# bmartacho/UniPose

Hardware: AMD Instinct MI355X
Metric: images/sec fwd+bwd, UniPose ResNet-101 368x368 (higher is better)
Workload: dtype f32; 1 GPU; UniPose ResNet-101 (K=16) train step: fwd + MSE + bwd + Adam, synthetic 368x368, batch 32/GPU (BASELINE.json configs[1]; configs[2] for N>1); global_batch=32, per_gpu_batch=32, parallelism=dp1, optimizer=torch.optim.Adam(lr=1e-4, fused=True), arithmetic=fp32 MFMA 32x32x2 everywhere

## Files before the change

include/unipose_hip.h:

```cpp
#ifndef UNIPOSE_HIP_H
#define UNIPOSE_HIP_H

#include <stddef.h>
#include <stdint.h>

#ifdef __cplusplus
extern "C" {
#endif

typedef enum {
    UP_OK = 0,
    UP_ERR_INVALID = -1,
    UP_ERR_UNSUPPORTED = -2,
    UP_ERR_LAUNCH = -3,
    UP_ERR_WORKSPACE = -4
} up_status;

const char* up_last_error(void);
int up_abi_version(void);

typedef struct {
    int32_t N, H, W;
    int32_t C, Cp;
    int32_t ldx;
    int32_t K;
    int32_t R, S;
    int32_t stride, pad, dil;
    int32_t P, Q;
    int32_t ldy;
    int32_t Kp;
} up_conv_desc;

typedef struct {
    float eps, momentum;
    float* running_mean;
    float* running_var;
    const float* gamma;
    const float* beta;
    float* mean;
    float* invstd;
    float* scale;
    float* shift;
    int32_t folded;
} up_bn_fold;
typedef struct {
    const float* scale;
    const float* shift;
    const float* bias;
    const float* residual;
    int32_t ldr;
    int32_t relu;
    float* stats;
    up_bn_fold* fold;
} up_conv_epilogue;

int up_pack_weights(const up_conv_desc* d, const float* w_oihw, float* w_fwd, float* w_dgrad, void* stream);
typedef struct {
    const float* w;
    float* w_fwd;
    float* w_dgrad;
    int32_t K, C, Cp, Kp, taps;
    int32_t geometry;
} up_pack_job;
int up_pack_weights_batched(const up_pack_job* jobs_device, int njobs, void* stream);

int up_conv2d_fwd(const up_conv_desc* d, const float* x, const float* w_fwd, float* y,
                  const up_conv_epilogue* ep, void* stream);
int up_conv_stats_tiles(const up_conv_desc* d);
int up_conv_stats_tiles_math(const up_conv_desc* d, int math);
int up_conv_split_parts(const up_conv_desc* d);
int up_stream_release(void* stream);
int up_stream_create_cu_mask(const uint32_t* mask, int words, void** stream);
int up_stream_destroy(void* stream);
int up_probe_placement(int blocks, int* out_device, void* stream);
int up_conv_tune(const char* key, int value);
long long up_conv_counter(const char* name);
int up_conv_tap_visits(const up_conv_desc* d, int data_gradient, double* image_order, double* tap_sorted, double* live);
int up_conv_wgrad_visits(const up_conv_desc* d, double* rect_fraction);

int up_conv2d_bwd_data(const up_conv_desc* d, const float* dy, const float* w_dgrad, float* dx,
                       const float* add, int ld_add, void* stream);
int up_bn_stats_groups_t(const void* y, int ldy, int64_t rows_per_group, int C, int groups, int dtype, float* stats, float eps,
                         float momentum, float* running_mean, float* running_var, const float* gamma, const float* beta, float* coef,
                         void* stream);
int up_bn_bwd_groups_finalized_t(const void* dz, int lddz, const uint32_t* relu_bits, const void* y, int ldy, const float* gamma,
                                 const float* coef, int relu, void* dy, int lddy, void* dres, int lddres, const float* gsum,
                                 int64_t rows_per_group, int C, int groups, int dtype, void* stream);
int up_bn_bwd_groups_prereduced_ok(int64_t rows_per_group, int C, int groups, int ld);
int up_bn_bwd_groups_prereduced_t(const void* dz, int lddz, const uint32_t* relu_bits, const void* y, int ldy, const float* gamma,
                                  const float* coef, int relu, void* dy, int lddy, void* dres, int lddres, float* dgamma, float* dbeta,
                                  float* workspace, size_t workspace_bytes, const float* partial, int tiles, int64_t rows_per_group,
                                  int C, int groups, int dtype, void* stream);
int up_conv_stats_tiles_grouped(const up_conv_desc* d, int groups);
int up_conv2d_fwd_grouped(const up_conv_desc* d, const float* x, const float* w_fwd, float* y, float* stats, int groups, void* stream);

typedef struct {
    const void* y;
    const uint32_t* relu_bits;
    const float* mean;
    const float* invstd;
    float* partial;
    int32_t ld, C;
    int32_t group_stride;
    float* dgamma;
    float* dbeta;
    float* gsum;
    int32_t folded;
} up_bn_reduce_slot;
typedef struct {
    const void* add;
    const uint32_t* add_relu_bits;
    up_bn_reduce_slot* bn;
    int32_t ld_add;
    int32_t groups;
} up_dgrad_epilogue;
int up_conv2d_bwd_data_tiles_grouped(const up_conv_desc* d, int groups);
int up_conv2d_bwd_data_tiles(const up_conv_desc* d);
int up_conv2d_bwd_data_tiles_math(const up_conv_desc* d, int math);
int up_conv2d_bwd_data_ex(const up_conv_desc* d, const void* dy, const void* w_dgrad, void* dx, const up_dgrad_epilogue* ep,
                          int math, void* stream);

typedef enum { UP_MATH_F32 = 0, UP_MATH_BF16X3 = 1, UP_MATH_BF16 = 2, UP_MATH_BF16S = 3, UP_MATH_BF16S_F32OUT = 4 } up_math;
int up_pack_weights_bf16(const up_conv_desc* d, const float* w_oihw, uint16_t* fwd_hi, uint16_t* fwd_lo,
                         uint16_t* dgrad_hi, uint16_t* dgrad_lo, void* stream);
typedef struct {
    const float* w;
    uint16_t* fwd_hi;
    uint16_t* fwd_lo;
    uint16_t* dgrad_hi;
    uint16_t* dgrad_lo;
    int32_t K, C, Cp, Kp, taps, reserved;
} up_pack_job_bf16;
int up_pack_weights_bf16_batched(const up_pack_job_bf16* jobs_device, int njobs, void* stream);
int up_conv2d_fwd_bf16(const up_conv_desc* d, const float* x, const uint16_t* w_hi, const uint16_t* w_lo, float* y,
                       const up_conv_epilogue* ep, int math, void* stream);
int up_conv2d_bwd_data_bf16(const up_conv_desc* d, const float* dy, const uint16_t* w_hi, const uint16_t* w_lo,
                            float* dx, const float* add, int ld_add, int math, void* stream);

size_t up_conv2d_bwd_weight_workspace(const up_conv_desc* d);
int up_conv2d_bwd_weight(const up_conv_desc* d, const float* x, const float* dy, float* dw_oihw,
                         float* dbias, void* workspace, size_t workspace_bytes, void* stream);
int up_conv2d_bwd_weight_bf16(const up_conv_desc* d, const float* x, const float* dy, float* dw_oihw,
                              float* dbias, void* workspace, size_t workspace_bytes, void* stream);

enum { UP_DT_F32 = 0, UP_DT_BF16 = 1 };
int up_conv2d_bwd_weight_bf16s(const up_conv_desc* d, const void* x_bf16, const void* dy_bf16, float* dw_oihw,
                               float* dbias, void* workspace, size_t workspace_bytes, void* stream);

int up_conv2d_bwd_weight_acc(const up_conv_desc* d, const void* x, const void* dy, float* dw_oihw, float* dbias,
                             void* workspace, size_t workspace_bytes, int math, int accumulate, void* stream);

int up_bn_eval_coeffs(const float* gamma, const float* beta, const float* running_mean,
                      const float* running_var, float eps, int C, float* scale, float* shift, void* stream);
int up_bn_finalize(const float* stats, int tiles, int C, float eps, float momentum,
                   float* running_mean, float* running_var,
                   const float* gamma, const float* beta,
                   float* mean, float* invstd, float* scale, float* shift, void* stream);
int up_bn_apply(const float* y, int ldy, const float* scale, const float* shift,
                const float* residual, int ldr, int relu, float* z, int ldz, uint32_t* relu_bits,
                int64_t rows, int C, void* stream);
int up_bn_bwd(const float* dz, int lddz, const float* z, int ldz, const uint32_t* relu_bits,
              const float* y, int ldy,
              const float* gamma, const float* mean, const float* invstd, int relu, int use_batch_stats,
              float* dy, int lddy, float* dres, int lddres, float* dgamma, float* dbeta,
              float* workspace, size_t workspace_bytes, int64_t rows, int C, void* stream);
size_t up_bn_bwd_workspace(int64_t rows, int C);
int up_bn_apply_t(const void* y, int ldy, const float* scale, const float* shift, const void* residual, int ldr,
                  int relu, void* z, int ldz, uint32_t* relu_bits, int64_t rows, int C, int dtype, void* stream);
int up_bn_apply_centered_t(const void* y, int ldy, const float* mean, const float* scale, const float* beta, const void* residual,
                           int ldr, int relu, void* z, int ldz, uint32_t* relu_bits, int64_t rows, int C, int dtype, void* stream);
int up_bn_bwd_t(const void* dz, int lddz, const void* z, int ldz, const uint32_t* relu_bits, const void* y, int ldy,
                const float* gamma, const float* mean, const float* invstd, int relu, int use_batch_stats,
                void* dy, int lddy, void* dres, int lddres, float* dgamma, float* dbeta,
                float* workspace, size_t workspace_bytes, int64_t rows, int C, int dtype, void* stream);
int up_bn_bwd_acc_t(const void* dz, int lddz, const void* z, int ldz, const uint32_t* relu_bits, const void* y, int ldy,
                const float* gamma, const float* mean, const float* invstd, int relu, int use_batch_stats,
                void* dy, int lddy, void* dres, int lddres, float* dgamma, float* dbeta, float* acc_dgamma, float* acc_dbeta,
                float* workspace, size_t workspace_bytes, int64_t rows, int C, int dtype, void* stream);
int up_bn_bwd_prereduced_t(const void* dz, int lddz, const uint32_t* relu_bits, const void* y, int ldy, const float* gamma,
                           const float* mean, const float* invstd, int relu, int use_batch_stats, void* dy, int lddy, void* dres,
                           int lddres, float* dgamma, float* dbeta, float* acc_dgamma, float* acc_dbeta, float* partial, int chunks,
                           int64_t rows, int C, int dtype, void* stream);
int up_bn_bwd_finalized_t(const void* dz, int lddz, const uint32_t* relu_bits, const void* y, int ldy, const float* gamma,
                          const float* mean, const float* invstd, int relu, int use_batch_stats, void* dy, int lddy, void* dres,
                          int lddres, const float* dgamma, const float* dbeta, int64_t rows, int C, int dtype, void* stream);

int up_bn_exact_stats_t(const void* y, int ldy, int64_t rows_per_group, int C, int groups, int dtype, float* stats, void* stream);
int up_bn_batch_stats_tiles(int64_t rows_per_group);
int up_bn_batch_stats_t(const void* y, int ldy, int64_t rows_per_group, int C, int groups, int dtype, float* stats, void* stream);
int up_bn_finalize_groups(const float* stats, int tiles, int C, int groups, int64_t rows_per_group, float eps, float momentum,
                          float* running_mean, float* running_var, const float* gamma, const float* beta, float* coef,
                          void* stream);
int up_bn_apply_groups_t(const void* y, int ldy, const float* coef, const float* beta, const void* res, int ldr, int relu, void* z,
                         int ldz, uint32_t* relu_bits, int64_t rows_per_group, int C, int groups, int dtype, void* stream);
size_t up_bn_bwd_groups_workspace(int64_t rows_per_group, int C, int groups);
int up_bn_bwd_groups_t(const void* dz, int lddz, const uint32_t* relu_bits, const void* y, int ldy, const float* gamma,
                       const float* coef, int relu, void* dy, int lddy, void* dres, int lddres, float* dgamma, float* dbeta,
                       float* workspace, size_t workspace_bytes, int64_t rows_per_group, int C, int groups, int dtype,
                       void* stream);

int up_relu_bwd(const float* dz, const float* z, float* dx, int64_t n, void* stream);
int up_copy2d(const float* src, int lds, float* dst, int ldd, int64_t rows, int C, void* stream);
int up_add2d(const float* a, int lda, const float* b, int ldb, float* dst, int ldd, int64_t rows, int C, void* stream);
int up_nchw_to_nhwc(const float* x, float* y, int N, int C, int H, int W, int ldy, void* stream);
int up_nhwc_to_nchw(const float* x, int ldx, float* y, int N, int C, int H, int W, void* stream);
int up_maxpool3s2_fwd(const float* x, int ldx, float* y, int ldy, uint8_t* idx,
                      int N, int H, int W, int C, int P, int Q, void* stream);
int up_maxpool3s2_bwd(const float* dy, int lddy, const uint8_t* idx, float* dx, int lddx,
                      int N, int H, int W, int C, int P, int Q, void* stream);
int up_bilinear_fwd(const float* x, int ldx, float* y, int ldy, int N, int H, int W, int C, int P, int Q, void* stream);
int up_bilinear_bwd(const float* dy, int lddy, float* dx, int lddx, int N, int H, int W, int C, int P, int Q, void* stream);
int up_gap_fwd(const float* x, int ldx, float* y, int N, int HW, int C, void* stream);
int up_gap_bwd(const float* dy, float* dx, int lddx, int N, int HW, int C, void* stream);
int up_avgpool9s8_fwd(const float* x, float* y, int ldy, int coff, int N, int H, int W, int P, int Q, void* stream);
int up_clip_nchw_to_nhwc(const float* x, float* y, int B, int T, int C, int H, int W, int ldy, void* stream);
int up_clip_avgpool9s8_fwd(const float* x, float* y, int ldy, int coff, int B, int T, int H, int W, int P, int Q, void* stream);
int up_clip_nhwc_to_nchw(const float* x, int ldx, float* y, int B, int T, int C, int H, int W, void* stream);
int up_dropout_fwd(const float* x, float* y, uint8_t* mask, const float* ext_mask, int64_t n,
                   float p, uint64_t seed, void* stream);
int up_dropout_bwd(const float* dy, const uint8_t* mask, float* dx, int64_t n, float p, void* stream);
int up_nchw_to_nhwc_t(const float* x, void* y, int N, int C, int H, int W, int ldy, int dt_out, void* stream);
int up_nhwc_to_nchw_t(const void* x, int ldx, float* y, int N, int C, int H, int W, int dt_in, void* stream);
int up_maxpool3s2_fwd_t(const void* x, int ldx, void* y, int ldy, uint8_t* idx, int N, int H, int W, int C, int P, int Q,
                        int dt_in, int dt_out, void* stream);
int up_maxpool3s2_bwd_t(const void* dy, int lddy, const uint8_t* idx, void* dx, int lddx, int N, int H, int W, int C, int P,
                        int Q, int dt_in, int dt_out, void* stream);
int up_bilinear_fwd_t(const void* x, int ldx, void* y, int ldy, int N, int H, int W, int C, int P, int Q, int dtype,
                      void* stream);
int up_bilinear_bwd_t(const void* dy, int lddy, void* dx, int lddx, int N, int H, int W, int C, int P, int Q, int dtype,
                      void* stream);
int up_gap_fwd_t(const void* x, int ldx, void* y, int N, int HW, int C, int dtype, void* stream);
int up_gap_bwd_t(const void* dy, void* dx, int lddx, int N, int HW, int C, int dtype, void* stream);
int up_dropout_fwd_t(const void* x, void* y, uint8_t* mask, const float* ext_mask, int64_t n, float p, uint64_t seed,
                     int dtype, void* stream);
int up_dropout_fwd_step_t(const void* x, void* y, uint8_t* mask, const float* ext_mask, int64_t n, float p, uint64_t seed,
                          const uint64_t* step_device, int dtype, void* stream);
int up_dropout_bwd_t(const void* dy, const uint8_t* mask, void* dx, int64_t n, float p, int dtype, void* stream);
int up_mse_fwd(const float* y, const float* t, float* loss, float* workspace, int64_t n, void* stream);
int up_mse_bwd(const float* y, const float* t, const float* dloss, float* dy, int64_t n, void* stream);
size_t up_mse_workspace(int64_t n);

int up_lstm0_fwd(const float* gates, int ldg, float* cell, float* hide, int ldo, int64_t rows, int Cg, void* stream);
int up_lstm0_bwd(const float* gates, int ldg, const float* dcell, const float* dhide, int ldo,
                 float* dgates, int64_t rows, int Cg, void* stream);
int up_lstm_fwd(const float* gates, int ldg, const float* cprev, int ldc, float* cell, float* hide, int ldo,
                int64_t rows, int Cg, void* stream);
int up_lstm_bwd(const float* gates, int ldg, const float* cprev, int ldc, const float* cell,
                const float* dcell, const float* dhide, int ldo,
                float* dgates, float* dcprev, int64_t rows, int Cg, void* stream);

int up_heatmap_argmax(const float* hm, int B, int J, int H, int W,
                      int32_t* idx, float* preds_xy, float* maxvals, void* stream);

int up_heatmap_decode(const float* hm, int64_t stride_b, int64_t stride_j, int64_t stride_p, int B, int J, int H, int W,
                      int P, int Q, int32_t* idx, float* preds_xy, float* maxvals, void* stream);

int up_make_heatmaps(const double* kpt_xy, int B, int K, int H, int W, double stride, double sigma, float* out,
                     void* stream);
int up_make_gaussian_maps(const double* center_xy, int N, int H, int W, double sigma, float* out, void* stream);
int up_normalize_image(const float* img_hwc, int B, int H, int W, int C, float mean, float stdv, float* out_chw,
                       void* stream);

enum { UP_BOX_OK = 0, UP_BOX_NO_VISIBLE_JOINT = 1 };
int up_make_box_maps(const double* kpt_xy, int B, int K, int height, int width, double stride, double sigma, float* out,
                     int32_t* status, void* stream);

enum { UP_PIX_U8 = 0, UP_PIX_F32 = 1 };
int up_augment_image(const void* src_hwc, int src_type, int B, int Hs, int Ws, int C, const int32_t* valid_hw, const double* inv,
                     int frames_per_map, float border, float mean, float stdv, float* out_chw, int Ho, int Wo, void* stream);

enum { UP_DS_LSP = 0, UP_DS_COCO = 1, UP_DS_PENN_ACTION = 2, UP_DS_NTID = 3, UP_DS_POSETRACK = 4, UP_DS_BBC = 5,
       UP_DS_MPII = 6 };
int up_pck_accuracy(const float* pred_xy, const float* target_xy, int B, int J, int H, int W, int dataset,
                    double thr_pck, double thr_pckh, double* acc, double* pck, double* pckh, double* visible,
                    int32_t* cnt, void* stream);

int up_peak_mask(const float* maps, int nmaps, int H, int W, uint8_t* mask, void* stream);
int up_box_argmax(const float* maps, int C, int H, int W, const int32_t* boxes, int P, int ch0, int nch,
                  int32_t* out_hw, void* stream);

enum { UP_PERSONS_OK = 0, UP_PERSONS_MISSING_CORNER = 1, UP_PERSONS_EMPTY_BOX = 2, UP_PERSONS_OVERFLOW = 3 };
enum { UP_PERSONS_CAP = 512 };
int up_persons_decode(const float* maps, int64_t stride_b, int64_t stride_j, int64_t stride_p, int B, int C, int H, int W,
                      int box_ch0, int joint_ch0, int njoints, int max_persons, int32_t* count, int32_t* status, int32_t* kpts,
                      void* stream);

typedef struct up_unipose_plan up_unipose_plan;
typedef struct {
    int32_t batch, height, width;
    int32_t output_stride;
    int32_t out_channels;
} up_unipose_config;
int up_unipose_plan_create(const up_unipose_config* cfg, up_unipose_plan** plan);
void up_unipose_plan_destroy(up_unipose_plan* plan);
int up_unipose_plan_num_convs(const up_unipose_plan* plan);
const char* up_unipose_plan_conv_name(const up_unipose_plan* plan, int i);
int up_unipose_plan_conv_shape(const up_unipose_plan* plan, int i, int32_t* oihw , int32_t* has_bias);
int up_unipose_plan_set_conv(up_unipose_plan* plan, int i, const float* w_oihw, const float* bias, void* stream);
size_t up_unipose_plan_workspace(const up_unipose_plan* plan);
int up_unipose_forward(up_unipose_plan* plan, const float* x_nchw, float* heat_nchw, void* workspace, size_t workspace_bytes,
                       void* stream);
int up_unipose_forward_upsampled(up_unipose_plan* plan, const float* x_nchw, float* heat_nchw, void* workspace,
                                 size_t workspace_bytes, void* stream);
int up_unipose_keypoints(up_unipose_plan* plan, const float* x_nchw, int out_h, int out_w, int32_t* idx, float* preds_xy,
                         float* maxvals, void* workspace, size_t workspace_bytes, void* stream);
int up_unipose_persons(up_unipose_plan* plan, const float* x_nchw, int box_ch0, int joint_ch0, int njoints, int max_persons,
                       int32_t* count, int32_t* status, int32_t* kpts, void* workspace, size_t workspace_bytes, void* stream);

typedef struct up_unipose_lstm_plan up_unipose_lstm_plan;
typedef struct {
    int32_t batch, frames, height, width;
    int32_t output_stride;
    int32_t num_classes;
} up_unipose_lstm_config;
int up_unipose_lstm_plan_create(const up_unipose_lstm_config* cfg, up_unipose_lstm_plan** plan);
void up_unipose_lstm_plan_destroy(up_unipose_lstm_plan* plan);
int up_unipose_lstm_plan_num_convs(const up_unipose_lstm_plan* plan);
const char* up_unipose_lstm_plan_conv_name(const up_unipose_lstm_plan* plan, int i);
int up_unipose_lstm_plan_conv_shape(const up_unipose_lstm_plan* plan, int i, int32_t* oihw , int32_t* has_bias);
int up_unipose_lstm_plan_set_conv(up_unipose_lstm_plan* plan, int i, const float* w_oihw, const float* bias, void* stream);
size_t up_unipose_lstm_plan_workspace(const up_unipose_lstm_plan* plan);
int up_unipose_lstm_step(up_unipose_lstm_plan* plan, const float* x_nchw, const float* center_nchw, const float* prev_hide,
                         const float* prev_cell, float* heat_nchw, float* cell_nchw, float* hide_nchw, void* workspace,
// ... 16 lines not shown
```

unipose_amd/_C.py:

```python
from __future__ import annotations

import ctypes as C
import os

_HERE = os.path.dirname(os.path.abspath(__file__))
LIB_PATH = os.path.join(_HERE, "libunipose_hip.so")



class ConvDesc(C.Structure):
    _fields_ = [(n, C.c_int32) for n in
                ("N", "H", "W", "C", "Cp", "ldx", "K", "R", "S", "stride", "pad", "dil", "P", "Q", "ldy", "Kp")]


class BnFold(C.Structure):
    _fields_ = [("eps", C.c_float), ("momentum", C.c_float), ("running_mean", C.c_void_p), ("running_var", C.c_void_p),
                ("gamma", C.c_void_p), ("beta", C.c_void_p), ("mean", C.c_void_p), ("invstd", C.c_void_p), ("scale", C.c_void_p),
                ("shift", C.c_void_p), ("folded", C.c_int32)]


class ConvEpilogue(C.Structure):
    _fields_ = [("scale", C.c_void_p), ("shift", C.c_void_p), ("bias", C.c_void_p), ("residual", C.c_void_p),
                ("ldr", C.c_int32), ("relu", C.c_int32), ("stats", C.c_void_p), ("fold", C.POINTER(BnFold))]


_i, _i64, _f, _u64, _sz, _p = C.c_int, C.c_int64, C.c_float, C.c_uint64, C.c_size_t, C.c_void_p


class BnReduceSlot(C.Structure):
    _fields_ = [("y", C.c_void_p), ("relu_bits", C.c_void_p), ("mean", C.c_void_p), ("invstd", C.c_void_p),
                ("partial", C.c_void_p), ("ld", C.c_int32), ("C", C.c_int32), ("group_stride", C.c_int32),
                ("dgamma", C.c_void_p), ("dbeta", C.c_void_p), ("gsum", C.c_void_p), ("folded", C.c_int32)]


class DgradEpilogue(C.Structure):
    _fields_ = [("add", C.c_void_p), ("add_relu_bits", C.c_void_p), ("bn", C.POINTER(BnReduceSlot)), ("ld_add", C.c_int32),
                ("groups", C.c_int32)]


_D, _E = C.POINTER(ConvDesc), C.POINTER(ConvEpilogue)

SIGNATURES = {
    "up_last_error": (C.c_char_p, []),
    "up_abi_version": (_i, []),
    "up_pack_weights": (_i, [_D, _p, _p, _p, _p]),
    "up_conv2d_fwd": (_i, [_D, _p, _p, _p, _E, _p]),
    "up_pack_weights_batched": (_i, [_p, _i, _p]),
    "up_conv_stats_tiles": (_i, [_D]),
    "up_conv_stats_tiles_math": (_i, [_D, _i]),
    "up_conv_split_parts": (_i, [_D]),
    "up_stream_release": (_i, [_p]),
    "up_stream_create_cu_mask": (_i, [C.POINTER(C.c_uint32), _i, C.POINTER(_p)]),
    "up_stream_destroy": (_i, [_p]),
    "up_probe_placement": (_i, [_i, _p, _p]),
    "up_conv_tune": (_i, [C.c_char_p, _i]),
    "up_conv_counter": (C.c_longlong, [C.c_char_p]),
    "up_conv_wgrad_visits": (_i, [_D, C.POINTER(C.c_double)]),
    "up_conv_tap_visits": (_i, [_D, _i, C.POINTER(C.c_double), C.POINTER(C.c_double), C.POINTER(C.c_double)]),
    "up_conv2d_bwd_data": (_i, [_D, _p, _p, _p, _p, _i, _p]),
    "up_conv2d_bwd_data_tiles": (_i, [_D]),
    "up_conv2d_bwd_data_tiles_math": (_i, [_D, _i]),
    "up_conv2d_bwd_data_ex": (_i, [_D, _p, _p, _p, C.POINTER(DgradEpilogue), _i, _p]),
    "up_conv_stats_tiles_grouped": (_i, [_D, _i]),
    "up_conv2d_bwd_data_tiles_grouped": (_i, [_D, _i]),
    "up_bn_bwd_groups_prereduced_ok": (_i, [_i64, _i, _i, _i]),
    "up_bn_stats_groups_t": (_i, [_p, _i, _i64, _i, _i, _i, _p, _f, _f, _p, _p, _p, _p, _p, _p]),
    "up_bn_bwd_groups_finalized_t": (_i, [_p, _i, _p, _p, _i, _p, _p, _i, _p, _i, _p, _i, _p, _i64, _i, _i, _i, _p]),
    "up_bn_bwd_groups_prereduced_t": (_i, [_p, _i, _p, _p, _i, _p, _p, _i, _p, _i, _p, _i, _p, _p, _p, _sz, _p, _i, _i64, _i, _i, _i, _p]),
    "up_conv2d_fwd_grouped": (_i, [_D, _p, _p, _p, _p, _i, _p]),
    "up_bn_bwd_prereduced_t": (_i, [_p, _i, _p, _p, _i, _p, _p, _p, _i, _i, _p, _i, _p, _i, _p, _p, _p, _p, _p, _i, _i64, _i,
                                    _i, _p]),
    "up_bn_bwd_finalized_t": (_i, [_p, _i, _p, _p, _i, _p, _p, _p, _i, _i, _p, _i, _p, _i, _p, _p, _i64, _i, _i, _p]),
    "up_pack_weights_bf16": (_i, [_D, _p, _p, _p, _p, _p, _p]),
    "up_pack_weights_bf16_batched": (_i, [_p, _i, _p]),
    "up_conv2d_fwd_bf16": (_i, [_D, _p, _p, _p, _p, _E, _i, _p]),
    "up_conv2d_bwd_data_bf16": (_i, [_D, _p, _p, _p, _p, _p, _i, _i, _p]),
    "up_conv2d_bwd_weight_workspace": (_sz, [_D]),
    "up_conv2d_bwd_weight": (_i, [_D, _p, _p, _p, _p, _p, _sz, _p]),
    "up_conv2d_bwd_weight_bf16": (_i, [_D, _p, _p, _p, _p, _p, _sz, _p]),
    "up_conv2d_bwd_weight_bf16s": (_i, [_D, _p, _p, _p, _p, _p, _sz, _p]),
    "up_conv2d_bwd_weight_acc": (_i, [_D, _p, _p, _p, _p, _p, _sz, _i, _i, _p]),
    "up_bn_eval_coeffs": (_i, [_p, _p, _p, _p, _f, _i, _p, _p, _p]),
    "up_bn_finalize": (_i, [_p, _i, _i, _f, _f, _p, _p, _p, _p, _p, _p, _p, _p, _p]),
    "up_bn_apply": (_i, [_p, _i, _p, _p, _p, _i, _i, _p, _i, _p, _i64, _i, _p]),
    "up_bn_bwd": (_i, [_p, _i, _p, _i, _p, _p, _i, _p, _p, _p, _i, _i, _p, _i, _p, _i, _p, _p, _p, _sz, _i64, _i, _p]),
    "up_bn_bwd_workspace": (_sz, [_i64, _i]),
    "up_bn_apply_t": (_i, [_p, _i, _p, _p, _p, _i, _i, _p, _i, _p, _i64, _i, _i, _p]),
    "up_bn_bwd_t": (_i, [_p, _i, _p, _i, _p, _p, _i, _p, _p, _p, _i, _i, _p, _i, _p, _i, _p, _p, _p, _sz, _i64, _i, _i, _p]),
    "up_bn_bwd_acc_t": (_i, [_p, _i, _p, _i, _p, _p, _i, _p, _p, _p, _i, _i, _p, _i, _p, _i, _p, _p, _p, _p, _p, _sz, _i64, _i, _i, _p]),
    "up_bn_exact_stats_t": (_i, [_p, _i, _i64, _i, _i, _i, _p, _p]),
    "up_bn_batch_stats_tiles": (_i, [_i64]),
    "up_bn_batch_stats_t": (_i, [_p, _i, _i64, _i, _i, _i, _p, _p]),
    "up_bn_finalize_groups": (_i, [_p, _i, _i, _i, _i64, _f, _f, _p, _p, _p, _p, _p, _p]),
    "up_bn_apply_groups_t": (_i, [_p, _i, _p, _p, _p, _i, _i, _p, _i, _p, _i64, _i, _i, _i, _p]),
    "up_bn_apply_centered_t": (_i, [_p, _i, _p, _p, _p, _p, _i, _i, _p, _i, _p, _i64, _i, _i, _p]),
    "up_bn_bwd_groups_workspace": (_sz, [_i64, _i, _i]),
    "up_bn_bwd_groups_t": (_i, [_p, _i, _p, _p, _i, _p, _p, _i, _p, _i, _p, _i, _p, _p, _p, _sz, _i64, _i, _i, _i, _p]),
    "up_relu_bwd": (_i, [_p, _p, _p, _i64, _p]),
    "up_copy2d": (_i, [_p, _i, _p, _i, _i64, _i, _p]),
    "up_add2d": (_i, [_p, _i, _p, _i, _p, _i, _i64, _i, _p]),
    "up_nchw_to_nhwc": (_i, [_p, _p, _i, _i, _i, _i, _i, _p]),
    "up_nhwc_to_nchw": (_i, [_p, _i, _p, _i, _i, _i, _i, _p]),
    "up_maxpool3s2_fwd": (_i, [_p, _i, _p, _i, _p, _i, _i, _i, _i, _i, _i, _p]),
    "up_maxpool3s2_bwd": (_i, [_p, _i, _p, _p, _i, _i, _i, _i, _i, _i, _i, _p]),
    "up_bilinear_fwd": (_i, [_p, _i, _p, _i, _i, _i, _i, _i, _i, _i, _p]),
    "up_bilinear_bwd": (_i, [_p, _i, _p, _i, _i, _i, _i, _i, _i, _i, _p]),
    "up_gap_fwd": (_i, [_p, _i, _p, _i, _i, _i, _p]),
    "up_gap_bwd": (_i, [_p, _p, _i, _i, _i, _i, _p]),
    "up_avgpool9s8_fwd": (_i, [_p, _p, _i, _i, _i, _i, _i, _i, _i, _p]),
    "up_dropout_fwd": (_i, [_p, _p, _p, _p, _i64, _f, _u64, _p]),
    "up_dropout_bwd": (_i, [_p, _p, _p, _i64, _f, _p]),
    "up_nchw_to_nhwc_t": (_i, [_p, _p, _i, _i, _i, _i, _i, _i, _p]),
    "up_nhwc_to_nchw_t": (_i, [_p, _i, _p, _i, _i, _i, _i, _i, _p]),
    "up_maxpool3s2_fwd_t": (_i, [_p, _i, _p, _i, _p, _i, _i, _i, _i, _i, _i, _i, _i, _p]),
    "up_maxpool3s2_bwd_t": (_i, [_p, _i, _p, _p, _i, _i, _i, _i, _i, _i, _i, _i, _i, _p]),
    "up_bilinear_fwd_t": (_i, [_p, _i, _p, _i, _i, _i, _i, _i, _i, _i, _i, _p]),
    "up_bilinear_bwd_t": (_i, [_p, _i, _p, _i, _i, _i, _i, _i, _i, _i, _i, _p]),
    "up_gap_fwd_t": (_i, [_p, _i, _p, _i, _i, _i, _i, _p]),
    "up_gap_bwd_t": (_i, [_p, _p, _i, _i, _i, _i, _i, _p]),
    "up_dropout_fwd_t": (_i, [_p, _p, _p, _p, _i64, _f, _u64, _i, _p]),
    "up_dropout_fwd_step_t": (_i, [_p, _p, _p, _p, _i64, _f, _u64, _p, _i, _p]),
    "up_dropout_bwd_t": (_i, [_p, _p, _p, _i64, _f, _i, _p]),
    "up_mse_fwd": (_i, [_p, _p, _p, _p, _i64, _p]),
    "up_mse_bwd": (_i, [_p, _p, _p, _p, _i64, _p]),
    "up_mse_workspace": (_sz, [_i64]),
    "up_lstm0_fwd": (_i, [_p, _i, _p, _p, _i, _i64, _i, _p]),
    "up_lstm0_bwd": (_i, [_p, _i, _p, _p, _i, _p, _i64, _i, _p]),
    "up_lstm_fwd": (_i, [_p, _i, _p, _i, _p, _p, _i, _i64, _i, _p]),
    "up_lstm_bwd": (_i, [_p, _i, _p, _i, _p, _p, _p, _i, _p, _p, _i64, _i, _p]),
    "up_heatmap_argmax": (_i, [_p, _i, _i, _i, _i, _p, _p, _p, _p]),
    "up_heatmap_decode": (_i, [_p, _i64, _i64, _i64, _i, _i, _i, _i, _i, _i, _p, _p, _p, _p]),
    "up_make_heatmaps": (_i, [_p, _i, _i, _i, _i, C.c_double, C.c_double, _p, _p]),
    "up_make_box_maps": (_i, [_p, _i, _i, _i, _i, C.c_double, C.c_double, _p, _p, _p]),
    "up_make_gaussian_maps": (_i, [_p, _i, _i, _i, C.c_double, _p, _p]),
    "up_normalize_image": (_i, [_p, _i, _i, _i, _i, _f, _f, _p, _p]),
    "up_augment_image": (_i, [_p, _i, _i, _i, _i, _i, _p, _p, _i, _f, _f, _f, _p, _i, _i, _p]),
    "up_pck_accuracy": (_i, [_p, _p, _i, _i, _i, _i, _i, C.c_double, C.c_double, _p, _p, _p, _p, _p, _p]),
    "up_peak_mask": (_i, [_p, _i, _i, _i, _p, _p]),
    "up_box_argmax": (_i, [_p, _i, _i, _i, _p, _i, _i, _i, _p, _p]),
    "up_persons_decode": (_i, [_p, _i64, _i64, _i64, _i, _i, _i, _i, _i, _i, _i, _i, _p, _p, _p, _p]),
    "up_unipose_plan_create": (_i, [_p, C.POINTER(_p)]),
    "up_unipose_plan_destroy": (None, [_p]),
    "up_unipose_plan_num_convs": (_i, [_p]),
    "up_unipose_plan_conv_name": (C.c_char_p, [_p, _i]),
    "up_unipose_plan_conv_shape": (_i, [_p, _i, C.POINTER(C.c_int32), C.POINTER(C.c_int32)]),
    "up_unipose_plan_set_conv": (_i, [_p, _i, _p, _p, _p]),
    "up_unipose_plan_workspace": (_sz, [_p]),
    "up_unipose_forward": (_i, [_p, _p, _p, _p, _sz, _p]),
    "up_unipose_forward_upsampled": (_i, [_p, _p, _p, _p, _sz, _p]),
    "up_unipose_keypoints": (_i, [_p, _p, _i, _i, _p, _p, _p, _p, _sz, _p]),
    "up_unipose_persons": (_i, [_p, _p, _i, _i, _i, _i, _p, _p, _p, _p, _sz, _p]),
    "up_clip_nchw_to_nhwc": (_i, [_p, _p, _i, _i, _i, _i, _i, _i, _p]),
    "up_clip_avgpool9s8_fwd": (_i, [_p, _p, _i, _i, _i, _i, _i, _i, _i, _i, _p]),
    "up_clip_nhwc_to_nchw": (_i, [_p, _i, _p, _i, _i, _i, _i, _i, _p]),
    "up_unipose_lstm_plan_create": (_i, [_p, C.POINTER(_p)]),
    "up_unipose_lstm_plan_destroy": (None, [_p]),
    "up_unipose_lstm_plan_num_convs": (_i, [_p]),
    "up_unipose_lstm_plan_conv_name": (C.c_char_p, [_p, _i]),
    "up_unipose_lstm_plan_conv_shape": (_i, [_p, _i, C.POINTER(C.c_int32), C.POINTER(C.c_int32)]),
    "up_unipose_lstm_plan_set_conv": (_i, [_p, _i, _p, _p, _p]),
    "up_unipose_lstm_plan_workspace": (_sz, [_p]),
    "up_unipose_lstm_step": (_i, [_p, _p, _p, _p, _p, _p, _p, _p, _p, _sz, _p]),
    "up_unipose_lstm_clip": (_i, [_p, _p, _p, _p, _p, _p, _p, _sz, _p]),
    "up_profile_variants": (_i, []),
    "up_profile_variant_name": (C.c_char_p, [_i]),
    "up_profile_begin": (_i, []),
    "up_profile_enable": (_i, [_i]),
    "up_profile_live_flops": (_i, [C.POINTER(C.c_double), _i]),
    "up_profile_end": (_i, [C.POINTER(C.c_double), _i]),
}

_lib = None
_ALLOW_HOST_POINTERS = False


class UniPoseHipError(RuntimeError):
    pass


def load(path: str | None = None):
    global _lib
    path = path or LIB_PATH
    if not os.path.exists(path):
        raise UniPoseHipError(
            f"{path} not found: build it with `python -c 'import __graft_entry__ as g; g.build()'` "
            "(hipcc --offload-arch=gfx950).  unipose_amd has no non-HIP fallback.")
    lib = C.CDLL(path)
    for name, (res, args) in SIGNATURES.items():
        fn = getattr(lib, name)
        fn.restype = res
        fn.argtypes = args
    _lib = lib
    return lib


def lib():
    return _lib if _lib is not None else load()


def check(status: int, what: str = ""):
    if status != 0:
        msg = lib().up_last_error().decode(errors="replace")
        if status == -2:
            raise NotImplementedError(f"{what}: {msg}")
        raise UniPoseHipError(f"{what}: status {status}: {msg}")
```

unipose_amd/csrc/norm_act.hip:

```cpp
#include "up_common.h"
#include "bn_fold.h"

#include <stdarg.h>
#include <stdlib.h>

namespace up {

static thread_local char g_err[512] = "";
void set_error(const char* fmt, ...) {
    va_list ap;
    va_start(ap, fmt);
    vsnprintf(g_err, sizeof(g_err), fmt, ap);
    va_end(ap);
}
int check_launch(const char* what) {
    hipError_t e = hipGetLastError();
    if (e != hipSuccess) {
        set_error("%s: %s", what, hipGetErrorString(e));
        return UP_ERR_LAUNCH;
    }
    return UP_OK;
}

static inline int grid_for(int64_t work_items, int per_block = 256, int cap = 16384) {
    int64_t g = (work_items + per_block - 1) / per_block;
    if (g < 1) g = 1;
    return (int)(g > cap ? cap : g);
}

__device__ __forceinline__ void wf_merge3(float& n1, float& m1, float& s1, float n2, float m2, float s2) {
    if (n2 == 0.f) return;
    if (n1 == 0.f) {
        n1 = n2;
        m1 = m2;
        s1 = s2;
        return;
    }
    float n = n1 + n2;
    float d = m2 - m1;
    m1 = m1 + d * (n2 / n);
    s1 = s1 + s2 + d * d * (n1 * n2 / n);
    n1 = n;
}

__global__ void __launch_bounds__(256) bn_eval_coeffs_kernel(const float* g, const float* b, const float* rm,
                                                             const float* rv, float eps, int C, float* scale,
                                                             float* shift) {
    int c = blockIdx.x * 256 + threadIdx.x;
    if (c >= C) return;
    float is = 1.0f / sqrtf(rv[c] + eps);
    float sc = g[c] * is;
    scale[c] = sc;
    shift[c] = b[c] - rm[c] * sc;
}

struct GroupArgs {
    int pstride, gstride;
};

template <int NV>
__global__ void __launch_bounds__(256) bn_fold_arrive_kernel(const float* partial, BnFold f) {
    __shared__ __attribute__((aligned(16))) unsigned char lds[FOLD_LDS_BYTES];
    const int c0 = blockIdx.y * FOLD_COLS;
    bn_fold_arrive<NV>(f, partial, blockIdx.x, c0, f.C - c0 < FOLD_COLS ? f.C - c0 : FOLD_COLS, lds, blockIdx.z);
}

__global__ void __launch_bounds__(256) bn_finalize_kernel(const float* stats, int tiles, int C, float eps, float mom,
                                                          float* rm, float* rv, const float* gamma,
                                                          const float* beta, float* mean_o, float* invstd_o,
                                                          float* scale, float* shift, GroupArgs grp) {
    __shared__ float red[256][3];
    const int c = blockIdx.x, t0 = threadIdx.x;
    {
        const int g = blockIdx.y;
        stats += (size_t)g * tiles * C * 3;
        mean_o += (size_t)g * grp.pstride;
        invstd_o += (size_t)g * grp.pstride;
        scale += (size_t)g * grp.pstride;
        shift += (size_t)g * grp.pstride;
    }
    float n = 0.f, m = 0.f, q = 0.f;
    for (int t = t0; t < tiles; t += 512) {
        const float* s = stats + ((size_t)t * C + c) * 3;
        const int t2 = t + 256;
        const float* s2 = stats + ((size_t)(t2 < tiles ? t2 : t) * C + c) * 3;
        const float a0 = s[0], a1 = s[1], a2 = s[2];
        const float b0 = t2 < tiles ? s2[0] : 0.f, b1 = s2[1], b2 = s2[2];
        wf_merge3(n, m, q, a0, a1, a2);
        wf_merge3(n, m, q, b0, b1, b2);
    }
    red[t0][0] = n;
    red[t0][1] = m;
    red[t0][2] = q;
    __syncthreads();
#pragma unroll
    for (int off = 128; off >= 1; off >>= 1) {
        if (t0 < off) {
            wf_merge3(n, m, q, red[t0 + off][0], red[t0 + off][1], red[t0 + off][2]);
            red[t0][0] = n;
            red[t0][1] = m;
            red[t0][2] = q;
        }
        __syncthreads();
    }
    if (t0 == 0) {
        float var = q / n;
        float is = 1.0f / sqrtf(var + eps);
        mean_o[c] = m;
        invstd_o[c] = is;
        float sc = gamma[c] * is;
        scale[c] = sc;
        shift[c] = beta[c] - m * sc;
        if (rm) {
            float unb = n > 1.f ? q / (n - 1.f) : var;
            rm[c] = (1.f - mom) * rm[c] + mom * m;
            rv[c] = (1.f - mom) * rv[c] + mom * unb;
        }
    }
}

template <typename T>
__global__ void __launch_bounds__(256) bn_apply_kernel(const T* y, int ldy, const float* scale,
                                                       const float* shift, const float* mean, const T* res, int ldr, int relu,
                                                       T* z, int ldz, uint32_t* relu_bits, int64_t total, int C4,
                                                       FastDiv fC4) {
    const int lane = threadIdx.x & 63;
    for (int64_t i0 = (int64_t)blockIdx.x * 256 + (threadIdx.x & ~63); i0 < total; i0 += (int64_t)gridDim.x * 256) {
        const int64_t i = i0 + lane;
        uint32_t nib = 0;
        if (i < total) {
            uint32_t row = fdiv((uint32_t)i, fC4);
            int c = ((int)i - (int)row * C4) * 4;
            float4 v = ld4<T>(y + (size_t)row * ldy + c);
            float4 s = *reinterpret_cast<const float4*>(scale + c);
            float4 h = *reinterpret_cast<const float4*>(shift + c);
            const float4 mu = mean ? *reinterpret_cast<const float4*>(mean + c) : make_float4(0.f, 0.f, 0.f, 0.f);
            v.x = (v.x - mu.x) * s.x + h.x;
            v.y = (v.y - mu.y) * s.y + h.y;
            v.z = (v.z - mu.z) * s.z + h.z;
            v.w = (v.w - mu.w) * s.w + h.w;
            if (res) {
                float4 r = ld4<T>(res + (size_t)row * ldr + c);
                v.x += r.x;
                v.y += r.y;
                v.z += r.z;
                v.w += r.w;
            }
            if (relu) {
                v.x = fmaxf(v.x, 0.f);
                v.y = fmaxf(v.y, 0.f);
                v.z = fmaxf(v.z, 0.f);
                v.w = fmaxf(v.w, 0.f);
            }
            st4(z + (size_t)row * ldz + c, v);
            nib = (v.x > 0.f ? 1u : 0u) | (v.y > 0.f ? 2u : 0u) | (v.z > 0.f ? 4u : 0u) | (v.w > 0.f ? 8u : 0u);
        }
        if (relu_bits) {
            uint32_t w = nib << (4 * (lane & 7));
            w |= __shfl_xor(w, 1);
            w |= __shfl_xor(w, 2);
            w |= __shfl_xor(w, 4);
            if ((lane & 7) == 0 && i < total) relu_bits[i >> 3] = w;
        }
    }
}

struct F8 {
    float v[8];
};
__device__ __forceinline__ F8 ld8(const bf16_t* p) {
    const uint4 u = *reinterpret_cast<const uint4*>(p);
    F8 r;
    r.v[0] = bf_lo(u.x); r.v[1] = bf_hi(u.x); r.v[2] = bf_lo(u.y); r.v[3] = bf_hi(u.y);
    r.v[4] = bf_lo(u.z); r.v[5] = bf_hi(u.z); r.v[6] = bf_lo(u.w); r.v[7] = bf_hi(u.w);
    return r;
}
__device__ __forceinline__ F8 ld8(const float* p) {
    const float4 a = *reinterpret_cast<const float4*>(p), b = *reinterpret_cast<const float4*>(p + 4);
    F8 r;
    r.v[0] = a.x; r.v[1] = a.y; r.v[2] = a.z; r.v[3] = a.w; r.v[4] = b.x; r.v[5] = b.y; r.v[6] = b.z; r.v[7] = b.w;
    return r;
}
__device__ __forceinline__ void st8(bf16_t* p, const F8& a) {
    uint4 u;
    u.x = pack_bf16x2(a.v[0], a.v[1]);
    u.y = pack_bf16x2(a.v[2], a.v[3]);
    u.z = pack_bf16x2(a.v[4], a.v[5]);
    u.w = pack_bf16x2(a.v[6], a.v[7]);
    *reinterpret_cast<uint4*>(p) = u;
}

__global__ void __launch_bounds__(256) bn_apply8_kernel(const bf16_t* y, int ldy, const float* scale, const float* shift,
                                                        const float* mean, const bf16_t* res, int ldr, int relu, bf16_t* z, int ldz,
                                                        uint32_t* relu_bits, int64_t total, int C8, FastDiv fC8) {
    const int lane = threadIdx.x & 63;
    for (int64_t i0 = (int64_t)blockIdx.x * 256 + (threadIdx.x & ~63); i0 < total; i0 += (int64_t)gridDim.x * 256) {
        const int64_t i = i0 + lane;
        uint32_t byte = 0;
        if (i < total) {
            const uint32_t row = fdiv((uint32_t)i, fC8);
            const int c = ((int)i - (int)row * C8) * 8;
            F8 v = ld8(y + (size_t)row * ldy + c);
            const F8 s = ld8(scale + c), h = ld8(shift + c);
            F8 mu;
#pragma unroll
            for (int e = 0; e < 8; ++e) mu.v[e] = 0.f;
            if (mean) mu = ld8(mean + c);
#pragma unroll
            for (int e = 0; e < 8; ++e) v.v[e] = (v.v[e] - mu.v[e]) * s.v[e] + h.v[e];
            if (res) {
                const F8 r = ld8(res + (size_t)row * ldr + c);
#pragma unroll
                for (int e = 0; e < 8; ++e) v.v[e] += r.v[e];
            }
            if (relu) {
#pragma unroll
                for (int e = 0; e < 8; ++e) v.v[e] = fmaxf(v.v[e], 0.f);
            }
            st8(z + (size_t)row * ldz + c, v);
#pragma unroll
            for (int e = 0; e < 8; ++e) byte |= v.v[e] > 0.f ? (1u << e) : 0u;
        }
        if (relu_bits) {
            uint32_t w = byte << (8 * (lane & 3));
            w |= __shfl_xor(w, 1);
            w |= __shfl_xor(w, 2);
            if ((lane & 3) == 0 && i < total) relu_bits[i >> 2] = w;
        }
    }
}

template <typename T>
struct Row16 {
    static constexpr int E = 16 / (int)sizeof(T);
    float v[E];
};
__device__ __forceinline__ Row16<float> ld16(const float* p) {
    const float4 a = *reinterpret_cast<const float4*>(p);
    return Row16<float>{{a.x, a.y, a.z, a.w}};
}
__device__ __forceinline__ Row16<bf16_t> ld16(const bf16_t* p) {
    const uint4 u = *reinterpret_cast<const uint4*>(p);
    return Row16<bf16_t>{{bf_lo(u.x), bf_hi(u.x), bf_lo(u.y), bf_hi(u.y), bf_lo(u.z), bf_hi(u.z), bf_lo(u.w), bf_hi(u.w)}};
}
__device__ __forceinline__ void st16(float* p, const Row16<float>& a) {
    *reinterpret_cast<float4*>(p) = make_float4(a.v[0], a.v[1], a.v[2], a.v[3]);
}
__device__ __forceinline__ void st16(bf16_t* p, const Row16<bf16_t>& a) {
    uint4 u;
    u.x = pack_bf16x2(a.v[0], a.v[1]);
    u.y = pack_bf16x2(a.v[2], a.v[3]);
    u.z = pack_bf16x2(a.v[4], a.v[5]);
    u.w = pack_bf16x2(a.v[6], a.v[7]);
    *reinterpret_cast<uint4*>(p) = u;
}
template <int E>
__device__ __forceinline__ void ldparam(const float* p, float (&o)[E]) {
#pragma unroll
    for (int e = 0; e < E; e += 4) {
        const float4 a = *reinterpret_cast<const float4*>(p + e);
        o[e] = a.x;
        o[e + 1] = a.y;
        o[e + 2] = a.z;
        o[e + 3] = a.w;
    }
}
constexpr int BN_ROWS_UNROLL = 4;

template <typename T>
__global__ void __launch_bounds__(256) bn_apply_rows_kernel(const T* __restrict__ y, int ldy, const float* __restrict__ scale,
                                                            const float* __restrict__ shift, const float* __restrict__ mean,
                                                            const T* __restrict__ res, int ldr,
                                                            int relu, T* __restrict__ z, int ldz, uint32_t* __restrict__ relu_bits,
                                                            int rows, int C, int lcs, GroupArgs grp) {
    constexpr int E = Row16<T>::E, LPW = 32 / E;
    const int lane = threadIdx.x & 63;
    const int64_t grow0 = (int64_t)blockIdx.z * rows;
    y += grow0 * ldy;
    z += grow0 * ldz;
    if (res) res += grow0 * ldr;
    scale += (size_t)blockIdx.z * grp.pstride;
    shift += mean ? 0 : (size_t)blockIdx.z * grp.pstride;
    const int cl = threadIdx.x & ((1 << lcs) - 1), rl = threadIdx.x >> lcs;
    const int rpb = 256 >> lcs;
    const int c = ((blockIdx.y << lcs) + cl) * E;
    float sc[E], sh[E], mu[E];
    ldparam<E>(scale + c, sc);
    ldparam<E>(shift + c, sh);
#pragma unroll
    for (int e = 0; e < E; ++e) mu[e] = 0.f;
    if (mean) ldparam<E>(mean + (size_t)blockIdx.z * grp.pstride + c, mu);
    const int stride = gridDim.x * rpb;
    for (int base = blockIdx.x * rpb; base < rows; base += BN_ROWS_UNROLL * stride) {
        Row16<T> v[BN_ROWS_UNROLL], r[BN_ROWS_UNROLL];
#pragma unroll
        for (int u = 0; u < BN_ROWS_UNROLL; ++u) {
            const int row = base + u * stride + rl;
            const int rr = row < rows ? row : rows - 1;
            v[u] = ld16(y + (size_t)rr * ldy + c);
            if (res) r[u] = ld16(res + (size_t)rr * ldr + c);
        }
#pragma unroll
        for (int u = 0; u < BN_ROWS_UNROLL; ++u) {
            const int row = base + u * stride + rl;
            const bool ok = row < rows;
            uint32_t bits = 0;
#pragma unroll
            for (int e = 0; e < E; ++e) {
                float t = (v[u].v[e] - mu[e]) * sc[e] + sh[e];
                if (res) t += r[u].v[e];
                if (relu) t = fmaxf(t, 0.f);
                v[u].v[e] = t;
                bits |= t > 0.f ? (1u << e) : 0u;
            }
            if (ok) st16(z + (size_t)row * ldz + c, v[u]);
            if (relu_bits) {
                uint32_t w = bits << (E * (lane & (LPW - 1)));
#pragma unroll
                for (int m = 1; m < LPW; m <<= 1) w |= __shfl_xor(w, m);
                if ((lane & (LPW - 1)) == 0 && ok) relu_bits[((grow0 + row) * C + c) >> 5] = w;
            }
        }
    }
}

template <typename T, int UNROLL, bool ZPATH>
__global__ void __launch_bounds__(256) bn_bwd_apply_rows_kernel(const T* __restrict__ dz, int lddz, const T* __restrict__ z, int ldz,
                                                                const uint32_t* __restrict__ bits, const T* __restrict__ y, int ldy,
                                                                const float* __restrict__ gamma, const float* __restrict__ mean,
                                                                const float* __restrict__ invstd, const float* __restrict__ dgamma,
                                                                const float* __restrict__ dbeta, int relu, int use_batch, float inv_m,
                                                                T* __restrict__ dy, int lddy, T* __restrict__ dres, int lddres,
                                                                int rows, int C, int lcs, GroupArgs grp) {
    constexpr int E = Row16<T>::E;
    const int64_t grow0 = (int64_t)blockIdx.z * rows;
    dz += grow0 * lddz;
    y += grow0 * ldy;
    dy += grow0 * lddy;
    if (ZPATH) z += grow0 * ldz;
    if (dres) dres += grow0 * lddres;
    mean += (size_t)blockIdx.z * grp.pstride;
    invstd += (size_t)blockIdx.z * grp.pstride;
    dgamma += (size_t)blockIdx.z * grp.gstride;
    dbeta += (size_t)blockIdx.z * grp.gstride;
    const int cl = threadIdx.x & ((1 << lcs) - 1), rl = threadIdx.x >> lcs;
    const int rpb = 256 >> lcs;
    const int c = ((blockIdx.y << lcs) + cl) * E;
    float kk[E], aa[E], bb[E], mu[E];
    {
        float is[E], t[E];
        ldparam<E>(invstd + c, is);
        ldparam<E>(gamma + c, kk);
        ldparam<E>(mean + c, mu);
#pragma unroll
        for (int e = 0; e < E; ++e) kk[e] *= is[e];
        ldparam<E>(dbeta + c, t);
#pragma unroll
        for (int e = 0; e < E; ++e) aa[e] = use_batch ? -kk[e] * t[e] * inv_m : 0.f;
        ldparam<E>(dgamma + c, t);
#pragma unroll
        for (int e = 0; e < E; ++e) bb[e] = use_batch ? -kk[e] * is[e] * t[e] * inv_m : 0.f;
    }
    const int stride = gridDim.x * rpb;
    for (int base = blockIdx.x * rpb + rl; base < rows; base += UNROLL * stride) {
        Row16<T> g[UNROLL], yv[UNROLL], zz[ZPATH ? UNROLL : 1];
        uint32_t mk[UNROLL];
#pragma unroll
        for (int u = 0; u < UNROLL; ++u) {
            const int row = base + u * stride;
            const int rr = row < rows ? row : rows - 1;
            g[u] = ld16(dz + (size_t)rr * lddz + c);
            yv[u] = ld16(y + (size_t)rr * ldy + c);
            mk[u] = 0xffffffffu;
            if (ZPATH) {
                zz[u] = ld16(z + (size_t)rr * ldz + c);
            } else if (relu) {
                const int64_t b = (grow0 + rr) * C + c;
                mk[u] = bits[b >> 5] >> (int)(b & 31);
            }
        }
#pragma unroll
        for (int u = 0; u < UNROLL; ++u) {
            const int row = base + u * stride;
            if (row >= rows) continue;
            Row16<T> o;
#pragma unroll
            for (int e = 0; e < E; ++e) {
                float ge = g[u].v[e];
                const bool pos = ZPATH ? zz[ZPATH ? u : 0].v[e] > 0.f : ((mk[u] >> e) & 1u) != 0u;
                if (!pos) ge = 0.f;
                g[u].v[e] = ge;
                o.v[e] = kk[e] * ge + (aa[e] + (yv[u].v[e] - mu[e]) * bb[e]);
            }
            if (dres) st16(dres + (size_t)row * lddres + c, g[u]);
            st16(dy + (size_t)row * lddy + c, o);
        }
    }
}
template <typename T>
static void launch_bn_bwd_apply_rows(dim3 grid, hipStream_t st, const T* dz, int lddz, const T* z, int ldz, const uint32_t* bits,
                                     const T* y, int ldy, const float* gamma, const float* mean, const float* invstd,
                                     const float* dgamma, const float* dbeta, int relu, int use_batch, float inv_m, T* dy, int lddy,
                                     T* dres, int lddres, int rows, int C, int lcs, GroupArgs grp) {
    constexpr int U = sizeof(T) == 4 ? 1 : 2;
    if (relu && !bits)
        hipLaunchKernelGGL((bn_bwd_apply_rows_kernel<T, U, true>), grid, dim3(256), 0, st, dz, lddz, z, ldz, bits, y, ldy, gamma, mean,
                           invstd, dgamma, dbeta, relu, use_batch, inv_m, dy, lddy, dres, lddres, rows, C, lcs, grp);
    else
        hipLaunchKernelGGL((bn_bwd_apply_rows_kernel<T, U, false>), grid, dim3(256), 0, st, dz, lddz, z, ldz, bits, y, ldy, gamma, mean,
                           invstd, dgamma, dbeta, relu, use_batch, inv_m, dy, lddy, dres, lddres, rows, C, lcs, grp);
}
template <typename T>
static bool rows_geometry(int64_t rows, int C, dim3& grid, int& lcs) {
    constexpr int E = 16 / (int)sizeof(T);
    if (C % E) return false;
    const int cgs = C / E;
    if (cgs < 8 || (cgs & (cgs - 1)) || rows >= (1ll << 31)) return false;
    const int lc = cgs < 256 ? cgs : 256;
    lcs = 0;
    while ((1 << lcs) < lc) ++lcs;
    const int rpb = 256 / lc, gy = cgs / lc;
    int64_t gx = (rows + (int64_t)rpb * BN_ROWS_UNROLL - 1) / ((int64_t)rpb * BN_ROWS_UNROLL);
    const int64_t cap = 2048 / gy;
    if (gx > cap) gx = cap;
    if (gx < 1) gx = 1;
    grid = dim3((unsigned)gx, (unsigned)gy);
    return true;
}
static int g_bn_rows = -1;
void set_bn_rows(int on) { g_bn_rows = on ? 1 : 0; }
static bool bn_rows_enabled() {
    if (g_bn_rows < 0) {
        const char* e = getenv("UP_BN_ROWS");
        g_bn_rows = (e && atoi(e) == 0) ? 0 : 1;
    }
    return g_bn_rows != 0;
}

constexpr int BNS_ROWS = 256;
template <typename T>
__global__ void __launch_bounds__(256) bn_batch_stats_kernel(const T* y, int ldy, int rows_per_group, int C, float* stats, int tiles,
                                                             BnFold fold) {
    __shared__ __attribute__((aligned(16))) float red[16][64][3];
    static_assert(sizeof(float) * 16 * 64 * 3 >= FOLD_LDS_BYTES, "the fold's ticket re-uses the reduction buffer");
    const int cq = threadIdx.x & 15, rl = threadIdx.x >> 4;
    const int c = blockIdx.y * 64 + cq * 4;
    const int g = blockIdx.z;
    const int r0 = blockIdx.x * BNS_ROWS, r1 = min(rows_per_group, r0 + BNS_ROWS);
    float n = 0.f, sh[4] = {0.f, 0.f, 0.f, 0.f}, s[4] = {0.f, 0.f, 0.f, 0.f}, q[4] = {0.f, 0.f, 0.f, 0.f};
    if (c < C) {
        const T* base = y + (size_t)g * rows_per_group * ldy + c;
        const float4 s0 = ld4<T>(base + (size_t)r0 * ldy);
        sh[0] = s0.x, sh[1] = s0.y, sh[2] = s0.z, sh[3] = s0.w;
        auto acc = [&](const float4& v) {
            const float x[4] = {v.x, v.y, v.z, v.w};
#pragma unroll
            for (int e = 0; e < 4; ++e) {
                const float d = x[e] - sh[e];
                s[e] += d;
                q[e] += d * d;
            }
            n += 1.f;
        };
// ... 287 lines not shown

__device__ __forceinline__ uint32_t mix_hash(uint64_t seed, uint64_t idx) {
    uint64_t v = seed ^ (idx * 0x9E3779B97F4A7C15ull);
    v ^= v >> 30;
    v *= 0xBF58476D1CE4E5B9ull;
    v ^= v >> 27;
    v *= 0x94D049BB133111EBull;
    v ^= v >> 31;
    return (uint32_t)(v >> 40);
}
template <typename T>
__global__ void __launch_bounds__(256) dropout_fwd_kernel(const T* x, T* y, uint8_t* mask,
                                                          const float* ext, int64_t n, float p, float inv_keep,
                                                          uint64_t seed, const uint64_t* step_dev) {
    if (step_dev) seed += *step_dev * 0x9E3779B97F4A7C15ull;
    for (int64_t i = (int64_t)blockIdx.x * 256 + threadIdx.x; i < n; i += (int64_t)gridDim.x * 256) {
        bool keep;
        if (ext)
            keep = ext[i] != 0.f;
        else
            keep = (float)mix_hash(seed, (uint64_t)i) * (1.0f / 16777216.0f) >= p;
        mask[i] = keep ? 1 : 0;
        st1(y + i, keep ? ld1(x + i) * inv_keep : 0.f);
    }
}
template <typename T>
__global__ void __launch_bounds__(256) dropout_bwd_kernel(const T* dy, const uint8_t* mask, T* dx, int64_t n,
                                                          float inv_keep) {
    for (int64_t i = (int64_t)blockIdx.x * 256 + threadIdx.x; i < n; i += (int64_t)gridDim.x * 256)
        st1(dx + i, mask[i] ? ld1(dy + i) * inv_keep : 0.f);
}

__device__ __forceinline__ float block_sum_256(float v, float* red) {
#pragma unroll
    for (int off = 32; off >= 1; off >>= 1) v += __shfl_down(v, off);
    if ((threadIdx.x & 63) == 0) red[threadIdx.x >> 6] = v;
    __syncthreads();
    return red[0] + red[1] + red[2] + red[3];
}
__global__ void __launch_bounds__(256) mse_partial_kernel(const float* y, const float* t, float* ws, int64_t n) {
    __shared__ float red[4];
    float s = 0.f;
    for (int64_t i = (int64_t)blockIdx.x * 256 + threadIdx.x; i < n; i += (int64_t)gridDim.x * 256) {
        float d = y[i] - t[i];
        s += d * d;
    }
    s = block_sum_256(s, red);
    if (threadIdx.x == 0) ws[blockIdx.x] = s;
}
__global__ void __launch_bounds__(256) mse_final_kernel(const float* ws, int parts, float inv_n, float* loss) {
    __shared__ float red[4];
    float s = 0.f;
    for (int i = threadIdx.x; i < parts; i += 256) s += ws[i];
    s = block_sum_256(s, red);
    if (threadIdx.x == 0) loss[0] = s * inv_n;
}
__global__ void __launch_bounds__(256) mse_bwd_kernel(const float* y, const float* t, const float* dloss, float* dy,
                                                      int64_t n, float two_inv_n) {
    float k = two_inv_n * dloss[0];
    for (int64_t i = (int64_t)blockIdx.x * 256 + threadIdx.x; i < n; i += (int64_t)gridDim.x * 256)
        dy[i] = (y[i] - t[i]) * k;
}

constexpr int MSE_PARTS = 512;
constexpr int BNB_ROWS = 128;

}

using namespace up;

extern "C" const char* up_last_error(void) { return g_err; }
extern "C" int up_stream_create_cu_mask(const uint32_t* mask, int words, void** stream) {
    UP_REQUIRE(mask && words > 0 && stream, UP_ERR_INVALID, "stream_create_cu_mask: bad argument");
#ifdef UP_EMU
    *stream = nullptr;
    return UP_OK;
#else
    hipStream_t st = nullptr;
    hipError_t e = hipExtStreamCreateWithCUMask(&st, (uint32_t)words, mask);
    if (e != hipSuccess) {
        set_error("stream_create_cu_mask: %s", hipGetErrorString(e));
        return UP_ERR_LAUNCH;
    }
    *stream = st;
    return UP_OK;
#endif
}
extern "C" int up_stream_destroy(void* stream) {
#ifndef UP_EMU
    if (stream && hipStreamDestroy(as_stream(stream)) != hipSuccess) {
        (void)hipGetLastError();
        return UP_ERR_LAUNCH;
    }
#endif
    return UP_OK;
}
namespace up {
__global__ void __launch_bounds__(64) placement_kernel(int* out) {
#ifndef UP_EMU
    if (threadIdx.x == 0) {
        const unsigned xcc = __builtin_amdgcn_s_getreg((20 << 0) | (0 << 6) | (3 << 11));
        const unsigned hw = __builtin_amdgcn_s_getreg((4 << 0) | (0 << 6) | (31 << 11));
        out[2 * blockIdx.x] = (int)(xcc & 15u);
        out[2 * blockIdx.x + 1] = (int)((hw >> 8) & 0xffu);
        for (int i = 0; i < 2000; ++i) __builtin_amdgcn_s_sleep(32);
    }
#else
    if (threadIdx.x == 0) out[2 * blockIdx.x] = out[2 * blockIdx.x + 1] = 0;
#endif
}
}
extern "C" int up_probe_placement(int blocks, int* out_device, void* stream) {
    UP_REQUIRE(blocks > 0 && out_device, UP_ERR_INVALID, "probe_placement: bad argument");
    hipLaunchKernelGGL(placement_kernel, dim3(blocks), dim3(64), 0, as_stream(stream), out_device);
    return check_launch("probe_placement");
}

extern "C" int up_abi_version(void) { return 10; }

extern "C" int up_bn_eval_coeffs(const float* gamma, const float* beta, const float* rm, const float* rv, float eps,
                                 int C, float* scale, float* shift, void* stream) {
    UP_REQUIRE(gamma && beta && rm && rv && scale && shift && C > 0, UP_ERR_INVALID, "bn_eval_coeffs: bad argument");
    hipLaunchKernelGGL(bn_eval_coeffs_kernel, dim3(cdiv(C, 256)), dim3(256), 0, as_stream(stream), gamma, beta, rm,
                       rv, eps, C, scale, shift);
    return check_launch("bn_eval_coeffs");
}

extern "C" int up_bn_finalize(const float* stats, int tiles, int C, float eps, float momentum, float* rm, float* rv,
                              const float* gamma, const float* beta, float* mean, float* invstd, float* scale,
                              float* shift, void* stream) {
    UP_REQUIRE(stats && gamma && beta && mean && invstd && scale && shift && tiles > 0 && C > 0, UP_ERR_INVALID,
               "bn_finalize: bad argument");
    UP_REQUIRE((rm == nullptr) == (rv == nullptr), UP_ERR_INVALID, "bn_finalize: running stats must come in pairs");
    BnFold f;
    memset(&f, 0, sizeof(f));
    UP_REQUIRE(bn_fold_scratch(as_stream(stream), tiles, C, 3, &f), UP_ERR_WORKSPACE,
               "bn_finalize: %d partial rows x %d channels exceed the per-stream merge scratch", tiles, C);
    f.eps = eps;
    f.mom = momentum;
    f.rm = rm;
    f.rv = rv;
    f.gamma = gamma;
    f.beta = beta;
    f.mean = mean;
    f.invstd = invstd;
    f.scale = scale;
    f.shift = shift;
    hipLaunchKernelGGL(bn_fold_arrive_kernel<3>, dim3(tiles, cdiv(C, FOLD_COLS)), dim3(256), 0, as_stream(stream), stats, f);
    return check_launch("bn_finalize");
}

static int bn_apply_impl(const void* y, int ldy, const float* mean, const float* scale, const float* shift, const void* res,
                         int ldr, int relu, void* z, int ldz, uint32_t* relu_bits, int64_t rows, int C, int dtype,
                         void* stream) {
    UP_REQUIRE(y && scale && shift && z && rows > 0 && C > 0, UP_ERR_INVALID, "bn_apply: bad argument");
    UP_REQUIRE(C % 4 == 0 && ldy % 4 == 0 && ldz % 4 == 0 && (!res || ldr % 4 == 0), UP_ERR_INVALID,
               "bn_apply: C and strides must be multiples of 4");
    UP_REQUIRE(rows * (C / 4) < (1ll << 31), UP_ERR_UNSUPPORTED, "bn_apply: tensor too large");
    UP_REQUIRE(dtype == UP_DT_F32 || dtype == UP_DT_BF16, UP_ERR_INVALID, "bn_apply: dtype %d", dtype);
    int64_t total = rows * (C / 4);
    {
        dim3 grid;
        int lcs = 0;
        if (bn_rows_enabled() && dtype == UP_DT_BF16 && ldy % 8 == 0 && ldz % 8 == 0 && (!res || ldr % 8 == 0) &&
            rows_geometry<bf16_t>(rows, C, grid, lcs)) {
            hipLaunchKernelGGL(bn_apply_rows_kernel<bf16_t>, grid, dim3(256), 0, as_stream(stream), (const bf16_t*)y, ldy, scale,
                               shift, mean, (const bf16_t*)res, ldr, relu, (bf16_t*)z, ldz, relu_bits, (int)rows, C, lcs, GroupArgs{0, 0});
            return check_launch("bn_apply");
        }
        if (bn_rows_enabled() && dtype == UP_DT_F32 && rows_geometry<float>(rows, C, grid, lcs)) {
            hipLaunchKernelGGL(bn_apply_rows_kernel<float>, grid, dim3(256), 0, as_stream(stream), (const float*)y, ldy, scale,
                               shift, mean, (const float*)res, ldr, relu, (float*)z, ldz, relu_bits, (int)rows, C, lcs, GroupArgs{0, 0});
            return check_launch("bn_apply");
        }
    }
    if (dtype == UP_DT_BF16 && C % 8 == 0 && ldy % 8 == 0 && ldz % 8 == 0 && (!res || ldr % 8 == 0))
        hipLaunchKernelGGL(bn_apply8_kernel, dim3(grid_for(total / 2)), dim3(256), 0, as_stream(stream), (const bf16_t*)y, ldy,
                           scale, shift, mean, (const bf16_t*)res, ldr, relu, (bf16_t*)z, ldz, relu_bits, total / 2, C / 8,
                           make_fastdiv(C / 8));
    else if (dtype == UP_DT_BF16)
        hipLaunchKernelGGL(bn_apply_kernel<bf16_t>, dim3(grid_for(total)), dim3(256), 0, as_stream(stream),
                           (const bf16_t*)y, ldy, scale, shift, mean, (const bf16_t*)res, ldr, relu, (bf16_t*)z, ldz, relu_bits,
                           total, C / 4, make_fastdiv(C / 4));
    else
        hipLaunchKernelGGL(bn_apply_kernel<float>, dim3(grid_for(total)), dim3(256), 0, as_stream(stream), (const float*)y,
                           ldy, scale, shift, mean, (const float*)res, ldr, relu, (float*)z, ldz, relu_bits, total, C / 4,
                           make_fastdiv(C / 4));
    return check_launch("bn_apply");
}
extern "C" int up_bn_apply_t(const void* y, int ldy, const float* scale, const float* shift, const void* res,
                             int ldr, int relu, void* z, int ldz, uint32_t* relu_bits, int64_t rows, int C, int dtype,
                             void* stream) {
    return bn_apply_impl(y, ldy, nullptr, scale, shift, res, ldr, relu, z, ldz, relu_bits, rows, C, dtype, stream);
}
extern "C" int up_bn_apply_centered_t(const void* y, int ldy, const float* mean, const float* scale, const float* beta,
                                      const void* res, int ldr, int relu, void* z, int ldz, uint32_t* relu_bits, int64_t rows,
                                      int C, int dtype, void* stream) {
    UP_REQUIRE(mean, UP_ERR_INVALID, "bn_apply_centered: null mean");
    return bn_apply_impl(y, ldy, mean, scale, beta, res, ldr, relu, z, ldz, relu_bits, rows, C, dtype, stream);
}
extern "C" int up_bn_apply(const float* y, int ldy, const float* scale, const float* shift, const float* res,
                           int ldr, int relu, float* z, int ldz, uint32_t* relu_bits, int64_t rows, int C,
                           void* stream) {
    return up_bn_apply_t(y, ldy, scale, shift, res, ldr, relu, z, ldz, relu_bits, rows, C, UP_DT_F32, stream);
}

extern "C" size_t up_bn_bwd_workspace(int64_t rows, int C) {
    return (size_t)cdiv(rows, BNB_ROWS) * C * 2 * sizeof(float);
}

namespace up {
template <typename T>
static void launch_bn_bwd(const T* dz, int lddz, const T* z, int ldz, const uint32_t* relu_bits, const T* y, int ldy,
                          const float* gamma, const float* mean, const float* invstd, int relu, int use_batch_stats, T* dy,
                          int lddy, T* dres, int lddres, float* dgamma, float* dbeta, float* acc_dgamma, float* acc_dbeta,
                          float* workspace, int64_t rows, int C, hipStream_t st, int prereduced_chunks = 0) {
    if (prereduced_chunks >= 0) {
        int chunks = prereduced_chunks > 0 ? prereduced_chunks : cdiv(rows, BNB_ROWS);
        BnFold f;
        memset(&f, 0, sizeof(f));
        const bool tree = !acc_dgamma && bn_fold_scratch(st, chunks, C, 2, &f);
        f.dgamma = dgamma;
        f.dbeta = dbeta;
        const bool carried = tree && prereduced_chunks == 0 && bn_fold_enabled();
        BnFold none;
        memset(&none, 0, sizeof(none));
        if (prereduced_chunks == 0)
            hipLaunchKernelGGL(bn_bwd_reduce_kernel<T>, dim3(chunks, cdiv(C, 64)), dim3(256), 0, st, dz, lddz, z, ldz, relu_bits,
                               y, ldy, mean, invstd, relu, workspace, rows, C, BNB_ROWS, GroupArgs{0, 0}, carried ? f : none);
        if (tree && !carried)
            hipLaunchKernelGGL(bn_fold_arrive_kernel<2>, dim3(chunks, cdiv(C, FOLD_COLS)), dim3(256), 0, st, (const float*)workspace, f);
        else if (!tree)
            hipLaunchKernelGGL(bn_bwd_finalize_kernel, dim3(C), dim3(256), 0, st, (const float*)workspace, chunks, C,
                               dgamma, dbeta, acc_dgamma, acc_dbeta, GroupArgs{0, 0});
    }
    int64_t total = rows * (C / 4);
    {
        dim3 grid;
        int lcs = 0;
        constexpr int E = 16 / (int)sizeof(T);
        if (bn_rows_enabled() && lddz % E == 0 && ldy % E == 0 && lddy % E == 0 && (!relu || relu_bits || ldz % E == 0) &&
            (!dres || lddres % E == 0) && rows_geometry<T>(rows, C, grid, lcs)) {
            launch_bn_bwd_apply_rows<T>(grid, st, dz, lddz, z, ldz, relu_bits, y, ldy, gamma, mean, invstd, (const float*)dgamma,
                                        (const float*)dbeta, relu, use_batch_stats, 1.0f / (float)rows, dy, lddy, dres, lddres,
                                        (int)rows, C, lcs, GroupArgs{0, 0});
            return;
        }
    }
    if constexpr (sizeof(T) == 2) {
        if (C % 8 == 0 && lddz % 8 == 0 && ldy % 8 == 0 && lddy % 8 == 0 && (!relu || relu_bits || ldz % 8 == 0) &&
            (!dres || lddres % 8 == 0)) {
            hipLaunchKernelGGL(bn_bwd_apply8_kernel, dim3(grid_for(total / 2)), dim3(256), 0, st, dz, lddz, z, ldz, relu_bits,
                               y, ldy, gamma, mean, invstd, (const float*)dgamma, (const float*)dbeta, relu, use_batch_stats,
                               1.0f / (float)rows, dy, lddy, dres, lddres, total / 2, C / 8, make_fastdiv(C / 8));
            return;
        }
    }
    hipLaunchKernelGGL(bn_bwd_apply_kernel<T>, dim3(grid_for(total)), dim3(256), 0, st, dz, lddz, z, ldz, relu_bits, y,
                       ldy, gamma, mean, invstd, (const float*)dgamma, (const float*)dbeta, relu, use_batch_stats,
                       1.0f / (float)rows, dy, lddy, dres, lddres, total, C / 4, make_fastdiv(C / 4));
}
}

extern "C" int up_bn_bwd_t(const void* dz, int lddz, const void* z, int ldz, const uint32_t* relu_bits, const void* y,
                           int ldy, const float* gamma, const float* mean, const float* invstd, int relu,
                           int use_batch_stats, void* dy, int lddy, void* dres, int lddres, float* dgamma, float* dbeta,
                           float* workspace, size_t workspace_bytes, int64_t rows, int C, int dtype, void* stream) {
    return up_bn_bwd_acc_t(dz, lddz, z, ldz, relu_bits, y, ldy, gamma, mean, invstd, relu, use_batch_stats, dy, lddy, dres,
                           lddres, dgamma, dbeta, nullptr, nullptr, workspace, workspace_bytes, rows, C, dtype, stream);
}
extern "C" int up_bn_bwd_acc_t(const void* dz, int lddz, const void* z, int ldz, const uint32_t* relu_bits, const void* y,
                               int ldy, const float* gamma, const float* mean, const float* invstd, int relu,
                               int use_batch_stats, void* dy, int lddy, void* dres, int lddres, float* dgamma,
                               float* dbeta, float* acc_dgamma, float* acc_dbeta, float* workspace, size_t workspace_bytes,
                               int64_t rows, int C, int dtype, void* stream) {
    UP_REQUIRE(!acc_dgamma == !acc_dbeta, UP_ERR_INVALID, "bn_bwd: acc_dgamma and acc_dbeta come together");
    UP_REQUIRE(dz && y && gamma && mean && invstd && dy && dgamma && dbeta && workspace, UP_ERR_INVALID,
               "bn_bwd: null pointer");
    UP_REQUIRE(!relu || z || relu_bits, UP_ERR_INVALID, "bn_bwd: relu needs the forward output z or its sign bits");
    UP_REQUIRE(C % 4 == 0 && lddz % 4 == 0 && ldy % 4 == 0 && lddy % 4 == 0 && (!relu || relu_bits || ldz % 4 == 0) &&
                   (!dres || lddres % 4 == 0),
               UP_ERR_INVALID, "bn_bwd: C and strides must be multiples of 4");
    UP_REQUIRE(rows * (C / 4) < (1ll << 31), UP_ERR_UNSUPPORTED, "bn_bwd: tensor too large");
    UP_REQUIRE(workspace_bytes >= up_bn_bwd_workspace(rows, C), UP_ERR_WORKSPACE, "bn_bwd: workspace too small");
    UP_REQUIRE(dtype == UP_DT_F32 || dtype == UP_DT_BF16, UP_ERR_INVALID, "bn_bwd: dtype %d", dtype);
    hipStream_t st = as_stream(stream);
    if (dtype == UP_DT_BF16)
        launch_bn_bwd<bf16_t>((const bf16_t*)dz, lddz, (const bf16_t*)z, ldz, relu_bits, (const bf16_t*)y, ldy, gamma, mean,
                              invstd, relu, use_batch_stats, (bf16_t*)dy, lddy, (bf16_t*)dres, lddres, dgamma, dbeta,
                              acc_dgamma, acc_dbeta, workspace, rows, C, st);
    else
        launch_bn_bwd<float>((const float*)dz, lddz, (const float*)z, ldz, relu_bits, (const float*)y, ldy, gamma, mean,
                             invstd, relu, use_batch_stats, (float*)dy, lddy, (float*)dres, lddres, dgamma, dbeta,
                             acc_dgamma, acc_dbeta, workspace, rows, C, st);
    return check_launch("bn_bwd");
}
extern "C" int up_bn_bwd_prereduced_t(const void* dz, int lddz, const uint32_t* relu_bits, const void* y, int ldy,
                                      const float* gamma, const float* mean, const float* invstd, int relu, int use_batch_stats,
                                      void* dy, int lddy, void* dres, int lddres, float* dgamma, float* dbeta, float* acc_dgamma,
                                      float* acc_dbeta, float* partial, int chunks, int64_t rows, int C, int dtype, void* stream) {
    UP_REQUIRE(!acc_dgamma == !acc_dbeta, UP_ERR_INVALID, "bn_bwd_prereduced: acc_dgamma and acc_dbeta come together");
    UP_REQUIRE(dz && y && gamma && mean && invstd && dy && dgamma && dbeta && partial && chunks > 0, UP_ERR_INVALID,
               "bn_bwd_prereduced: null pointer / no partial rows");
    UP_REQUIRE(!relu || relu_bits, UP_ERR_INVALID, "bn_bwd_prereduced: relu needs the sign bits of the forward output");
    UP_REQUIRE(C % 4 == 0 && lddz % 4 == 0 && ldy % 4 == 0 && lddy % 4 == 0 && (!dres || lddres % 4 == 0), UP_ERR_INVALID,
               "bn_bwd_prereduced: C and strides must be multiples of 4");
    UP_REQUIRE(rows * (C / 4) < (1ll << 31), UP_ERR_UNSUPPORTED, "bn_bwd_prereduced: tensor too large");
    UP_REQUIRE(dtype == UP_DT_F32 || dtype == UP_DT_BF16, UP_ERR_INVALID, "bn_bwd_prereduced: dtype %d", dtype);
    if (dtype == UP_DT_BF16)
        launch_bn_bwd<bf16_t>((const bf16_t*)dz, lddz, (const bf16_t*)nullptr, 0, relu_bits, (const bf16_t*)y, ldy, gamma, mean, invstd,
                              relu, use_batch_stats, (bf16_t*)dy, lddy, (bf16_t*)dres, lddres, dgamma, dbeta, acc_dgamma, acc_dbeta,
                              partial, rows, C, as_stream(stream), chunks);
    else
        launch_bn_bwd<float>((const float*)dz, lddz, (const float*)nullptr, 0, relu_bits, (const float*)y, ldy, gamma, mean, invstd, relu,
                             use_batch_stats, (float*)dy, lddy, (float*)dres, lddres, dgamma, dbeta, acc_dgamma, acc_dbeta, partial,
                             rows, C, as_stream(stream), chunks);
    return check_launch("bn_bwd_prereduced");
}
extern "C" int up_bn_bwd_finalized_t(const void* dz, int lddz, const uint32_t* relu_bits, const void* y, int ldy, const float* gamma,
                                     const float* mean, const float* invstd, int relu, int use_batch_stats, void* dy, int lddy,
                                     void* dres, int lddres, const float* dgamma, const float* dbeta, int64_t rows, int C, int dtype,
                                     void* stream) {
    UP_REQUIRE(dz && y && gamma && mean && invstd && dy && dgamma && dbeta, UP_ERR_INVALID, "bn_bwd_finalized: null pointer");
    UP_REQUIRE(!relu || relu_bits, UP_ERR_INVALID, "bn_bwd_finalized: relu needs the sign bits of the forward output");
    UP_REQUIRE(C % 4 == 0 && lddz % 4 == 0 && ldy % 4 == 0 && lddy % 4 == 0 && (!dres || lddres % 4 == 0), UP_ERR_INVALID,
               "bn_bwd_finalized: C and strides must be multiples of 4");
    UP_REQUIRE(rows * (C / 4) < (1ll << 31), UP_ERR_UNSUPPORTED, "bn_bwd_finalized: tensor too large");
    UP_REQUIRE(dtype == UP_DT_F32 || dtype == UP_DT_BF16, UP_ERR_INVALID, "bn_bwd_finalized: dtype %d", dtype);
    if (dtype == UP_DT_BF16)
        launch_bn_bwd<bf16_t>((const bf16_t*)dz, lddz, (const bf16_t*)nullptr, 0, relu_bits, (const bf16_t*)y, ldy, gamma, mean, invstd,
                              relu, use_batch_stats, (bf16_t*)dy, lddy, (bf16_t*)dres, lddres, const_cast<float*>(dgamma),
                              const_cast<float*>(dbeta), nullptr, nullptr, nullptr, rows, C, as_stream(stream), -1);
    else
        launch_bn_bwd<float>((const float*)dz, lddz, (const float*)nullptr, 0, relu_bits, (const float*)y, ldy, gamma, mean, invstd, relu,
                             use_batch_stats, (float*)dy, lddy, (float*)dres, lddres, const_cast<float*>(dgamma),
                             const_cast<float*>(dbeta), nullptr, nullptr, nullptr, rows, C, as_stream(stream), -1);
    return check_launch("bn_bwd_finalized");
}
extern "C" int up_bn_bwd(const float* dz, int lddz, const float* z, int ldz, const uint32_t* relu_bits,
                         const float* y, int ldy,
                         const float* gamma, const float* mean, const float* invstd, int relu, int use_batch_stats,
                         float* dy, int lddy, float* dres, int lddres, float* dgamma, float* dbeta,
                         float* workspace, size_t workspace_bytes, int64_t rows, int C, void* stream) {
    return up_bn_bwd_t(dz, lddz, z, ldz, relu_bits, y, ldy, gamma, mean, invstd, relu, use_batch_stats, dy, lddy, dres,
                       lddres, dgamma, dbeta, workspace, workspace_bytes, rows, C, UP_DT_F32, stream);
}

constexpr int BN_MAXG = 8;
__global__ void __launch_bounds__(256) bn_running_groups_kernel(const float* coef, int groups, int C, float n, float eps, float mom,
                                                                float* rm, float* rv) {
    const int c = blockIdx.x * 256 + threadIdx.x;
    if (c >= C) return;
    float m = rm[c], v = rv[c];
    for (int g = 0; g < groups; ++g) {
        const float mean = coef[(size_t)g * 4 * C + c], is = coef[(size_t)g * 4 * C + C + c];
        const float var = 1.0f / (is * is) - eps;
        const float unb = n > 1.f ? var * (n / (n - 1.f)) : var;
        m = (1.f - mom) * m + mom * mean;
        v = (1.f - mom) * v + mom * unb;
    }
    rm[c] = m;
    rv[c] = v;
}
__global__ void __launch_bounds__(256) bn_sum_groups_kernel(const float* gsum, int groups, int C, float* dgamma, float* dbeta) {
    const int c = blockIdx.x * 256 + threadIdx.x;
    if (c >= C) return;
    float a = 0.f, b = 0.f;
    for (int g = 0; g < groups; ++g) {
        a += gsum[(size_t)g * 2 * C + c];
        b += gsum[(size_t)g * 2 * C + C + c];
    }
    dgamma[c] = a;
    dbeta[c] = b;
}

extern "C" int up_bn_batch_stats_tiles(int64_t rows_per_group) { return cdiv(rows_per_group, BNS_ROWS); }
namespace up {
static void launch_bn_batch_stats(const void* y, int ldy, int64_t rows_per_group, int C, int groups, int dtype, float* stats,
                                  const BnFold& fold, hipStream_t st) {
    const int tiles = cdiv(rows_per_group, BNS_ROWS);
    dim3 grid(tiles, cdiv(C, 64), groups);
    if (dtype == UP_DT_BF16)
        hipLaunchKernelGGL(bn_batch_stats_kernel<bf16_t>, grid, dim3(256), 0, st, (const bf16_t*)y, ldy, (int)rows_per_group, C, stats,
                           tiles, fold);
    else
        hipLaunchKernelGGL(bn_batch_stats_kernel<float>, grid, dim3(256), 0, st, (const float*)y, ldy, (int)rows_per_group, C, stats,
                           tiles, fold);
}
}
extern "C" int up_bn_batch_stats_t(const void* y, int ldy, int64_t rows_per_group, int C, int groups, int dtype, float* stats,
                                   void* stream) {
    UP_REQUIRE(y && stats && rows_per_group > 0 && rows_per_group < (1ll << 31) && C > 0 && groups > 0 && groups <= 65535,
               UP_ERR_INVALID, "bn_batch_stats: bad argument");
    UP_REQUIRE(C % 4 == 0 && ldy % 4 == 0, UP_ERR_INVALID, "bn_batch_stats: C and ldy must be multiples of 4");
    UP_REQUIRE(dtype == UP_DT_F32 || dtype == UP_DT_BF16, UP_ERR_INVALID, "bn_batch_stats: dtype %d", dtype);
    BnFold none;
    memset(&none, 0, sizeof(none));
    launch_bn_batch_stats(y, ldy, rows_per_group, C, groups, dtype, stats, none, as_stream(stream));
    return check_launch("bn_batch_stats");
}
extern "C" int up_bn_stats_groups_t(const void* y, int ldy, int64_t rows_per_group, int C, int groups, int dtype, float* stats,
                                    float eps, float momentum, float* rm, float* rv, const float* gamma, const float* beta, float* coef,
                                    void* stream) {
    UP_REQUIRE(y && stats && gamma && beta && coef && rows_per_group > 0 && rows_per_group < (1ll << 31) && C > 0 && groups > 0 &&
                   groups <= 65535, UP_ERR_INVALID, "bn_stats_groups: bad argument");
    UP_REQUIRE(C % 4 == 0 && ldy % 4 == 0, UP_ERR_INVALID, "bn_stats_groups: C and ldy must be multiples of 4");
    UP_REQUIRE(dtype == UP_DT_F32 || dtype == UP_DT_BF16, UP_ERR_INVALID, "bn_stats_groups: dtype %d", dtype);
    UP_REQUIRE((rm == nullptr) == (rv == nullptr), UP_ERR_INVALID, "bn_stats_groups: running stats must come in pairs");
    const int tiles = cdiv(rows_per_group, BNS_ROWS);
    BnFold f;
    memset(&f, 0, sizeof(f));
    if (bn_fold_enabled() && groups <= BN_MAXG && bn_fold_scratch(as_stream(stream), tiles, C, 3, &f, groups)) {
        f.eps = eps;
        f.mom = momentum;
        f.rm = rm;
        f.rv = rv;
        f.gamma = gamma;
        f.beta = beta;
        f.mean = coef;
        f.invstd = coef + C;
        f.scale = coef + 2 * C;
        f.shift = coef + 3 * C;
        f.ostride = 4 * C;
        launch_bn_batch_stats(y, ldy, rows_per_group, C, groups, dtype, stats, f, as_stream(stream));
        return check_launch("bn_stats_groups");
    }
    if (int e = up_bn_batch_stats_t(y, ldy, rows_per_group, C, groups, dtype, stats, stream)) return e;
    return up_bn_finalize_groups(stats, tiles, C, groups, rows_per_group, eps, momentum, rm, rv, gamma, beta, coef, stream);
}
extern "C" int up_bn_exact_stats_t(const void* y, int ldy, int64_t rows_per_group, int C, int groups, int dtype, float* stats,
                                   void* stream) {
    UP_REQUIRE(y && stats && rows_per_group > 0 && rows_per_group <= 4096 && C > 0 && groups > 0 && groups <= 65535, UP_ERR_INVALID,
               "bn_exact_stats: bad argument (1..4096 rows per group)");
    UP_REQUIRE(dtype == UP_DT_F32 || dtype == UP_DT_BF16, UP_ERR_INVALID, "bn_exact_stats: dtype %d", dtype);
    dim3 grid(cdiv(C, 256), groups);
    if (dtype == UP_DT_BF16)
        hipLaunchKernelGGL(bn_exact_stats_kernel<bf16_t>, grid, dim3(256), 0, as_stream(stream), (const bf16_t*)y, ldy,
                           (int)rows_per_group, C, stats);
    else
        hipLaunchKernelGGL(bn_exact_stats_kernel<float>, grid, dim3(256), 0, as_stream(stream), (const float*)y, ldy,
                           (int)rows_per_group, C, stats);
    return check_launch("bn_exact_stats");
}
extern "C" int up_bn_finalize_groups(const float* stats, int tiles, int C, int groups, int64_t rows_per_group, float eps,
                                     float momentum, float* rm, float* rv, const float* gamma, const float* beta, float* coef,
                                     void* stream) {
    UP_REQUIRE(stats && gamma && beta && coef && tiles > 0 && C > 0 && groups > 0 && groups <= 65535 && rows_per_group > 0,
               UP_ERR_INVALID, "bn_finalize_groups: bad argument");
    UP_REQUIRE((rm == nullptr) == (rv == nullptr), UP_ERR_INVALID, "bn_finalize_groups: running stats must come in pairs");
    BnFold f;
    memset(&f, 0, sizeof(f));
    if (groups <= BN_MAXG && bn_fold_scratch(as_stream(stream), tiles, C, 3, &f, groups)) {
        f.eps = eps;
        f.mom = momentum;
        f.rm = rm;
        f.rv = rv;
        f.gamma = gamma;
        f.beta = beta;
        f.mean = coef;
        f.invstd = coef + C;
        f.scale = coef + 2 * C;
        f.shift = coef + 3 * C;
        f.ostride = 4 * C;
        hipLaunchKernelGGL(bn_fold_arrive_kernel<3>, dim3(tiles, cdiv(C, FOLD_COLS), groups), dim3(256), 0, as_stream(stream), stats, f);
        return check_launch("bn_finalize_groups");
    }
    hipLaunchKernelGGL(bn_finalize_kernel, dim3(C, groups), dim3(256), 0, as_stream(stream), stats, tiles, C, eps, momentum,
                       (float*)nullptr, (float*)nullptr, gamma, beta, coef, coef + C, coef + 2 * C, coef + 3 * C, GroupArgs{4 * C, 0});
    if (rm)
        hipLaunchKernelGGL(bn_running_groups_kernel, dim3(cdiv(C, 256)), dim3(256), 0, as_stream(stream), (const float*)coef, groups,
                           C, (float)rows_per_group, eps, momentum, rm, rv);
    return check_launch("bn_finalize_groups");
}
extern "C" int up_bn_apply_groups_t(const void* y, int ldy, const float* coef, const float* beta, const void* res, int ldr, int relu,
                                    void* z, int ldz, uint32_t* relu_bits, int64_t rows_per_group, int C, int groups, int dtype,
                                    void* stream) {
    const float* gmean = beta ? coef : nullptr;
    const float* gshift = beta ? beta : coef + 3 * C;
    UP_REQUIRE(y && z && coef && groups > 0 && groups <= 65535 && rows_per_group > 0, UP_ERR_INVALID, "bn_apply_groups: bad argument");
    UP_REQUIRE(dtype == UP_DT_F32 || dtype == UP_DT_BF16, UP_ERR_INVALID, "bn_apply_groups: dtype %d", dtype);
    UP_REQUIRE(!relu_bits || (rows_per_group * C) % 32 == 0, UP_ERR_UNSUPPORTED,
               "bn_apply_groups: rows_per_group * C must be a multiple of 32 (a group's ReLU bits start on a word)");
    const size_t es = dtype == UP_DT_BF16 ? 2 : 4;
    dim3 grid;
    int lcs = 0;
    const GroupArgs ga{4 * C, 0};
    if (dtype == UP_DT_F32 && ldy % 4 == 0 && ldz % 4 == 0 && (!res || ldr % 4 == 0) && rows_geometry<float>(rows_per_group, C, grid, lcs)) {
        grid.z = groups;
        hipLaunchKernelGGL(bn_apply_rows_kernel<float>, grid, dim3(256), 0, as_stream(stream), (const float*)y, ldy, coef + 2 * C,
                           gshift, gmean, (const float*)res, ldr, relu, (float*)z, ldz, relu_bits, (int)rows_per_group, C, lcs, ga);
        return check_launch("bn_apply_groups");
    }
    if (dtype == UP_DT_BF16 && ldy % 8 == 0 && ldz % 8 == 0 && (!res || ldr % 8 == 0) &&
        rows_geometry<bf16_t>(rows_per_group, C, grid, lcs)) {
        grid.z = groups;
        hipLaunchKernelGGL(bn_apply_rows_kernel<bf16_t>, grid, dim3(256), 0, as_stream(stream), (const bf16_t*)y, ldy, coef + 2 * C,
                           gshift, gmean, (const bf16_t*)res, ldr, relu, (bf16_t*)z, ldz, relu_bits, (int)rows_per_group, C, lcs, ga);
        return check_launch("bn_apply_groups");
    }
    for (int g = 0; g < groups; ++g) {
        const float* cg = coef + (size_t)g * 4 * C;
        const size_t r0 = (size_t)g * rows_per_group;
        if (int e = bn_apply_impl((const char*)y + r0 * ldy * es, ldy, beta ? cg : nullptr, cg + 2 * C, beta ? beta : cg + 3 * C,
                                  res ? (const char*)res + r0 * ldr * es : nullptr, ldr, relu, (char*)z + r0 * ldz * es, ldz,
                                  relu_bits ? relu_bits + r0 * C / 32 : nullptr, rows_per_group, C, dtype, stream))
            return e;
    }
    return UP_OK;
}
extern "C" size_t up_bn_bwd_groups_workspace(int64_t rows_per_group, int C, int groups) {
    return (size_t)groups * (up_bn_bwd_workspace(rows_per_group, C) + (size_t)2 * C * sizeof(float));
}
namespace up {
template <typename T>
static bool launch_bn_bwd_groups(const T* dz, int lddz, const uint32_t* relu_bits, const T* y, int ldy, const float* gamma,
                                 const float* coef, int relu, T* dy, int lddy, T* dres, int lddres, float* dgamma, float* dbeta,
                                 float* workspace, int64_t rows, int C, int groups, hipStream_t st,
                                 const float* prereduced = nullptr, int prereduced_tiles = 0, const float* finalized_gsum = nullptr) {
    constexpr int E = 16 / (int)sizeof(T);
    dim3 grid;
    int lcs = 0;
    if (!(lddz % E == 0 && ldy % E == 0 && lddy % E == 0 && (!dres || lddres % E == 0) && rows_geometry<T>(rows, C, grid, lcs)))
        return false;
    const int chunks = prereduced ? prereduced_tiles : cdiv(rows, BNB_ROWS);
    float* gsum = finalized_gsum ? const_cast<float*>(finalized_gsum) : workspace;
    const float* partial = prereduced ? prereduced : workspace + (size_t)groups * 2 * C;
    const GroupArgs ga{4 * C, 2 * C};
    if (!finalized_gsum) {
        BnFold f;
        memset(&f, 0, sizeof(f));
        const bool tree = groups <= BN_MAXG && bn_fold_scratch(st, chunks, C, 2, &f, groups);
        f.dgamma = dgamma;
        f.dbeta = dbeta;
        f.gsum = gsum;
        f.ostride = 2 * C;
        const bool carried = tree && !prereduced && bn_fold_enabled();
        BnFold none;
        memset(&none, 0, sizeof(none));
        if (!prereduced)
            hipLaunchKernelGGL(bn_bwd_reduce_kernel<T>, dim3(chunks, cdiv(C, 64), groups), dim3(256), 0, st, dz, lddz, (const T*)nullptr, 0,
                               relu_bits, y, ldy, coef, coef + C, relu, workspace + (size_t)groups * 2 * C, rows, C, BNB_ROWS, ga,
                               carried ? f : none);
        if (carried) {
        } else if (tree) {
            hipLaunchKernelGGL(bn_fold_arrive_kernel<2>, dim3(chunks, cdiv(C, FOLD_COLS), groups), dim3(256), 0, st, (const float*)partial, f);
        } else {
            hipLaunchKernelGGL(bn_bwd_finalize_kernel, dim3(C, groups), dim3(256), 0, st, (const float*)partial, chunks, C, gsum, gsum + C,
                               (float*)nullptr, (float*)nullptr, ga);
            hipLaunchKernelGGL(bn_sum_groups_kernel, dim3(cdiv(C, 256)), dim3(256), 0, st, (const float*)gsum, groups, C, dgamma, dbeta);
        }
    }
    grid.z = groups;
    launch_bn_bwd_apply_rows<T>(grid, st, dz, lddz, (const T*)nullptr, 0, relu_bits, y, ldy, gamma, coef, coef + C, (const float*)gsum,
                                (const float*)(gsum + C), relu, 1, 1.0f / (float)rows, dy, lddy, dres, lddres, (int)rows, C, lcs, ga);
    return true;
}
}
extern "C" int up_bn_bwd_groups_t(const void* dz, int lddz, const uint32_t* relu_bits, const void* y, int ldy, const float* gamma,
                                  const float* coef, int relu, void* dy, int lddy, void* dres, int lddres, float* dgamma,
                                  float* dbeta, float* workspace, size_t workspace_bytes, int64_t rows_per_group, int C, int groups,
                                  int dtype, void* stream) {
    UP_REQUIRE(dz && y && dy && gamma && coef && dgamma && dbeta && workspace && groups > 0 && groups <= 65535 && rows_per_group > 0,
               UP_ERR_INVALID, "bn_bwd_groups: bad argument");
    UP_REQUIRE(dtype == UP_DT_F32 || dtype == UP_DT_BF16, UP_ERR_INVALID, "bn_bwd_groups: dtype %d", dtype);
    UP_REQUIRE(!relu || relu_bits, UP_ERR_INVALID, "bn_bwd_groups: relu needs the sign bits of the forward output");
    UP_REQUIRE(C % 4 == 0 && rows_per_group * (C / 4) < (1ll << 31), UP_ERR_UNSUPPORTED, "bn_bwd_groups: C %% 4 or tensor too large");
    UP_REQUIRE(workspace_bytes >= up_bn_bwd_groups_workspace(rows_per_group, C, groups), UP_ERR_WORKSPACE,
               "bn_bwd_groups: workspace too small");
    UP_REQUIRE(!relu_bits || (rows_per_group * C) % 32 == 0, UP_ERR_UNSUPPORTED,
               "bn_bwd_groups: rows_per_group * C must be a multiple of 32 (a group's ReLU bits start on a word)");
    const size_t es = dtype == UP_DT_BF16 ? 2 : 4;
    hipStream_t st = as_stream(stream);
    const bool done = dtype == UP_DT_BF16
        ? launch_bn_bwd_groups<bf16_t>((const bf16_t*)dz, lddz, relu_bits, (const bf16_t*)y, ldy, gamma, coef, relu, (bf16_t*)dy, lddy,
                                       (bf16_t*)dres, lddres, dgamma, dbeta, workspace, rows_per_group, C, groups, st)
        : launch_bn_bwd_groups<float>((const float*)dz, lddz, relu_bits, (const float*)y, ldy, gamma, coef, relu, (float*)dy, lddy,
                                      (float*)dres, lddres, dgamma, dbeta, workspace, rows_per_group, C, groups, st);
    if (done) return check_launch("bn_bwd_groups");
    if (hipMemsetAsync(dgamma, 0, sizeof(float) * C, st) != hipSuccess || hipMemsetAsync(dbeta, 0, sizeof(float) * C, st) != hipSuccess)
        return check_launch("bn_bwd_groups memset");
    float* gsum = workspace;
    float* ws = workspace + 2 * (size_t)C;
    for (int g = 0; g < groups; ++g) {
        const float* cg = coef + (size_t)g * 4 * C;
        const size_t r0 = (size_t)g * rows_per_group;
        if (int e = up_bn_bwd_acc_t((const char*)dz + r0 * lddz * es, lddz, nullptr, 0, relu_bits ? relu_bits + r0 * C / 32 : nullptr,
                                    (const char*)y + r0 * ldy * es, ldy, gamma, cg, cg + C, relu, 1, (char*)dy + r0 * lddy * es, lddy,
                                    dres ? (char*)dres + r0 * lddres * es : nullptr, lddres, gsum, gsum + C, dgamma, dbeta, ws,
                                    workspace_bytes - 2 * (size_t)C * sizeof(float), rows_per_group, C, dtype, stream))
            return e;
    }
    return UP_OK;
}

extern "C" int up_bn_bwd_groups_prereduced_t(const void* dz, int lddz, const uint32_t* relu_bits, const void* y, int ldy,
                                             const float* gamma, const float* coef, int relu, void* dy, int lddy, void* dres,
                                             int lddres, float* dgamma, float* dbeta, float* workspace, size_t workspace_bytes,
                                             const float* partial, int tiles, int64_t rows_per_group, int C, int groups, int dtype,
                                             void* stream) {
    UP_REQUIRE(dz && y && dy && gamma && coef && dgamma && dbeta && workspace && partial && tiles > 0 && groups > 0 && groups <= BN_MAXG &&
               rows_per_group > 0, UP_ERR_INVALID, "bn_bwd_groups_prereduced: bad argument (1..%d groups)", BN_MAXG);
    UP_REQUIRE(dtype == UP_DT_F32, UP_ERR_UNSUPPORTED, "bn_bwd_groups_prereduced: fp32 only");
    UP_REQUIRE(!relu || relu_bits, UP_ERR_INVALID, "bn_bwd_groups_prereduced: relu needs the sign bits of the forward output");
    UP_REQUIRE(C % 4 == 0 && rows_per_group * (C / 4) < (1ll << 31), UP_ERR_UNSUPPORTED, "bn_bwd_groups_prereduced: C %% 4 or tensor too large");
    UP_REQUIRE(workspace_bytes >= (size_t)groups * 2 * C * sizeof(float), UP_ERR_WORKSPACE, "bn_bwd_groups_prereduced: workspace too small");
    UP_REQUIRE(!relu_bits || (rows_per_group * C) % 32 == 0, UP_ERR_UNSUPPORTED,
               "bn_bwd_groups_prereduced: rows_per_group * C must be a multiple of 32");
    const bool done = launch_bn_bwd_groups<float>((const float*)dz, lddz, relu_bits, (const float*)y, ldy, gamma, coef, relu, (float*)dy,
                                                  lddy, (float*)dres, lddres, dgamma, dbeta, workspace, rows_per_group, C, groups,
                                                  as_stream(stream), partial, tiles);
    UP_REQUIRE(done, UP_ERR_UNSUPPORTED, "bn_bwd_groups_prereduced: no row-strided geometry for C = %d (use up_bn_bwd_groups_t)", C);
    return check_launch("bn_bwd_groups_prereduced");
}
extern "C" int up_bn_bwd_groups_finalized_t(const void* dz, int lddz, const uint32_t* relu_bits, const void* y, int ldy,
                                            const float* gamma, const float* coef, int relu, void* dy, int lddy, void* dres, int lddres,
                                            const float* gsum, int64_t rows_per_group, int C, int groups, int dtype, void* stream) {
    UP_REQUIRE(dz && y && dy && gamma && coef && gsum && groups > 0 && groups <= BN_MAXG && rows_per_group > 0, UP_ERR_INVALID,
               "bn_bwd_groups_finalized: bad argument (1..%d groups)", BN_MAXG);
    UP_REQUIRE(dtype == UP_DT_F32, UP_ERR_UNSUPPORTED, "bn_bwd_groups_finalized: fp32 only");
    UP_REQUIRE(!relu || relu_bits, UP_ERR_INVALID, "bn_bwd_groups_finalized: relu needs the sign bits of the forward output");
    UP_REQUIRE(C % 4 == 0 && rows_per_group * (C / 4) < (1ll << 31), UP_ERR_UNSUPPORTED, "bn_bwd_groups_finalized: C %% 4 or tensor too large");
    UP_REQUIRE(!relu_bits || (rows_per_group * C) % 32 == 0, UP_ERR_UNSUPPORTED,
               "bn_bwd_groups_finalized: rows_per_group * C must be a multiple of 32");
    const bool done = launch_bn_bwd_groups<float>((const float*)dz, lddz, relu_bits, (const float*)y, ldy, gamma, coef, relu, (float*)dy,
                                                  lddy, (float*)dres, lddres, nullptr, nullptr, nullptr, rows_per_group, C, groups,
                                                  as_stream(stream), nullptr, 0, gsum);
    UP_REQUIRE(done, UP_ERR_UNSUPPORTED, "bn_bwd_groups_finalized: no row-strided geometry for C = %d", C);
    return check_launch("bn_bwd_groups_finalized");
}
extern "C" int up_bn_bwd_groups_prereduced_ok(int64_t rows_per_group, int C, int groups, int ld) {
    dim3 grid;
    int lcs = 0;
    return groups >= 1 && groups <= BN_MAXG && ld % 4 == 0 && rows_geometry<float>(rows_per_group, C, grid, lcs) ? 1 : 0;
}

extern "C" int up_relu_bwd(const float* dz, const float* z, float* dx, int64_t n, void* stream) {
    UP_REQUIRE(dz && z && dx && n > 0, UP_ERR_INVALID, "relu_bwd: bad argument");
    hipLaunchKernelGGL(relu_bwd_kernel, dim3(grid_for(n)), dim3(256), 0, as_stream(stream), dz, z, dx, n);
    return check_launch("relu_bwd");
}

extern "C" int up_dropout_fwd_step_t(const void* x, void* y, uint8_t* mask, const float* ext_mask, int64_t n, float p,
                                     uint64_t seed, const uint64_t* step_device, int dtype, void* stream) {
    UP_REQUIRE(x && y && mask && n > 0 && p >= 0.f && p < 1.f, UP_ERR_INVALID, "dropout_fwd: bad argument");
    UP_REQUIRE(dtype == UP_DT_F32 || dtype == UP_DT_BF16, UP_ERR_INVALID, "dropout_fwd: dtype %d", dtype);
    if (dtype == UP_DT_BF16)
        hipLaunchKernelGGL(dropout_fwd_kernel<bf16_t>, dim3(grid_for(n)), dim3(256), 0, as_stream(stream), (const bf16_t*)x,
                           (bf16_t*)y, mask, ext_mask, n, p, 1.0f / (1.0f - p), seed, step_device);
    else
        hipLaunchKernelGGL(dropout_fwd_kernel<float>, dim3(grid_for(n)), dim3(256), 0, as_stream(stream), (const float*)x,
// ... 43 lines not shown
```

unipose_amd/modules.py:

```python
from __future__ import annotations

import math

import torch
import torch.nn as nn

from . import ops


def _kaiming_all(module: nn.Module):
    for m in module.modules():
        if isinstance(m, nn.Conv2d):
            nn.init.kaiming_normal_(m.weight)
        elif isinstance(m, nn.BatchNorm2d):
            nn.init.ones_(m.weight)
            nn.init.zeros_(m.bias)


_GLOBAL_FWD_HOOKS = getattr(torch.nn.modules.module, "_global_forward_hooks", {})
_GLOBAL_PRE_HOOKS = getattr(torch.nn.modules.module, "_global_forward_pre_hooks", {})


class Bottleneck(nn.Module):
    expansion = 4

    def __init__(self, inplanes, planes, stride=1, dilation=1, downsample=None, BatchNorm=nn.BatchNorm2d):
        super().__init__()
        self.conv1 = nn.Conv2d(inplanes, planes, 1, bias=False)
        self.bn1 = BatchNorm(planes)
        self.conv2 = nn.Conv2d(planes, planes, 3, stride=stride, dilation=dilation, padding=dilation, bias=False)
        self.bn2 = BatchNorm(planes)
        self.conv3 = nn.Conv2d(planes, planes * 4, 1, bias=False)
        self.bn3 = BatchNorm(planes * 4)
        self.relu = nn.ReLU(inplace=True)
        self.downsample = downsample
        self.stride = stride
        self.dilation = dilation

    def forward(self, x):
        grad = torch.is_grad_enabled()
        link = ops.GradLink() if self.downsample is None and x.requires_grad and grad else None
        s_in = getattr(x, "_up_bnslot", None) if link is not None else None
        s1, s2, s3 = (ops.BnSlot(), ops.BnSlot(), ops.BnSlot()) if grad else (None, None, None)
        if self._forward_hooks or self._forward_pre_hooks or _GLOBAL_FWD_HOOKS or _GLOBAL_PRE_HOOKS:
            s_in = s3 = None
        link_ds = ops.GradLink() if self.downsample is not None and x.requires_grad and grad else None
        y = ops.conv_bn_act(x, self.conv1, self.bn1, relu=True, link_in=link if link is not None else link_ds, slot_in=s_in,
                            slot_out=s1)
        y = ops.conv_bn_act(y, self.conv2, self.bn2, relu=True, slot_in=s1, slot_out=s2)
        if self.downsample is not None:
            x = ops.conv_bn_act(x, self.downsample[0], self.downsample[1], relu=False, link_dx=link_ds)
        out = ops.conv_bn_act(y, self.conv3, self.bn3, relu=True, residual=x, link_out=link, slot_in=s2, slot_out=s3)
        if s3 is not None and s3.y is not None:
            out._up_bnslot = s3
        return out


class ResNet(nn.Module):

    def __init__(self, layers=(3, 4, 23, 3), output_stride=16, BatchNorm=nn.BatchNorm2d, pretrained_path=None):
        super().__init__()
        if output_stride == 16:
            strides, dilations = (1, 2, 2, 1), (1, 1, 1, 2)
        elif output_stride == 8:
            strides, dilations = (1, 2, 1, 1), (1, 1, 2, 4)
        else:
            raise NotImplementedError
        self.inplanes = 64
        self.conv1 = nn.Conv2d(3, 64, 7, stride=2, padding=3, bias=False)
        self.bn1 = BatchNorm(64)
        self.relu = nn.ReLU(inplace=True)
        self.maxpool = nn.MaxPool2d(3, 2, 1)
        self.layer1 = self._stage(64, [1] * layers[0], strides[0], dilations[0], BatchNorm)
        self.layer2 = self._stage(128, [1] * layers[1], strides[1], dilations[1], BatchNorm)
        self.layer3 = self._stage(256, [1] * layers[2], strides[2], dilations[2], BatchNorm)
        self.layer4 = self._stage(512, [1, 2, 4], strides[3], dilations[3], BatchNorm)
        self._init_weight()
        if pretrained_path:
            self.load_pretrained(pretrained_path)

    def _stage(self, planes, grid, stride, dilation, BatchNorm):
        down = None
        if stride != 1 or self.inplanes != planes * 4:
            down = nn.Sequential(nn.Conv2d(self.inplanes, planes * 4, 1, stride=stride, bias=False),
                                 BatchNorm(planes * 4))
        blocks = [Bottleneck(self.inplanes, planes, stride, grid[0] * dilation, down, BatchNorm)]
        self.inplanes = planes * 4
        for g in grid[1:]:
            blocks.append(Bottleneck(self.inplanes, planes, 1, g * dilation, None, BatchNorm))
        return nn.Sequential(*blocks)

    def _init_weight(self):
        for m in self.modules():
            if isinstance(m, nn.Conv2d):
                fan = m.kernel_size[0] * m.kernel_size[1] * m.out_channels
                m.weight.data.normal_(0, math.sqrt(2.0 / fan))
            elif isinstance(m, nn.BatchNorm2d):
                m.weight.data.fill_(1)
                m.bias.data.zero_()

    def load_pretrained(self, path):
        src = torch.load(path, map_location="cpu")
        own = self.state_dict()
        own.update({k: v for k, v in src.items() if k in own})
        self.load_state_dict(own)

    def forward(self, x_nhwc):
        x = ops.conv_bn_act(x_nhwc, self.conv1, self.bn1, relu=True)
        x = ops.MaxPool3s2.apply(x, ops.storage_dtype())
        x = self.layer1(x)
        low = x
        x = self.layer4(self.layer3(self.layer2(x)))
        return x, low


def build_backbone(backbone, output_stride, BatchNorm):
    if backbone == "resnet":
        return ResNet((3, 4, 23, 3), output_stride, BatchNorm)
    raise NotImplementedError


class _AtrousModule(nn.Module):

    def __init__(self, inplanes, planes, kernel_size, padding, dilation, BatchNorm):
        super().__init__()
        self.atrous_conv = nn.Conv2d(inplanes, planes, kernel_size, stride=1, padding=padding, dilation=dilation,
                                     bias=False)
        self.bn = BatchNorm(planes)
        self.relu = nn.ReLU()
        _kaiming_all(self)

    def forward(self, x):
        return ops.conv_bn_act(x, self.atrous_conv, self.bn, relu=True)


class WASP(nn.Module):

    def __init__(self, backbone, output_stride, BatchNorm, video=False):
        super().__init__()
        inplanes = 2048
        if output_stride == 16:
            dil = (24, 18, 12, 6)
        elif output_stride == 8:
            dil = (48, 36, 24, 12)
        else:
            raise NotImplementedError
        self.aspp1 = _AtrousModule(inplanes, 256, 1, 0, dil[0], BatchNorm)
        self.aspp2 = _AtrousModule(256, 256, 3, dil[1], dil[1], BatchNorm)
        self.aspp3 = _AtrousModule(256, 256, 3, dil[2], dil[2], BatchNorm)
        self.aspp4 = _AtrousModule(256, 256, 3, dil[3], dil[3], BatchNorm)
        gap = [nn.AdaptiveAvgPool2d((1, 1)), nn.Conv2d(inplanes, 256, 1, stride=1, bias=False)]
        if not video:
            gap.append(nn.BatchNorm2d(256))
        gap.append(nn.ReLU())
        self.global_avg_pool = nn.Sequential(*gap)
        self.conv1 = nn.Conv2d(1280, 256, 1, bias=False)
        self.conv2 = nn.Conv2d(256, 256, 1, bias=False)
        self.bn1 = BatchNorm(256)
        self.relu = nn.ReLU()
        self.dropout = nn.Dropout(0.5)
        self.video = video
        _kaiming_all(self)

    def forward(self, x):
        x1 = self.aspp1(x)
        x2 = self.aspp2(x1)
        x3 = self.aspp3(x2)
        x4 = self.aspp4(x3)
        n = x1.shape[0]
        ys = ops.conv_bias_act(ops.conv_bias_act(torch.cat((x1, x2, x3, x4), 0), self.conv2), self.conv2)
        br = ops.SplitBatch.apply(ys, 4)
        g = ops.GlobalAvgPool.apply(x)
        if self.video:
            g = ops.conv_bias_act(g, self.global_avg_pool[1], relu=True)
        else:
            g = ops.conv_bn_act(g, self.global_avg_pool[1], self.global_avg_pool[2], relu=True)
        g = ops.Bilinear.apply(g, x4.shape[1], x4.shape[2])
        y = ops.ConcatC.apply(0, *br, g)
        y = ops.conv_bn_act(y, self.conv1, self.bn1, relu=True)
        return ops.dropout(y, self.dropout)


def build_wasp(backbone, output_stride, BatchNorm, video=False):
    return WASP(backbone, output_stride, BatchNorm, video)


class Decoder(nn.Module):

    def __init__(self, dataset, num_classes, backbone, BatchNorm, bbox=False):
        super().__init__()
        if backbone != "resnet":
            raise NotImplementedError
        self.conv1 = nn.Conv2d(256, 48, 1, bias=False)
        self.bn1 = BatchNorm(48)
        self.relu = nn.ReLU()
        self.conv2 = nn.Conv2d(2048, 256, 1, bias=False)
        self.bn2 = BatchNorm(256)
        self.last_conv = nn.Sequential(nn.Conv2d(304, 256, 3, stride=1, padding=1, bias=False), BatchNorm(256),
                                       nn.ReLU(), nn.Dropout(0.5),
                                       nn.Conv2d(256, 256, 3, stride=1, padding=1, bias=False), BatchNorm(256),
                                       nn.ReLU(), nn.Dropout(0.1),
                                       nn.Conv2d(256, num_classes + (6 if bbox else 1), 1, stride=1))
        self.maxpool = nn.MaxPool2d(3, 2, 1)
        _kaiming_all(self)

# ... 59 lines not shown
```

unipose_amd/ops.py:

```python
from __future__ import annotations

import collections
import ctypes as C
import os
import weakref
from typing import Optional

import torch
from torch.autograd import Function
from torch.autograd.function import once_differentiable

from . import _C

BN_EPS_DEFAULT = 1e-5


def rup4(c: int) -> int:
    return (c + 3) // 4 * 4


def rup32(c: int) -> int:
    return (c + 31) // 32 * 32


# ... 281 lines not shown
        _launch_repack(self, weight, "up_pack_weights_bf16_batched", "pack_weights_bf16_batched", 64)
        for e in live:
            e[1] = e[0]()._version


_PACK16_CACHE = {}


def _packed_bf16(weight: torch.Tensor, d: _C.ConvDesc):
    ps = _PACK16_CACHE.get(weight.device.index)
    if ps is None:
        ps = _PACK16_CACHE[weight.device.index] = _Pack16Set()
    return ps.get(weight, d)


def invalidate_packed_weights():
    for ps in list(_PACK_CACHE.values()) + list(_PACK16_CACHE.values()):
        for e in ps.entries.values():
            e[1] = -1


OPTIMIZER_STEPS = 0


def _optimizer_stepped(optimizer, _args, _kwargs):
    global OPTIMIZER_STEPS
    OPTIMIZER_STEPS += 1
    try:
        ids = {id(p) for g in optimizer.param_groups for p in g["params"]}
    except Exception:
        return invalidate_packed_weights()
    for ps in list(_PACK_CACHE.values()) + list(_PACK16_CACHE.values()):
        for k, e in ps.entries.items():
            if k in ids:
                e[1] = -1


try:
    from torch.optim.optimizer import register_optimizer_step_post_hook as _reg_step_hook
    _STEP_HOOK = _reg_step_hook(_optimizer_stepped)
except ImportError:
    _STEP_HOOK = None


DEBUG_PACK = os.environ.get("UNIPOSE_DEBUG_PACK", "0") != "0"


def _check_packed(weight, d, wf):
    ref = torch.empty_like(wf)
    _C.check(_C.lib().up_pack_weights(C.byref(d), _dense(weight).data_ptr(), ref.data_ptr(), None, _stream(weight)), "pack_weights")
    if not torch.equal(ref, wf):
        raise _C.UniPoseHipError(
            f"stale packed weight image for a {tuple(weight.shape)} convolution weight: the parameter changed without the cache "
            "noticing (edited through .data / a raw pointer?) — call ops.invalidate_packed_weights() after such edits")


def packed_fwd(weight: torch.Tensor, d: _C.ConvDesc) -> torch.Tensor:
    wf = _packed(weight, d)[0]
    if DEBUG_PACK:
        _check_packed(weight, d, wf)
    return wf


def packed_dgrad(weight: torch.Tensor, d: _C.ConvDesc) -> torch.Tensor:
    return _packed(weight, d)[1]


def conv_fwd_raw(x, weight, cfg, *, scale=None, shift=None, bias=None, residual=None, relu=False, stats=False,
                 out=None, out_f32=False, fold=None):
    _dev_ok(x, weight, scale, shift, bias, residual)
    d = make_desc(x, weight, cfg, None if out is None else _nhwc_ok(out))
    out_f32 = out_f32 and x.dtype == torch.bfloat16
    if out is None:
        alloc = torch.zeros if d.ldy != d.K else torch.empty
        out = alloc((d.N, d.P, d.Q, d.ldy), dtype=torch.float32 if out_f32 else x.dtype, device=x.device)
    ep = _C.ConvEpilogue()
    ep.scale, ep.shift, ep.bias = _ptr(scale), _ptr(shift), _ptr(bias)
    ep.residual = _ptr(residual)
    ep.ldr = _nhwc_ok(residual) if residual is not None else 0
    ep.relu = int(relu)
    st = None
    if x.dtype == torch.bfloat16:
        math = MATH_BF16S
    elif CONV_MATH in (MATH_BF16X3, MATH_BF16, MATH_BF16S) and d.Cp % 32 == 0:
        math = min(CONV_MATH, MATH_BF16)
    else:
        math = MATH_F32
    if stats:
        tiles = _C.lib().up_conv_stats_tiles_math(C.byref(d), math)
        st = torch.empty((tiles, d.K, 3), dtype=torch.float32, device=x.device)
        ep.stats = st.data_ptr()
        if fold is not None:
            ep.fold = C.pointer(fold)
    if x.dtype == torch.bfloat16:
        if d.Cp % 32 or (residual is not None and residual.dtype != x.dtype) or \
                out.dtype != (torch.float32 if out_f32 else x.dtype) or (out_f32 and (residual is not None or stats)):
            raise NotImplementedError(f"bf16-storage convolution needs 32-aligned input channels (got {d.Cp}) and bf16 "
                                      "residual / output tensors (fp32 output: no residual, no statistics)")
        wf, _ = _packed_bf16(weight, d)
        _C.check(_C.lib().up_conv2d_fwd_bf16(C.byref(d), x.data_ptr(), wf[0].data_ptr(), wf[1].data_ptr(),
                                             out.data_ptr(), C.byref(ep), MATH_BF16S_F32OUT if out_f32 else MATH_BF16S,
                                             _stream(x)), "conv2d_fwd_bf16s")
    elif CONV_MATH in (MATH_BF16X3, MATH_BF16, MATH_BF16S) and d.Cp % 32 == 0:
        wf, _ = _packed_bf16(weight, d)
        _C.check(_C.lib().up_conv2d_fwd_bf16(C.byref(d), x.data_ptr(), wf[0].data_ptr(), wf[1].data_ptr(),
                                             out.data_ptr(), C.byref(ep), min(CONV_MATH, MATH_BF16), _stream(x)),
                 "conv2d_fwd_bf16")
    else:
        wp = packed_fwd(weight, d)
        _C.check(_C.lib().up_conv2d_fwd(C.byref(d), x.data_ptr(), wp.data_ptr(), out.data_ptr(), C.byref(ep),
                                        _stream(x)), "conv2d_fwd")
    return out, d, st


GROUPED_TILES = os.environ.get("UNIPOSE_GROUPED_TILES", "0") != "0"


def conv_fwd_grouped_raw(x, weight, cfg, groups):
    if not GROUPED_TILES or x.dtype != torch.float32 or CONV_MATH != MATH_F32:
        return None
    _dev_ok(x, weight)
    d = make_desc(x, weight, cfg)
    tiles = _C.lib().up_conv_stats_tiles_grouped(C.byref(d), groups)
    if tiles <= 0:
        return None
    alloc = torch.zeros if d.ldy != d.K else torch.empty
    out = alloc((d.N, d.P, d.Q, d.ldy), dtype=x.dtype, device=x.device)
    st = torch.empty((groups, tiles, d.K, 3), dtype=torch.float32, device=x.device)
    wp = packed_fwd(weight, d)
    _C.check(_C.lib().up_conv2d_fwd_grouped(C.byref(d), x.data_ptr(), wp.data_ptr(), out.data_ptr(), st.data_ptr(), groups,
                                            _stream(x)), "conv2d_fwd_grouped")
    return out, d, st


class BnSlot:
    __slots__ = ("y", "bits", "mean", "invstd", "C", "partial", "dz_ptr", "dz_version", "groups", "gstride", "dgb", "gsum")

    def __init__(self, y=None, bits=None, mean=None, invstd=None, C=0):
        self.y, self.bits, self.mean, self.invstd, self.C = y, bits, mean, invstd, C
        self.partial, self.dz_ptr, self.dz_version = None, 0, -1
        self.dgb = None
        self.gsum = None
        self.groups, self.gstride = 1, 0

    def clear(self):
        self.y = self.bits = self.mean = self.invstd = self.partial = self.dgb = self.gsum = None
        self.dz_ptr, self.dz_version = 0, -1
        self.groups, self.gstride = 1, 0

    def matches(self, dz, y):
        return self.partial is not None and self.dz_ptr == dz.data_ptr() and self.dz_version == dz._version and self.y is y


HOST_COUNTERS = {"bn_prereduced": 0, "dx_handed_over": 0, "bn_fwd_folded": 0, "bn_bwd_folded": 0}
BN_FUSE_REDUCE = os.environ.get("UNIPOSE_BN_FUSE_REDUCE", "1") != "0"
MASKED_ADDEND = os.environ.get("UNIPOSE_MASKED_ADDEND", "1") != "0"
GROUPED_REDUCE = os.environ.get("UNIPOSE_GROUPED_REDUCE", "1") != "0"
DX_HANDOVER = os.environ.get("UNIPOSE_DX_HANDOVER", "1") != "0"
BNRED_MIN_K = int(os.environ.get("UNIPOSE_BNRED_MIN_K", "0"))
BNRED_MIN_K_BF16 = int(os.environ.get("UNIPOSE_BNRED_MIN_K_BF16", "0"))


def dgrad_extras_tiles(d: _C.ConvDesc, x_shape, dtype) -> int:
    if dtype == torch.bfloat16:
        math = MATH_BF16S
    elif dtype == torch.float32 and CONV_MATH == MATH_F32:
        math = MATH_F32
    else:
        return 0
    dd = _C.ConvDesc.from_buffer_copy(d)
    dd.ldx = x_shape[3]
    return _C.lib().up_conv2d_bwd_data_tiles_math(C.byref(dd), math)


def conv_bwd_data_raw(dy, weight, d: _C.ConvDesc, x_shape, dev, add=None, bn_slot=None, add_bits=None):
    n, h, w, cp = x_shape
    alloc = torch.zeros if cp != d.C else torch.empty
    dx = alloc((n, h, w, cp), dtype=dy.dtype, device=dev)
    dd = _C.ConvDesc.from_buffer_copy(d)
    dd.ldx = cp
    dd.ldy = _nhwc_ok(dy)
    ld_add = _nhwc_ok(add) if add is not None else 0
    ex_math = MATH_BF16S if dy.dtype == torch.bfloat16 else (MATH_F32 if CONV_MATH == MATH_F32 else -1)
    tiles = 0
    want_slot = bn_slot is not None and bn_slot.y is not None and bn_slot.C == d.C == cp and bn_slot.y.dtype == dy.dtype and \
        bn_slot.y.shape[:3] == (n, h, w) and d.R * d.S * d.Kp >= (BNRED_MIN_K_BF16 if dy.dtype == torch.bfloat16 else BNRED_MIN_K)
    groups = bn_slot.groups if want_slot else 1
    if (want_slot or add_bits is not None) and ex_math >= 0:
        tiles = _C.lib().up_conv2d_bwd_data_tiles_math(C.byref(dd), ex_math)
        if groups > 1 and tiles > 0:
            gt = _C.lib().up_conv2d_bwd_data_tiles_grouped(C.byref(dd), groups) if ex_math == MATH_F32 else 0
            if gt > 0:
                tiles = groups * gt
            else:
                want_slot, groups = False, 1
                if add_bits is None:
                    tiles = 0
    if add_bits is not None and tiles <= 0:
        raise _C.UniPoseHipError("conv_bwd_data_raw: this launch cannot mask its addend (check dgrad_extras_tiles first)")
    if tiles > 0:
        ep = _C.DgradEpilogue()
        ep.add, ep.add_relu_bits, ep.ld_add = _ptr(add), _ptr(add_bits), ld_add
        if want_slot:
            partial = torch.empty((tiles, d.C, 2), dtype=torch.float32, device=dev)
            sl = _C.BnReduceSlot()
            sl.y, sl.relu_bits, sl.mean, sl.invstd = bn_slot.y.data_ptr(), _ptr(bn_slot.bits), bn_slot.mean.data_ptr(), \
                bn_slot.invstd.data_ptr()
            sl.partial, sl.ld, sl.C = partial.data_ptr(), _nhwc_ok(bn_slot.y), d.C
            sl.group_stride = bn_slot.gstride if groups > 1 else 0
            dgb = gsum = None
            if groups > 1 or not _DEFER["on"]:
                dgb = torch.empty((2, d.C), dtype=torch.float32, device=dev)
                sl.dgamma, sl.dbeta = dgb[0].data_ptr(), dgb[1].data_ptr()
                if groups > 1:
                    gsum = torch.empty((groups, 2, d.C), dtype=torch.float32, device=dev)
                    sl.gsum = gsum.data_ptr()
            ep.bn = C.pointer(sl)
            ep.groups = groups
        if ex_math == MATH_BF16S:
            if d.Kp % 32 or (add is not None and add.dtype != dy.dtype):
                raise NotImplementedError("bf16-storage data gradient needs 32-aligned output channels and a bf16 addend")
            wimg = _packed_bf16(weight, d)[1][0]
        else:
            wimg = packed_dgrad(weight, d)
        _C.check(_C.lib().up_conv2d_bwd_data_ex(C.byref(dd), dy.data_ptr(), wimg.data_ptr(), dx.data_ptr(), C.byref(ep), ex_math,
                                                _stream(dy)), "conv2d_bwd_data_ex")
        if want_slot:
            bn_slot.partial, bn_slot.dz_ptr, bn_slot.dz_version = partial, dx.data_ptr(), dx._version
            bn_slot.dgb = dgb if (dgb is not None and sl.folded) else None
            bn_slot.gsum = gsum if bn_slot.dgb is not None else None
        return dx
    if dy.dtype == torch.bfloat16:
        if d.Kp % 32 or (add is not None and add.dtype != dy.dtype):
            raise NotImplementedError("bf16-storage data gradient needs 32-aligned output channels and a bf16 addend")
        _, wd16 = _packed_bf16(weight, d)
        _C.check(_C.lib().up_conv2d_bwd_data_bf16(C.byref(dd), dy.data_ptr(), wd16[0].data_ptr(), wd16[1].data_ptr(),
                                                  dx.data_ptr(), _ptr(add), ld_add, MATH_BF16S, _stream(dy)),
                 "conv2d_bwd_data_bf16s")
    elif CONV_MATH in (MATH_BF16X3, MATH_BF16, MATH_BF16S) and d.Kp % 32 == 0:
        _, wd16 = _packed_bf16(weight, d)
        _C.check(_C.lib().up_conv2d_bwd_data_bf16(C.byref(dd), dy.data_ptr(), wd16[0].data_ptr(), wd16[1].data_ptr(),
                                                  dx.data_ptr(), _ptr(add), ld_add, min(CONV_MATH, MATH_BF16),
                                                  _stream(dy)), "conv2d_bwd_data_bf16")
    else:
        wd = packed_dgrad(weight, d)
        _C.check(_C.lib().up_conv2d_bwd_data(C.byref(dd), dy.data_ptr(), wd.data_ptr(), dx.data_ptr(), _ptr(add),
                                             ld_add, _stream(dy)), "conv2d_bwd_data")
    return dx


class GradLink:
    __slots__ = ("grad", "armed", "bits", "masked_ok")

    def __init__(self):
        self.grad = None
        self.armed = False
        self.bits = None
        self.masked_ok = False


def conv_bwd_weight_raw(x, dy, weight_shape, d: _C.ConvDesc, want_bias: bool, ws_tag: str = "main", out=None, accumulate=None,
                        db_out=None):
    if accumulate is None:
        accumulate = out is not None
    dd = _C.ConvDesc.from_buffer_copy(d)
    dd.ldx = _nhwc_ok(x)
    dd.ldy = _nhwc_ok(dy)
    need = _C.lib().up_conv2d_bwd_weight_workspace(C.byref(dd))
    ws = workspace(x.device, need, ws_tag)
    dw = out if out is not None else torch.empty(weight_shape, dtype=torch.float32, device=x.device)
    db = (db_out if db_out is not None else torch.empty(weight_shape[0], dtype=torch.float32, device=x.device)) if want_bias else None
    if x.dtype == torch.bfloat16 and dy.dtype == torch.bfloat16:
        math = MATH_BF16S
    elif x.dtype != torch.float32 or dy.dtype != torch.float32:
        raise TypeError(f"weight gradient of mixed element types {x.dtype} / {dy.dtype}")
    else:
        bf = CONV_MATH in (MATH_BF16, MATH_BF16S) and (WGRAD_BF16_ANY_WIDTH or (dd.Cp % 32 == 0 and dd.Kp % 32 == 0))
        math = MATH_BF16 if bf else MATH_F32
    _C.check(_C.lib().up_conv2d_bwd_weight_acc(C.byref(dd), x.data_ptr(), dy.data_ptr(), dw.data_ptr(), _ptr(db), ws.data_ptr(),
                                               ws.numel(), math, int(bool(accumulate)), _stream(x)), "conv2d_bwd_weight")
    return dw, db


ASYNC_WGRAD = os.environ.get("UNIPOSE_SYNC_WGRAD", "") == ""
_SIDE = {}
_PASS = {"seen": set(), "task": None, "keep": []}
KEEP_WGRAD_INPUTS = os.environ.get("UNIPOSE_KEEP_WGRAD_INPUTS", "0") != "0"
_DEFER = {"on": False, "acc": {}, "bn": {}, "shared": {}}
_SHARED_USES = {}


def _count_shared_use(weight):
    key = id(weight)
    if key not in _SHARED_USES:
        import weakref
        _SHARED_USES[key] = 0
        weakref.finalize(weight, _SHARED_USES.pop, key, None)
    _SHARED_USES[key] += 1


class deferred_wgrad:

    def __enter__(self):
        if _DEFER["on"]:
            raise RuntimeError("ops.deferred_wgrad() does not nest")
        _DEFER["on"], _DEFER["acc"], _DEFER["bn"], _DEFER["shared"] = True, {}, {}, {}
        return self

    def __exit__(self, exc_type, exc, tb):
        acc, bn, shared = _DEFER["acc"], _DEFER["bn"], _DEFER["shared"]
        _DEFER["acc"], _DEFER["bn"], _DEFER["shared"], _DEFER["on"] = {}, {}, {}, False
        if exc_type is None:
            wgrad_fence()
            pending = [e for e in shared.values() if e[2] > 0]
            if pending:
                raise RuntimeError(f"ops.deferred_wgrad: {len(pending)} shared non-leaf weight(s) still wait for "
                                   f"{sum(e[2] for e in pending)} use(s) whose gradient never arrived; their sums were not handed to autograd")
            pairs = []
            for ent in acc.values():
                pairs.append((ent[0], ent[1]))
                if ent[2] is not None:
                    pairs.append((ent[2], ent[3]))
            for gamma, beta, dgb in bn.values():
                pairs += [(gamma, dgb[0]), (beta, dgb[1])]
            for p, buf in pairs:
                if p.grad is None:
                    p.grad = buf
                else:
                    p.grad.add_(buf)
        return False


_GRAD_DEST = {"fn": None}


def set_grad_destinations(fn):
    _GRAD_DEST["fn"] = fn


def cu_mask_stream(dev, mask_bits):
    words = (C.c_uint32 * 8)()
    for b in mask_bits:
        words[b // 32] |= 1 << (b % 32)
    h = C.c_void_p()
    _C.check(_C.lib().up_stream_create_cu_mask(words, 8, C.byref(h)), "stream_create_cu_mask")
    return torch.cuda.ExternalStream(h.value, device=dev)


def _side_stream(dev):
    st = _SIDE.get(dev.index)
    if st is None:
        ncu = int(os.environ.get("UNIPOSE_SIDE_CUS", "0"))
        if ncu > 0 and dev.type == "cuda":
            stride = max(1, int(os.environ.get("UNIPOSE_SIDE_CU_STRIDE", "1")))
            bits, b = [], 0
            while len(bits) < ncu:
                if b not in bits:
                    bits.append(b)
                b = (b + stride) % 256
                if b in bits:
                    b = (b + 1) % 256
            st = cu_mask_stream(dev, bits)
        else:
            st = torch.cuda.Stream(device=dev, priority=int(os.environ.get("UNIPOSE_SIDE_PRIO", "0")))
        _SIDE[dev.index] = st
    return st


def wgrad_fence(dev=None):
    want = None
    if dev is not None:
        dev = torch.device(dev)
        if dev.type != "cuda":
            return
        want = dev.index if dev.index is not None else torch.cuda.current_device()
    for idx, st in _SIDE.items():
        if want is None or want == idx:
            torch.cuda.current_stream(st.device).wait_stream(st)


def _end_of_backward():
    wgrad_fence()
    _PASS["seen"].clear()
    _PASS["keep"].clear()
    _PASS["task"] = None


def _hold_for_side(side, *tensors):
    if KEEP_WGRAD_INPUTS:
        _PASS["keep"].extend(tensors)
    else:
        for t in tensors:
            t.record_stream(side)


def _graph_task_id():
    try:
        return torch._C._current_graph_task_id()
    except AttributeError:
        return 0


def _shared_wgrad(x, dy, weight, d, want_bias):
# ... 22 lines not shown
            return None, None
        main.wait_stream(side)
    else:
        conv_bwd_weight_raw(x, dy, weight.shape, d, want_bias, out=ent[0], accumulate=not first, db_out=ent[1])
        if ent[2] > 0:
            return None, None
    return ent[0], ent[1]


def _ensure_end_of_backward(dev):
    task = _graph_task_id()
    if task == -1:
        return False
    if _PASS["task"] != task:
        if _PASS["task"] is not None:
            wgrad_fence(dev)
            _PASS["seen"].clear()
            _PASS["keep"].clear()
        try:
            torch.autograd.Variable._execution_engine.queue_callback(_end_of_backward)
            _PASS["task"] = task
        except RuntimeError:
            return False
    return True


DEFER_BIAS = os.environ.get("UNIPOSE_DEFER_BIAS", "1") != "0"
DEFER_SHARED = os.environ.get("UNIPOSE_DEFER_SHARED", "1") != "0"
DEFER_WAIT = int(os.environ.get("UNIPOSE_DEFER_WAIT", "1"))


def conv_bwd_weight(x, dy, weight, d, want_bias, bias=None):
    if _DEFER["on"] and DEFER_SHARED and not weight.is_leaf and weight.requires_grad:
        return _shared_wgrad(x, dy, weight, d, want_bias)
    if not (ASYNC_WGRAD and dy.is_cuda and weight.is_leaf):
        return conv_bwd_weight_raw(x, dy, weight.shape, d, want_bias)
    dev = dy.device
    main, side = torch.cuda.current_stream(dev), _side_stream(dev)
    task = _graph_task_id()
    if task == -1:
        return conv_bwd_weight_raw(x, dy, weight.shape, d, want_bias)
    if _PASS["task"] != task:
        if _PASS["task"] is not None:
            wgrad_fence(dev)
            _PASS["seen"].clear()
            _PASS["keep"].clear()
        try:
            torch.autograd.Variable._execution_engine.queue_callback(_end_of_backward)
            _PASS["task"] = task
        except RuntimeError:
            return conv_bwd_weight_raw(x, dy, weight.shape, d, want_bias)
    bias_ok = not want_bias or (DEFER_BIAS and bias is not None and bias.is_leaf and not getattr(bias, "_post_accumulate_grad_hooks", None))
    defer = _DEFER["on"] and bias_ok and not getattr(weight, "_post_accumulate_grad_hooks", None)
    entry = _DEFER["acc"].get(id(weight)) if defer else None
    dst = None
    if entry is None:
        if _GRAD_DEST["fn"] is not None and not defer and weight.grad is None and id(weight) not in _PASS["seen"]:
            dst = _GRAD_DEST["fn"](weight)
        if dst is None:
            dst = torch.empty(weight.shape, dtype=torch.float32, device=dev)
    db_buf = torch.empty(weight.shape[0], dtype=torch.float32, device=dev) if want_bias else None
    side.wait_stream(main)
    with torch.cuda.stream(side):
        if entry is not None:
            conv_bwd_weight_raw(x, dy, weight.shape, d, want_bias, ws_tag="side", out=entry[1], db_out=entry[3])
            _hold_for_side(side, x, dy)
            if want_bias and DEFER_WAIT:
                main.wait_stream(side)
            return None, None
        dw, db = conv_bwd_weight_raw(x, dy, weight.shape, d, want_bias, ws_tag="side", out=dst, accumulate=False, db_out=db_buf)
        if defer:
            _DEFER["acc"][id(weight)] = (weight, dw, bias if want_bias else None, db)
            _hold_for_side(side, x, dy)
            if want_bias and DEFER_WAIT > 1:
                main.wait_stream(side)
            return None, None
    _hold_for_side(side, x, dy)
    key = id(weight)
    if key in _PASS["seen"] or weight.grad is not None:
        main.wait_stream(side)
    _PASS["seen"].add(key)
    return dw, db


_RELU_TRACE = None


def set_relu_trace(lst):
    global _RELU_TRACE
    _RELU_TRACE = lst


class ConvBias(Function):

    @staticmethod
    def forward(ctx, x, weight, bias, cfg: ConvCfg, relu: bool, out_f32: bool = False):
        y, d, _ = conv_fwd_raw(x, weight, cfg, bias=bias, relu=relu, out_f32=out_f32)
        if relu and _RELU_TRACE is not None:
            _RELU_TRACE.append(y.detach())
        ctx.d, ctx.relu, ctx.has_bias = d, relu, bias is not None
        ctx.bias = bias
        if ctx.needs_input_grad[1] and not weight.is_leaf:
            _count_shared_use(weight)
            ctx.shared_w = weight
        ctx.save_for_backward(x, weight, y if relu else None)
        return y

    @staticmethod
    @once_differentiable
    def backward(ctx, dy):
        x, weight, y = ctx.saved_tensors
        dy = _dense(dy)
        if dy.dtype != x.dtype and not ctx.relu:
            dy = dy.to(x.dtype)
        if ctx.relu:
            if dy.dtype != torch.float32:
                dy = torch.where(y > 0, dy, torch.zeros_like(dy))
            else:
                g = torch.empty_like(dy)
                _C.check(_C.lib().up_relu_bwd(dy.data_ptr(), y.data_ptr(), g.data_ptr(), dy.numel(), _stream(dy)),
                         "relu_bwd")
                dy = g
        dx = conv_bwd_data_raw(dy, weight, ctx.d, x.shape, x.device) if ctx.needs_input_grad[0] else None
        dw = db = None
        if ctx.needs_input_grad[1]:
            dw, db = conv_bwd_weight(x, dy, getattr(ctx, "shared_w", weight), ctx.d, ctx.has_bias and ctx.needs_input_grad[2], bias=ctx.bias)
        elif ctx.has_bias and ctx.needs_input_grad[2]:
            db = dy.reshape(-1, dy.shape[3]).float().sum(0)[:weight.shape[0]]
        return dx, dw, db, None, None, None


_BN_GROUPS = {"n": 1}
EXACT_STATS_ROWS = 256


class bn_groups:

    def __init__(self, n: int):
        self.n, self.prev = int(n), 1

    def __enter__(self):
        self.prev, _BN_GROUPS["n"] = _BN_GROUPS["n"], self.n
        return self

    def __exit__(self, exc_type, exc, tb):
        _BN_GROUPS["n"] = self.prev
        return False


class ConvBnAct(Function):

    @staticmethod
    def forward(ctx, x, weight, gamma, beta, residual, rm, rv, cfg: ConvCfg, relu: bool, train: bool, eps: float,
                momentum: float, link_in=None, link_out=None, slot_in=None, slot_out=None, link_dx=None):
        L = _C.lib()
        dev = x.device
        k = weight.shape[0]
        groups = _BN_GROUPS["n"] if train else 1
        if groups > 1:
            if x.shape[0] % groups:
                raise ValueError(f"batch {x.shape[0]} is not a multiple of {groups} BatchNorm groups")
            d0 = make_desc(x, weight, cfg)
            fused = conv_fwd_grouped_raw(x, weight, cfg, groups) if (d0.N * d0.P * d0.Q) // groups > EXACT_STATS_ROWS else None
            if fused is not None:
                y, d, st = fused
                tiles = st.shape[1]
            else:
                y, d, _ = conv_fwd_raw(x, weight, cfg)
            rows = d.N * d.P * d.Q
            rpg = rows // groups
            if rpg <= 1:
                raise ValueError(f"Expected more than 1 value per channel when training, got input size "
                                 f"{(d.N // groups, k, d.P, d.Q)}")
            coef = torch.empty((groups, 4, k), dtype=torch.float32, device=dev)
            done = False
            if fused is None:
                tiles = 1 if rpg <= EXACT_STATS_ROWS else L.up_bn_batch_stats_tiles(rpg)
                st = torch.empty((groups, tiles, k, 3), dtype=torch.float32, device=dev)
                if rpg <= EXACT_STATS_ROWS:
                    _C.check(L.up_bn_exact_stats_t(y.data_ptr(), d.ldy, rpg, k, groups, _dt(y), st.data_ptr(), _stream(x)), "bn_exact_stats")
                else:
                    _C.check(L.up_bn_stats_groups_t(y.data_ptr(), d.ldy, rpg, k, groups, _dt(y), st.data_ptr(), eps, momentum,
                                                    _ptr(rm), _ptr(rv), gamma.data_ptr(), beta.data_ptr(), coef.data_ptr(),
                                                    _stream(x)), "bn_stats_groups")
                    done = True
            if not done:
                _C.check(L.up_bn_finalize_groups(st.data_ptr(), tiles, k, groups, rpg, eps, momentum, _ptr(rm), _ptr(rv),
                                                 gamma.data_ptr(), beta.data_ptr(), coef.data_ptr(), _stream(x)), "bn_finalize_groups")
        elif train:
            small = x.shape[0] * ((x.shape[1] + 2 * cfg.pad - cfg.dil * (weight.shape[2] - 1) - 1) // cfg.stride + 1) * \
                ((x.shape[2] + 2 * cfg.pad - cfg.dil * (weight.shape[3] - 1) - 1) // cfg.stride + 1) <= EXACT_STATS_ROWS
            coef = torch.empty((4, k), dtype=torch.float32, device=dev)
            fold = None
            if not small:
                fold = _C.BnFold()
                fold.eps, fold.momentum, fold.running_mean, fold.running_var = eps, momentum, _ptr(rm), _ptr(rv)
                fold.gamma, fold.beta = gamma.data_ptr(), beta.data_ptr()
                base, step = coef.data_ptr(), 4 * k
                fold.mean, fold.invstd, fold.scale, fold.shift = base, base + step, base + 2 * step, base + 3 * step
            y, d, st = conv_fwd_raw(x, weight, cfg, stats=not small, fold=fold)
            rows = d.N * d.P * d.Q
            if rows <= 1:
                raise ValueError(f"Expected more than 1 value per channel when training, got input size "
                                 f"{(d.N, k, d.P, d.Q)}")
            if small:
                assert rows <= EXACT_STATS_ROWS
                st = torch.empty((1, k, 3), dtype=torch.float32, device=dev)
                _C.check(L.up_bn_exact_stats_t(y.data_ptr(), d.ldy, rows, k, 1, _dt(y), st.data_ptr(), _stream(x)), "bn_exact_stats")
            if fold is not None and fold.folded:
                HOST_COUNTERS["bn_fwd_folded"] += 1
            else:
                _C.check(L.up_bn_finalize(st.data_ptr(), st.shape[0], k, eps, momentum, _ptr(rm), _ptr(rv),
                                          gamma.data_ptr(), beta.data_ptr(), coef[0].data_ptr(), coef[1].data_ptr(),
                                          coef[2].data_ptr(), coef[3].data_ptr(), _stream(x)), "bn_finalize")
        else:
            y, d, _ = conv_fwd_raw(x, weight, cfg)
            rows = d.N * d.P * d.Q
            coef = torch.empty((4, k), dtype=torch.float32, device=dev)
            coef[0].copy_(rm)
            torch.rsqrt(rv + eps, out=coef[1])
            _C.check(L.up_bn_eval_coeffs(gamma.data_ptr(), beta.data_ptr(), rm.data_ptr(), rv.data_ptr(), eps, k,
                                         coef[2].data_ptr(), coef[3].data_ptr(), _stream(x)), "bn_eval_coeffs")
        z = torch.empty_like(y) if d.ldy == k else torch.zeros_like(y)
        bits = torch.empty(((rows * k + 31) // 32,), dtype=torch.int32, device=dev) \
            if relu and any(ctx.needs_input_grad[:5]) else None
        if residual is not None and residual.dtype != y.dtype:
            raise TypeError(f"residual {residual.dtype} vs convolution output {y.dtype}")
        if groups > 1:
            _C.check(L.up_bn_apply_groups_t(y.data_ptr(), d.ldy, coef.data_ptr(), beta.data_ptr(), _ptr(residual),
                                            _nhwc_ok(residual) if residual is not None else 0, int(relu), z.data_ptr(), d.ldy,
                                            _ptr(bits), rows // groups, k, groups, _dt(y), _stream(x)), "bn_apply_groups")
        else:
            _C.check(L.up_bn_apply_centered_t(y.data_ptr(), d.ldy, coef[0].data_ptr(), coef[2].data_ptr(), beta.data_ptr(),
                                              _ptr(residual), _nhwc_ok(residual) if residual is not None else 0, int(relu),
                                              z.data_ptr(), d.ldy, _ptr(bits), rows, k, _dt(y), _stream(x)), "bn_apply")
        if relu and _RELU_TRACE is not None:
            _RELU_TRACE.append(z.detach())
        ctx.d, ctx.relu, ctx.train, ctx.has_res, ctx.groups = d, relu, train, residual is not None, groups
        ctx.beta = beta
        ctx.link_in, ctx.link_out = link_in, link_out
        if link_in is not None:
            link_in.armed = True
            link_in.masked_ok = MASKED_ADDEND and dgrad_extras_tiles(d, x.shape, x.dtype) > 0
        ctx.link_dx = link_dx if (DX_HANDOVER and link_dx is not None and ctx.needs_input_grad[0]) else None
        ctx.slot_out = None
        if slot_out is not None:
            slot_out.clear()
            if BN_FUSE_REDUCE and groups == 1 and d.ldy == k and (bits is not None or not relu) and \
                    ((y.dtype == torch.float32 and CONV_MATH == MATH_F32) or y.dtype == torch.bfloat16):
                slot_out.y, slot_out.bits, slot_out.mean, slot_out.invstd, slot_out.C = y, bits, coef[0], coef[1], k
                ctx.slot_out = slot_out
            elif BN_FUSE_REDUCE and GROUPED_REDUCE and 1 < groups <= 8 and d.ldy == k and (bits is not None or not relu) and \
                    y.dtype == torch.float32 and CONV_MATH == MATH_F32 and \
                    L.up_bn_bwd_groups_prereduced_ok((d.N * d.P * d.Q) // groups, k, groups, d.ldy):
                slot_out.y, slot_out.bits, slot_out.mean, slot_out.invstd, slot_out.C = y, bits, coef[0, 0], coef[0, 1], k
                slot_out.groups, slot_out.gstride = groups, 4 * k
                ctx.slot_out = slot_out
        ctx.slot_in = slot_in if (slot_in is not None and slot_in.y is not None and ctx.needs_input_grad[0]) else None
        ctx.save_for_backward(x, weight, gamma, y, bits, coef)
        return z

    @staticmethod
    def _slot_usable(ctx, dz, y):
        so = ctx.slot_out
        if so is None or not so.matches(dz, y):
            return False
        hooks = getattr(ctx, "z_hooks", None)
        return hooks is not None and len(hooks) == 0

    @staticmethod
    @once_differentiable
    def backward(ctx, dz):
        x, weight, gamma, y, bits, coef = ctx.saved_tensors
        L, d = _C.lib(), ctx.d
        dz = _dense(dz)
        k = weight.shape[0]
        rows = d.N * d.P * d.Q
        fresh = torch.empty_like if d.ldy == k else torch.zeros_like
        dy = fresh(y)
        lo = ctx.link_out
        masked = ctx.has_res and lo is not None and lo.armed and lo.masked_ok and ctx.relu and bits is not None and d.ldy == k \
            and (ctx.groups == 1 or GROUPED_REDUCE)
        dres = fresh(y) if ctx.has_res and not masked else None
        dgb = torch.empty((2, k), dtype=torch.float32, device=x.device)
        if dz.dtype != y.dtype:
            raise TypeError(f"gradient {dz.dtype} vs saved convolution output {y.dtype}")
        if ctx.groups > 1:
            rpg = rows // ctx.groups
            ws = workspace(x.device, L.up_bn_bwd_groups_workspace(rpg, k, ctx.groups))
            so = ctx.slot_out
            if so is not None and so.groups == ctx.groups and ConvBnAct._slot_usable(ctx, dz, y):
                partial, so.partial, so.dz_ptr, so.dz_version = so.partial, None, 0, -1
                HOST_COUNTERS["bn_prereduced"] += 1
                done, gsum, so.dgb, so.gsum = so.dgb, so.gsum, None, None
                if done is not None and gsum is not None:
                    HOST_COUNTERS["bn_bwd_folded"] += 1
                    dgb = done
                    _C.check(L.up_bn_bwd_groups_finalized_t(dz.data_ptr(), d.ldy, _ptr(bits), y.data_ptr(), d.ldy, gamma.data_ptr(),
                                                            coef.data_ptr(), int(ctx.relu), dy.data_ptr(), d.ldy, _ptr(dres), d.ldy,
                                                            gsum.data_ptr(), rpg, k, ctx.groups, _dt(y), _stream(x)),
                             "bn_bwd_groups_finalized")
                    return ConvBnAct._finish_backward(ctx, x, weight, d, dy, dres, dgb, True, (dz, bits) if masked else None)
                _C.check(L.up_bn_bwd_groups_prereduced_t(dz.data_ptr(), d.ldy, _ptr(bits), y.data_ptr(), d.ldy, gamma.data_ptr(),
                                                         coef.data_ptr(), int(ctx.relu), dy.data_ptr(), d.ldy, _ptr(dres), d.ldy,
                                                         dgb[0].data_ptr(), dgb[1].data_ptr(), ws.data_ptr(), ws.numel(),
                                                         partial.data_ptr(), partial.shape[0] // ctx.groups, rpg, k, ctx.groups,
                                                         _dt(y), _stream(x)), "bn_bwd_groups_prereduced")
                return ConvBnAct._finish_backward(ctx, x, weight, d, dy, dres, dgb, True, (dz, bits) if masked else None)
            _C.check(L.up_bn_bwd_groups_t(dz.data_ptr(), d.ldy, _ptr(bits), y.data_ptr(), d.ldy, gamma.data_ptr(), coef.data_ptr(),
                                          int(ctx.relu), dy.data_ptr(), d.ldy, _ptr(dres), d.ldy, dgb[0].data_ptr(),
                                          dgb[1].data_ptr(), ws.data_ptr(), ws.numel(), rpg, k, ctx.groups, _dt(y), _stream(x)),
                     "bn_bwd_groups")
            return ConvBnAct._finish_backward(ctx, x, weight, d, dy, dres, dgb, True, (dz, bits) if masked else None)
        need = L.up_bn_bwd_workspace(rows, k)
        ws = workspace(x.device, need)
        beta = ctx.beta
        hand_over = True
        acc = None
        if _DEFER["on"] and gamma.is_leaf and beta.is_leaf and ctx.needs_input_grad[2] and ctx.needs_input_grad[3] and \
                not getattr(gamma, "_post_accumulate_grad_hooks", None) and not getattr(beta, "_post_accumulate_grad_hooks", None):
            hand_over = False
            entry = _DEFER["bn"].get(id(gamma))
            if entry is None:
                _DEFER["bn"][id(gamma)] = (gamma, beta, dgb)
            else:
                acc = entry[2]
        so = ctx.slot_out
        if ConvBnAct._slot_usable(ctx, dz, y):
            partial, so.partial, so.dz_ptr, so.dz_version = so.partial, None, 0, -1
            HOST_COUNTERS["bn_prereduced"] += 1
            done, so.dgb = so.dgb, None
            if done is not None and acc is None:
                HOST_COUNTERS["bn_bwd_folded"] += 1
                dgb = done
                _C.check(L.up_bn_bwd_finalized_t(dz.data_ptr(), d.ldy, _ptr(bits), y.data_ptr(), d.ldy, gamma.data_ptr(),
                                                 coef[0].data_ptr(), coef[1].data_ptr(), int(ctx.relu), int(ctx.train), dy.data_ptr(),
                                                 d.ldy, _ptr(dres), d.ldy, dgb[0].data_ptr(), dgb[1].data_ptr(), rows, k, _dt(y),
                                                 _stream(x)), "bn_bwd_finalized")
                return ConvBnAct._finish_backward(ctx, x, weight, d, dy, dres, dgb, hand_over, (dz, bits) if masked else None)
            _C.check(L.up_bn_bwd_prereduced_t(dz.data_ptr(), d.ldy, _ptr(bits), y.data_ptr(), d.ldy, gamma.data_ptr(),
                                              coef[0].data_ptr(), coef[1].data_ptr(), int(ctx.relu), int(ctx.train), dy.data_ptr(),
                                              d.ldy, _ptr(dres), d.ldy, dgb[0].data_ptr(), dgb[1].data_ptr(),
                                              acc[0].data_ptr() if acc is not None else None,
                                              acc[1].data_ptr() if acc is not None else None, partial.data_ptr(),
                                              partial.shape[0], rows, k, _dt(y), _stream(x)), "bn_bwd_prereduced")
            return ConvBnAct._finish_backward(ctx, x, weight, d, dy, dres, dgb, hand_over, (dz, bits) if masked else None)
        _C.check(L.up_bn_bwd_acc_t(dz.data_ptr(), d.ldy, None, 0, _ptr(bits), y.data_ptr(), d.ldy, gamma.data_ptr(),
                                   coef[0].data_ptr(), coef[1].data_ptr(), int(ctx.relu), int(ctx.train), dy.data_ptr(),
                                   d.ldy, _ptr(dres), d.ldy, dgb[0].data_ptr(), dgb[1].data_ptr(),
                                   acc[0].data_ptr() if acc is not None else None,
                                   acc[1].data_ptr() if acc is not None else None, ws.data_ptr(),
                                   ws.numel(), rows, k, _dt(y), _stream(x)), "bn_bwd")
        return ConvBnAct._finish_backward(ctx, x, weight, d, dy, dres, dgb, hand_over, (dz, bits) if masked else None)

    @staticmethod
    def _finish_backward(ctx, x, weight, d, dy, dres, dgb, hand_over, masked_skip=None):
        add = add_bits = None
        if ctx.link_in is not None:
            li = ctx.link_in
            add, add_bits, li.grad, li.bits, li.armed = li.grad, li.bits, None, None, False
        si = ctx.slot_in
        if si is not None and ctx.link_in is not None and add is None:
            si = None
        if ctx.needs_input_grad[0]:
            dx = conv_bwd_data_raw(dy, weight, d, x.shape, x.device, add, bn_slot=si, add_bits=add_bits)
        else:
            dx = add if add_bits is None else None
        ld = ctx.link_dx
        if ld is not None and ld.armed and dx is not None and ld.grad is None:
            ld.grad, dx = dx, None
            HOST_COUNTERS["dx_handed_over"] += 1
        if masked_skip is not None:
            ctx.link_out.grad, ctx.link_out.bits = masked_skip
        elif ctx.link_out is not None and ctx.link_out.armed and dres is not None:
            ctx.link_out.grad, dres = dres, None
        dw = conv_bwd_weight(x, dy, weight, d, False)[0] if ctx.needs_input_grad[1] else None
        return dx, dw, (dgb[0] if hand_over else None), (dgb[1] if hand_over else None), dres, None, None, None, None, None, \
            None, None, None, None, None, None, None


def conv_bn_act_eval_fused(x, weight, gamma, beta, rm, rv, cfg, relu, residual=None, eps=BN_EPS_DEFAULT):
    k = weight.shape[0]
    coef = torch.empty((2, k), dtype=torch.float32, device=x.device)
    _C.check(_C.lib().up_bn_eval_coeffs(gamma.data_ptr(), beta.data_ptr(), rm.data_ptr(), rv.data_ptr(), eps, k,
                                        coef[0].data_ptr(), coef[1].data_ptr(), _stream(x)), "bn_eval_coeffs")
    y, _, _ = conv_fwd_raw(x, weight, cfg, scale=coef[0], shift=coef[1], residual=residual, relu=relu)
    return y


_BN_COUNT = {"mode": None, "seen": None}


class bn_counters:

    def __init__(self, module):
        self.module = module

    def __enter__(self):
        if _BN_COUNT["mode"] is not None:
            self.own = False
            return self
        self.own = True
        bns = self.module.__dict__.get("_up_bn_list")
        if bns is None:
            bns = self.module.__dict__["_up_bn_list"] = [m for m in self.module.modules()
                                                         if isinstance(m, torch.nn.BatchNorm2d)]
        self.sig = tuple(m.training for m in bns)
        plan = self.module.__dict__.get("_up_bn_plan")
        if plan is not None and plan[0] == self.sig:
            if plan[1]:
                torch._foreach_add_(plan[1], _BN_GROUPS["n"] if any(self.sig) else 1)
            _BN_COUNT["mode"] = "skip"
        else:
            _BN_COUNT["mode"], _BN_COUNT["seen"] = "record", []
        return self

    def __exit__(self, exc_type, exc, tb):
        if self.own:
            if _BN_COUNT["mode"] == "record" and exc_type is None:
                self.module.__dict__["_up_bn_plan"] = (self.sig, list(_BN_COUNT["seen"]))
            _BN_COUNT["mode"], _BN_COUNT["seen"] = None, None
        return False


class FoldedBatchNorm(torch.nn.Identity):
    """Stands where a BatchNorm2d stood after ``checkpoint.load_folded``: its affine map lives in the preceding
    convolution's weight and bias (inference export, SURVEY 8f N1).  No parameters, no buffers, inference only."""


def conv_bn_act(x, conv, bn, relu=True, residual=None, link_in=None, link_out=None, slot_in=None, slot_out=None, link_dx=None):
    weight, cfg = conv.weight, ConvCfg(conv.stride[0], conv.padding[0], conv.dilation[0])
    if isinstance(bn, FoldedBatchNorm):
        if torch.is_grad_enabled() and (x.requires_grad or weight.requires_grad):
            raise NotImplementedError("a BatchNorm-folded network is an inference export: run it under torch.no_grad()")
        return conv_fwd_raw(x, weight, cfg, bias=conv.bias, residual=residual, relu=relu)[0]
    need_grad = torch.is_grad_enabled() and (x.requires_grad or conv.weight.requires_grad or bn.weight.requires_grad)
    train = bn.training
    if not train and not need_grad:
        return conv_bn_act_eval_fused(x, weight, bn.weight, bn.bias, bn.running_mean, bn.running_var, cfg, relu,
                                      residual, bn.eps)
    if train and _BN_GROUPS["n"] > 1 and bn.momentum is None:
        raise NotImplementedError("grouped BatchNorm (ops.bn_groups) with momentum=None (cumulative average)")
    if train and bn.track_running_stats and _BN_COUNT["mode"] != "skip":
        bn.num_batches_tracked.add_(_BN_GROUPS["n"])
        if _BN_COUNT["mode"] == "record":
            _BN_COUNT["seen"].append(bn.num_batches_tracked)
    if bn.momentum is not None:
        mom = bn.momentum
    elif train and bn.track_running_stats:
        mom = 1.0 / float(max(int(bn.num_batches_tracked.item()), 1))
    else:
        mom = 0.0
    rm, rv = (bn.running_mean, bn.running_var) if bn.track_running_stats else (None, None)
    z = ConvBnAct.apply(x, weight, bn.weight, bn.bias, residual, rm, rv, cfg, relu, train, bn.eps, mom,
                        link_in, link_out, slot_in, slot_out, link_dx)
    node = z.grad_fn
    if node is not None and getattr(node, "slot_out", None) is not None:
        hooks = z._backward_hooks
        if hooks is None:
            hooks = z._backward_hooks = collections.OrderedDict()
            node._register_hook_dict(z)
        node.z_hooks = hooks
    return z


def conv_bias_act(x, conv, relu=False, out_f32=False):
    cfg = ConvCfg(conv.stride[0], conv.padding[0], conv.dilation[0])
    return ConvBias.apply(x, conv.weight, conv.bias, cfg, relu, out_f32)


class SplitBatch(Function):

    @staticmethod
    def forward(ctx, x, n):
        b = x.shape[0] // n
        ctx.b, ctx.tail = b, x.shape[1:]
        return tuple(x.narrow(0, i * b, b) for i in range(n))

    @staticmethod
    def backward(ctx, *grads):
        like = next((g for g in grads if g is not None), None)
        if like is None:
            return None, None
        parts = [g if g is not None else torch.zeros((ctx.b,) + tuple(ctx.tail), dtype=like.dtype, device=like.device) for g in grads]
        return torch.cat(parts, 0), None


class ToNHWC(Function):
    @staticmethod
    def forward(ctx, x):
        _dev_ok(x)
        x = _dense(x)
        n, c, h, w = x.shape
        y = torch.empty((n, h, w, rup4(c)), dtype=torch.float32, device=x.device)
        _C.check(_C.lib().up_nchw_to_nhwc(x.data_ptr(), y.data_ptr(), n, c, h, w, rup4(c), _stream(x)), "nchw_to_nhwc")
        ctx.c = c
        return y

    @staticmethod
    @once_differentiable
    def backward(ctx, dy):
        dy = _dense(dy)
        n, h, w, ld = dy.shape
        dx = torch.empty((n, ctx.c, h, w), dtype=torch.float32, device=dy.device)
        _C.check(_C.lib().up_nhwc_to_nchw(dy.data_ptr(), ld, dx.data_ptr(), n, ctx.c, h, w, _stream(dy)), "nhwc_to_nchw")
        return dx


class ToNCHW(Function):
    @staticmethod
    def forward(ctx, x, c: int):
        _dev_ok(x)
        n, h, w, _ = x.shape
        ld = _nhwc_ok(x)
        y = torch.empty((n, c, h, w), dtype=torch.float32, device=x.device)
        _C.check(_C.lib().up_nhwc_to_nchw_t(x.data_ptr(), ld, y.data_ptr(), n, c, h, w, _dt(x), _stream(x)),
                 "nhwc_to_nchw")
        ctx.ld, ctx.dtype = x.shape[3], x.dtype
        return y

    @staticmethod
    @once_differentiable
    def backward(ctx, dy):
        dy = _dense(dy)
        n, c, h, w = dy.shape
        dx = torch.empty((n, h, w, ctx.ld), dtype=ctx.dtype, device=dy.device)
        _C.check(_C.lib().up_nchw_to_nhwc_t(dy.data_ptr(), dx.data_ptr(), n, c, h, w, ctx.ld, _dt(dx), _stream(dy)),
                 "nchw_to_nhwc")
        return dx, None


class MaxPool3s2(Function):

    @staticmethod
    def forward(ctx, x, out_dtype=None):
        _dev_ok(x)
        n, h, w, c = x.shape
        p, q = (h - 1) // 2 + 1, (w - 1) // 2 + 1
        y = torch.empty((n, p, q, c), dtype=out_dtype or x.dtype, device=x.device)
        if y.dtype == torch.bfloat16 and c % 8:
            raise ValueError(f"bf16 tensors need channel counts that are multiples of 8, got {c}")
        idx = torch.empty((n, p, q, c), dtype=torch.uint8, device=x.device)
        _C.check(_C.lib().up_maxpool3s2_fwd_t(x.data_ptr(), _nhwc_ok(x), y.data_ptr(), c, idx.data_ptr(), n, h, w, c,
                                              p, q, _dt(x), _dt(y), _stream(x)), "maxpool_fwd")
        ctx.save_for_backward(idx)
        ctx.hw, ctx.in_dtype = (h, w), x.dtype
        return y

    @staticmethod
    @once_differentiable
    def backward(ctx, dy):
        (idx,) = ctx.saved_tensors
        dy = _dense(dy)
        n, p, q, c = dy.shape
        h, w = ctx.hw
        dx = torch.empty((n, h, w, c), dtype=ctx.in_dtype, device=dy.device)
        _C.check(_C.lib().up_maxpool3s2_bwd_t(dy.data_ptr(), c, idx.data_ptr(), dx.data_ptr(), c, n, h, w, c, p, q,
                                              _dt(dy), _dt(dx), _stream(dy)), "maxpool_bwd")
        return dx, None


class Bilinear(Function):

    @staticmethod
    def forward(ctx, x, p: int, q: int):
        _dev_ok(x)
        n, h, w, c = x.shape
        y = torch.empty((n, p, q, c), dtype=x.dtype, device=x.device)
        _C.check(_C.lib().up_bilinear_fwd_t(x.data_ptr(), _nhwc_ok(x), y.data_ptr(), c, n, h, w, c, p, q, _dt(x),
                                            _stream(x)), "bilinear_fwd")
        ctx.hw = (h, w)
        return y

    @staticmethod
    @once_differentiable
    def backward(ctx, dy):
        dy = _dense(dy)
        n, p, q, c = dy.shape
        h, w = ctx.hw
        dx = torch.empty((n, h, w, c), dtype=dy.dtype, device=dy.device)
        _C.check(_C.lib().up_bilinear_bwd_t(dy.data_ptr(), c, dx.data_ptr(), c, n, h, w, c, p, q, _dt(dy), _stream(dy)),
                 "bilinear_bwd")
        return dx, None, None


class GlobalAvgPool(Function):

    @staticmethod
    def forward(ctx, x):
        _dev_ok(x)
        n, h, w, c = x.shape
        y = torch.empty((n, 1, 1, c), dtype=x.dtype, device=x.device)
        _C.check(_C.lib().up_gap_fwd_t(x.data_ptr(), _nhwc_ok(x), y.data_ptr(), n, h * w, c, _dt(x), _stream(x)),
                 "gap_fwd")
        ctx.hw = (h, w)
        return y

    @staticmethod
    @once_differentiable
    def backward(ctx, dy):
        dy = _dense(dy)
        n, _, _, c = dy.shape
        h, w = ctx.hw
        dx = torch.empty((n, h, w, c), dtype=dy.dtype, device=dy.device)
        _C.check(_C.lib().up_gap_bwd_t(dy.data_ptr(), dx.data_ptr(), c, n, h * w, c, _dt(dy), _stream(dy)), "gap_bwd")
        return dx


# ... 484 lines not shown
```

Before: 523.6 images/sec.

## Fuse downsample BN apply into residual BN apply pass and reuse relu mask in backward

In bottleneck blocks with a downsample branch, the downsample BatchNorm apply is deferred. It is computed on the fly inside the conv3 BN+residual+ReLU apply kernel, which reads the raw downsample conv output and normalizes it as the residual. This removes one full elementwise read/write pass over the downsample activation. In backward, the residual gradient is passed through as dz instead of materializing a separate dres buffer, and the downsample BN backward reuses the conv3 relu bits. The cost is more cross-op state carried through a host-side pair object, with more fragile coupling between the two autograd nodes.

```diff
diff --git a/include/unipose_hip.h b/include/unipose_hip.h
--- a/include/unipose_hip.h
+++ b/include/unipose_hip.h
@@ -169,6 +169,9 @@
                   int relu, void* z, int ldz, uint32_t* relu_bits, int64_t rows, int C, int dtype, void* stream);
 int up_bn_apply_centered_t(const void* y, int ldy, const float* mean, const float* scale, const float* beta, const void* residual,
                            int ldr, int relu, void* z, int ldz, uint32_t* relu_bits, int64_t rows, int C, int dtype, void* stream);
+int up_bn_apply_pair_t(const void* y, int ldy, const float* mean, const float* scale, const float* beta, const void* y2, int ld2,
+                       const float* mean2, const float* scale2, const float* beta2, int relu, void* z, int ldz, uint32_t* relu_bits,
+                       int64_t rows, int C, int dtype, void* stream);
 int up_bn_bwd_t(const void* dz, int lddz, const void* z, int ldz, const uint32_t* relu_bits, const void* y, int ldy,
                 const float* gamma, const float* mean, const float* invstd, int relu, int use_batch_stats,
                 void* dy, int lddy, void* dres, int lddres, float* dgamma, float* dbeta,
diff --git a/unipose_amd/_C.py b/unipose_amd/_C.py
--- a/unipose_amd/_C.py
+++ b/unipose_amd/_C.py
@@ -94,6 +94,7 @@
     "up_bn_finalize_groups": (_i, [_p, _i, _i, _i, _i64, _f, _f, _p, _p, _p, _p, _p, _p]),
     "up_bn_apply_groups_t": (_i, [_p, _i, _p, _p, _p, _i, _i, _p, _i, _p, _i64, _i, _i, _i, _p]),
     "up_bn_apply_centered_t": (_i, [_p, _i, _p, _p, _p, _p, _i, _i, _p, _i, _p, _i64, _i, _i, _p]),
+    "up_bn_apply_pair_t": (_i, [_p, _i, _p, _p, _p, _p, _i, _p, _p, _p, _i, _p, _i, _p, _i64, _i, _i, _p]),
     "up_bn_bwd_groups_workspace": (_sz, [_i64, _i, _i]),
     "up_bn_bwd_groups_t": (_i, [_p, _i, _p, _p, _i, _p, _p, _i, _p, _i, _p, _i, _p, _p, _p, _sz, _i64, _i, _i, _i, _p]),
     "up_relu_bwd": (_i, [_p, _p, _p, _i64, _p]),
diff --git a/unipose_amd/csrc/norm_act.hip b/unipose_amd/csrc/norm_act.hip
--- a/unipose_amd/csrc/norm_act.hip
+++ b/unipose_amd/csrc/norm_act.hip
@@ -120,10 +120,16 @@
 }
 
 template <typename T>
+__device__ __forceinline__ float pair_residual(float r, float mu2, float sc2, float sh2) {
+    const float t = (r - mu2) * sc2 + sh2;
+    if (sizeof(T) == 2) return bf_lo(pack_bf16x2(t, 0.f));
+    return t;
+}
+template <typename T, bool PAIR>
 __global__ void __launch_bounds__(256) bn_apply_kernel(const T* y, int ldy, const float* scale,
                                                        const float* shift, const float* mean, const T* res, int ldr, int relu,
                                                        T* z, int ldz, uint32_t* relu_bits, int64_t total, int C4,
-                                                       FastDiv fC4) {
+                                                       FastDiv fC4, const float* mean2, const float* scale2, const float* shift2) {
     const int lane = threadIdx.x & 63;
     for (int64_t i0 = (int64_t)blockIdx.x * 256 + (threadIdx.x & ~63); i0 < total; i0 += (int64_t)gridDim.x * 256) {
         const int64_t i = i0 + lane;
@@ -141,6 +147,14 @@
             v.w = (v.w - mu.w) * s.w + h.w;
             if (res) {
                 float4 r = ld4<T>(res + (size_t)row * ldr + c);
+                if (PAIR) {
+                    const float4 m2 = *reinterpret_cast<const float4*>(mean2 + c), s2 = *reinterpret_cast<const float4*>(scale2 + c);
+                    const float4 h2 = *reinterpret_cast<const float4*>(shift2 + c);
+                    r.x = pair_residual<T>(r.x, m2.x, s2.x, h2.x);
+                    r.y = pair_residual<T>(r.y, m2.y, s2.y, h2.y);
+                    r.z = pair_residual<T>(r.z, m2.z, s2.z, h2.z);
+                    r.w = pair_residual<T>(r.w, m2.w, s2.w, h2.w);
+                }
                 v.x += r.x;
                 v.y += r.y;
                 v.z += r.z;
@@ -190,9 +204,11 @@
     *reinterpret_cast<uint4*>(p) = u;
 }
 
+template <bool PAIR>
 __global__ void __launch_bounds__(256) bn_apply8_kernel(const bf16_t* y, int ldy, const float* scale, const float* shift,
                                                         const float* mean, const bf16_t* res, int ldr, int relu, bf16_t* z, int ldz,
-                                                        uint32_t* relu_bits, int64_t total, int C8, FastDiv fC8) {
+                                                        uint32_t* relu_bits, int64_t total, int C8, FastDiv fC8, const float* mean2,
+                                                        const float* scale2, const float* shift2) {
     const int lane = threadIdx.x & 63;
     for (int64_t i0 = (int64_t)blockIdx.x * 256 + (threadIdx.x & ~63); i0 < total; i0 += (int64_t)gridDim.x * 256) {
         const int64_t i = i0 + lane;
@@ -209,7 +225,12 @@
 #pragma unroll
             for (int e = 0; e < 8; ++e) v.v[e] = (v.v[e] - mu.v[e]) * s.v[e] + h.v[e];
             if (res) {
-                const F8 r = ld8(res + (size_t)row * ldr + c);
+                F8 r = ld8(res + (size_t)row * ldr + c);
+                if (PAIR) {
+                    const F8 m2 = ld8(mean2 + c), s2 = ld8(scale2 + c), h2 = ld8(shift2 + c);
+#pragma unroll
+                    for (int e = 0; e < 8; ++e) r.v[e] = pair_residual<bf16_t>(r.v[e], m2.v[e], s2.v[e], h2.v[e]);
+                }
 #pragma unroll
                 for (int e = 0; e < 8; ++e) v.v[e] += r.v[e];
             }
@@ -267,12 +288,13 @@
 }
 constexpr int BN_ROWS_UNROLL = 4;
 
-template <typename T>
+template <typename T, bool PAIR>
 __global__ void __launch_bounds__(256) bn_apply_rows_kernel(const T* __restrict__ y, int ldy, const float* __restrict__ scale,
                                                             const float* __restrict__ shift, const float* __restrict__ mean,
                                                             const T* __restrict__ res, int ldr,
                                                             int relu, T* __restrict__ z, int ldz, uint32_t* __restrict__ relu_bits,
-                                                            int rows, int C, int lcs, GroupArgs grp) {
+                                                            int rows, int C, int lcs, GroupArgs grp, const float* __restrict__ mean2,
+                                                            const float* __restrict__ scale2, const float* __restrict__ shift2) {
     constexpr int E = Row16<T>::E, LPW = 32 / E;
     const int lane = threadIdx.x & 63;
     const int64_t grow0 = (int64_t)blockIdx.z * rows;
@@ -290,6 +312,12 @@
 #pragma unroll
     for (int e = 0; e < E; ++e) mu[e] = 0.f;
     if (mean) ldparam<E>(mean + (size_t)blockIdx.z * grp.pstride + c, mu);
+    float sc2[E], sh2[E], mu2[E];
+    if (PAIR) {
+        ldparam<E>(scale2 + c, sc2);
+        ldparam<E>(shift2 + c, sh2);
+        ldparam<E>(mean2 + c, mu2);
+    }
     const int stride = gridDim.x * rpb;
     for (int base = blockIdx.x * rpb; base < rows; base += BN_ROWS_UNROLL * stride) {
         Row16<T> v[BN_ROWS_UNROLL], r[BN_ROWS_UNROLL];
@@ -308,7 +336,10 @@
 #pragma unroll
             for (int e = 0; e < E; ++e) {
                 float t = (v[u].v[e] - mu[e]) * sc[e] + sh[e];
-                if (res) t += r[u].v[e];
+                if (PAIR)
+                    t += pair_residual<T>(r[u].v[e], mu2[e], sc2[e], sh2[e]);
+                else if (res)
+                    t += r[u].v[e];
                 if (relu) t = fmaxf(t, 0.f);
                 v[u].v[e] = t;
                 bits |= t > 0.f ? (1u << e) : 0u;
@@ -902,40 +933,47 @@
 
 static int bn_apply_impl(const void* y, int ldy, const float* mean, const float* scale, const float* shift, const void* res,
                          int ldr, int relu, void* z, int ldz, uint32_t* relu_bits, int64_t rows, int C, int dtype,
-                         void* stream) {
+                         void* stream, const float* mean2 = nullptr, const float* scale2 = nullptr, const float* shift2 = nullptr) {
     UP_REQUIRE(y && scale && shift && z && rows > 0 && C > 0, UP_ERR_INVALID, "bn_apply: bad argument");
     UP_REQUIRE(C % 4 == 0 && ldy % 4 == 0 && ldz % 4 == 0 && (!res || ldr % 4 == 0), UP_ERR_INVALID,
                "bn_apply: C and strides must be multiples of 4");
     UP_REQUIRE(rows * (C / 4) < (1ll << 31), UP_ERR_UNSUPPORTED, "bn_apply: tensor too large");
     UP_REQUIRE(dtype == UP_DT_F32 || dtype == UP_DT_BF16, UP_ERR_INVALID, "bn_apply: dtype %d", dtype);
     int64_t total = rows * (C / 4);
+    const bool pair = scale2 != nullptr;
+    hipStream_t st = as_stream(stream);
+#define UP_BN_APPLY_LAUNCH(PAIRED, PLAIN, GRID, ...)                                                           \
+    do {                                                                                                       \
+        if (pair)                                                                                              \
+            hipLaunchKernelGGL(PAIRED, GRID, dim3(256), 0, st, __VA_ARGS__, mean2, scale2, shift2);            \
+        else                                                                                                   \
+            hipLaunchKernelGGL(PLAIN, GRID, dim3(256), 0, st, __VA_ARGS__, mean2, scale2, shift2);             \
+    } while (0)
     {
         dim3 grid;
         int lcs = 0;
         if (bn_rows_enabled() && dtype == UP_DT_BF16 && ldy % 8 == 0 && ldz % 8 == 0 && (!res || ldr % 8 == 0) &&
             rows_geometry<bf16_t>(rows, C, grid, lcs)) {
-            hipLaunchKernelGGL(bn_apply_rows_kernel<bf16_t>, grid, dim3(256), 0, as_stream(stream), (const bf16_t*)y, ldy, scale,
-                               shift, mean, (const bf16_t*)res, ldr, relu, (bf16_t*)z, ldz, relu_bits, (int)rows, C, lcs, GroupArgs{0, 0});
+            UP_BN_APPLY_LAUNCH((bn_apply_rows_kernel<bf16_t, true>), (bn_apply_rows_kernel<bf16_t, false>), grid, (const bf16_t*)y, ldy, scale, shift, mean,
+                               (const bf16_t*)res, ldr, relu, (bf16_t*)z, ldz, relu_bits, (int)rows, C, lcs, GroupArgs{0, 0});
             return check_launch("bn_apply");
         }
         if (bn_rows_enabled() && dtype == UP_DT_F32 && rows_geometry<float>(rows, C, grid, lcs)) {
-            hipLaunchKernelGGL(bn_apply_rows_kernel<float>, grid, dim3(256), 0, as_stream(stream), (const float*)y, ldy, scale,
-                               shift, mean, (const float*)res, ldr, relu, (float*)z, ldz, relu_bits, (int)rows, C, lcs, GroupArgs{0, 0});
+            UP_BN_APPLY_LAUNCH((bn_apply_rows_kernel<float, true>), (bn_apply_rows_kernel<float, false>), grid, (const float*)y, ldy, scale, shift, mean,
+                               (const float*)res, ldr, relu, (float*)z, ldz, relu_bits, (int)rows, C, lcs, GroupArgs{0, 0});
             return check_launch("bn_apply");
         }
     }
     if (dtype == UP_DT_BF16 && C % 8 == 0 && ldy % 8 == 0 && ldz % 8 == 0 && (!res || ldr % 8 == 0))
-        hipLaunchKernelGGL(bn_apply8_kernel, dim3(grid_for(total / 2)), dim3(256), 0, as_stream(stream), (const bf16_t*)y, ldy,
-                           scale, shift, mean, (const bf16_t*)res, ldr, relu, (bf16_t*)z, ldz, relu_bits, total / 2, C / 8,
-                           make_fastdiv(C / 8));
+        UP_BN_APPLY_LAUNCH((bn_apply8_kernel<true>), (bn_apply8_kernel<false>), dim3(grid_for(total / 2)), (const bf16_t*)y, ldy, scale, shift, mean,
+                           (const bf16_t*)res, ldr, relu, (bf16_t*)z, ldz, relu_bits, total / 2, C / 8, make_fastdiv(C / 8));
     else if (dtype == UP_DT_BF16)
-        hipLaunchKernelGGL(bn_apply_kernel<bf16_t>, dim3(grid_for(total)), dim3(256), 0, as_stream(stream),
-                           (const bf16_t*)y, ldy, scale, shift, mean, (const bf16_t*)res, ldr, relu, (bf16_t*)z, ldz, relu_bits,
-                           total, C / 4, make_fastdiv(C / 4));
+        UP_BN_APPLY_LAUNCH((bn_apply_kernel<bf16_t, true>), (bn_apply_kernel<bf16_t, false>), dim3(grid_for(total)), (const bf16_t*)y, ldy, scale, shift, mean,
+                           (const bf16_t*)res, ldr, relu, (bf16_t*)z, ldz, relu_bits, total, C / 4, make_fastdiv(C / 4));
     else
-        hipLaunchKernelGGL(bn_apply_kernel<float>, dim3(grid_for(total)), dim3(256), 0, as_stream(stream), (const float*)y,
-                           ldy, scale, shift, mean, (const float*)res, ldr, relu, (float*)z, ldz, relu_bits, total, C / 4,
-                           make_fastdiv(C / 4));
+        UP_BN_APPLY_LAUNCH((bn_apply_kernel<float, true>), (bn_apply_kernel<float, false>), dim3(grid_for(total)), (const float*)y, ldy, scale, shift, mean,
+                           (const float*)res, ldr, relu, (float*)z, ldz, relu_bits, total, C / 4, make_fastdiv(C / 4));
+#undef UP_BN_APPLY_LAUNCH
     return check_launch("bn_apply");
 }
 extern "C" int up_bn_apply_t(const void* y, int ldy, const float* scale, const float* shift, const void* res,
@@ -948,6 +986,12 @@
                                       int C, int dtype, void* stream) {
     UP_REQUIRE(mean, UP_ERR_INVALID, "bn_apply_centered: null mean");
     return bn_apply_impl(y, ldy, mean, scale, beta, res, ldr, relu, z, ldz, relu_bits, rows, C, dtype, stream);
+}
+extern "C" int up_bn_apply_pair_t(const void* y, int ldy, const float* mean, const float* scale, const float* beta, const void* y2,
+                                  int ld2, const float* mean2, const float* scale2, const float* beta2, int relu, void* z, int ldz,
+                                  uint32_t* relu_bits, int64_t rows, int C, int dtype, void* stream) {
+    UP_REQUIRE(mean && y2 && mean2 && scale2 && beta2, UP_ERR_INVALID, "bn_apply_pair: null pointer");
+    return bn_apply_impl(y, ldy, mean, scale, beta, y2, ld2, relu, z, ldz, relu_bits, rows, C, dtype, stream, mean2, scale2, beta2);
 }
 extern "C" int up_bn_apply(const float* y, int ldy, const float* scale, const float* shift, const float* res,
                            int ldr, int relu, float* z, int ldz, uint32_t* relu_bits, int64_t rows, int C,
@@ -1237,15 +1281,17 @@
     const GroupArgs ga{4 * C, 0};
     if (dtype == UP_DT_F32 && ldy % 4 == 0 && ldz % 4 == 0 && (!res || ldr % 4 == 0) && rows_geometry<float>(rows_per_group, C, grid, lcs)) {
         grid.z = groups;
-        hipLaunchKernelGGL(bn_apply_rows_kernel<float>, grid, dim3(256), 0, as_stream(stream), (const float*)y, ldy, coef + 2 * C,
-                           gshift, gmean, (const float*)res, ldr, relu, (float*)z, ldz, relu_bits, (int)rows_per_group, C, lcs, ga);
+        hipLaunchKernelGGL((bn_apply_rows_kernel<float, false>), grid, dim3(256), 0, as_stream(stream), (const float*)y, ldy,
+                           coef + 2 * C, gshift, gmean, (const float*)res, ldr, relu, (float*)z, ldz, relu_bits, (int)rows_per_group, C,
+                           lcs, ga, (const float*)nullptr, (const float*)nullptr, (const float*)nullptr);
         return check_launch("bn_apply_groups");
     }
     if (dtype == UP_DT_BF16 && ldy % 8 == 0 && ldz % 8 == 0 && (!res || ldr % 8 == 0) &&
         rows_geometry<bf16_t>(rows_per_group, C, grid, lcs)) {
         grid.z = groups;
-        hipLaunchKernelGGL(bn_apply_rows_kernel<bf16_t>, grid, dim3(256), 0, as_stream(stream), (const bf16_t*)y, ldy, coef + 2 * C,
-                           gshift, gmean, (const bf16_t*)res, ldr, relu, (bf16_t*)z, ldz, relu_bits, (int)rows_per_group, C, lcs, ga);
+        hipLaunchKernelGGL((bn_apply_rows_kernel<bf16_t, false>), grid, dim3(256), 0, as_stream(stream), (const bf16_t*)y, ldy,
+                           coef + 2 * C, gshift, gmean, (const bf16_t*)res, ldr, relu, (bf16_t*)z, ldz, relu_bits, (int)rows_per_group,
+                           C, lcs, ga, (const float*)nullptr, (const float*)nullptr, (const float*)nullptr);
         return check_launch("bn_apply_groups");
     }
     for (int g = 0; g < groups; ++g) {
diff --git a/unipose_amd/modules.py b/unipose_amd/modules.py
--- a/unipose_amd/modules.py
+++ b/unipose_amd/modules.py
@@ -48,9 +48,15 @@
         y = ops.conv_bn_act(x, self.conv1, self.bn1, relu=True, link_in=link if link is not None else link_ds, slot_in=s_in,
                             slot_out=s1)
         y = ops.conv_bn_act(y, self.conv2, self.bn2, relu=True, slot_in=s1, slot_out=s2)
+        pair = None
         if self.downsample is not None:
-            x = ops.conv_bn_act(x, self.downsample[0], self.downsample[1], relu=False, link_dx=link_ds)
-        out = ops.conv_bn_act(y, self.conv3, self.bn3, relu=True, residual=x, link_out=link, slot_in=s2, slot_out=s3)
+            watched = self._forward_hooks or self._forward_pre_hooks or _GLOBAL_FWD_HOOKS or _GLOBAL_PRE_HOOKS
+            if ops.BN_PAIR_FWD and self.bn3.training and self.downsample[1].training and ops._BN_GROUPS["n"] == 1 and not watched:
+                pair = ops.BnPair()
+            x = ops.conv_bn_act(x, self.downsample[0], self.downsample[1], relu=False, link_dx=link_ds, pair_out=pair)
+            if pair is not None and not pair.y_ptr:
+                pair = None
+        out = ops.conv_bn_act(y, self.conv3, self.bn3, relu=True, residual=x, link_out=link, slot_in=s2, slot_out=s3, pair_in=pair)
         if s3 is not None and s3.y is not None:
             out._up_bnslot = s3
         return out
diff --git a/unipose_amd/ops.py b/unipose_amd/ops.py
--- a/unipose_amd/ops.py
+++ b/unipose_amd/ops.py
@@ -457,11 +457,13 @@
         return self.partial is not None and self.dz_ptr == dz.data_ptr() and self.dz_version == dz._version and self.y is y
 
 
-HOST_COUNTERS = {"bn_prereduced": 0, "dx_handed_over": 0, "bn_fwd_folded": 0, "bn_bwd_folded": 0}
+HOST_COUNTERS = {"bn_prereduced": 0, "dx_handed_over": 0, "bn_fwd_folded": 0, "bn_bwd_folded": 0, "bn_pair_fwd": 0, "bn_pair_bwd": 0}
 BN_FUSE_REDUCE = os.environ.get("UNIPOSE_BN_FUSE_REDUCE", "1") != "0"
 MASKED_ADDEND = os.environ.get("UNIPOSE_MASKED_ADDEND", "1") != "0"
 GROUPED_REDUCE = os.environ.get("UNIPOSE_GROUPED_REDUCE", "1") != "0"
 DX_HANDOVER = os.environ.get("UNIPOSE_DX_HANDOVER", "1") != "0"
+BN_PAIR_FWD = os.environ.get("UNIPOSE_BN_PAIR_FWD", "1") != "0"
+BN_PAIR_BWD = os.environ.get("UNIPOSE_BN_PAIR_BWD", "1") != "0"
 BNRED_MIN_K = int(os.environ.get("UNIPOSE_BNRED_MIN_K", "0"))
 BNRED_MIN_K_BF16 = int(os.environ.get("UNIPOSE_BNRED_MIN_K_BF16", "0"))
 
@@ -554,6 +556,16 @@
     return dx
 
 
+class BnPair:
+
+    def __init__(self):
+        self.y_ptr = 0
+        self.coef = None
+        self.beta = None
+        self.bits = None
+        self.dz_ptr = 0
+
+
 class GradLink:
     __slots__ = ("grad", "armed", "bits", "masked_ok")
 
@@ -882,7 +894,8 @@
 
     @staticmethod
     def forward(ctx, x, weight, gamma, beta, residual, rm, rv, cfg: ConvCfg, relu: bool, train: bool, eps: float,
-                momentum: float, link_in=None, link_out=None, slot_in=None, slot_out=None, link_dx=None):
+                momentum: float, link_in=None, link_out=None, slot_in=None, slot_out=None, link_dx=None, pair_out=None,
+                pair_in=None):
         L = _C.lib()
         dev = x.device
         k = weight.shape[0]
@@ -951,12 +964,29 @@
             torch.rsqrt(rv + eps, out=coef[1])
             _C.check(L.up_bn_eval_coeffs(gamma.data_ptr(), beta.data_ptr(), rm.data_ptr(), rv.data_ptr(), eps, k,
                                          coef[2].data_ptr(), coef[3].data_ptr(), _stream(x)), "bn_eval_coeffs")
-        z = torch.empty_like(y) if d.ldy == k else torch.zeros_like(y)
+        ctx.pair_out = ctx.pair_in = None
+        if pair_out is not None and BN_PAIR_FWD and train and groups == 1 and d.ldy == k and not relu and residual is None and \
+                slot_out is None:
+            pair_out.y_ptr, pair_out.coef, pair_out.beta, pair_out.bits, pair_out.dz_ptr = y.data_ptr(), coef, beta, None, 0
+            ctx.pair_out = pair_out
+        z = y if ctx.pair_out is not None else torch.empty_like(y) if d.ldy == k else torch.zeros_like(y)
         bits = torch.empty(((rows * k + 31) // 32,), dtype=torch.int32, device=dev) \
             if relu and any(ctx.needs_input_grad[:5]) else None
         if residual is not None and residual.dtype != y.dtype:
             raise TypeError(f"residual {residual.dtype} vs convolution output {y.dtype}")
-        if groups > 1:
+        if pair_in is not None and (residual is None or pair_in.y_ptr != residual.data_ptr() or
+                                    groups > 1 or not train or d.ldy != k or _nhwc_ok(residual) != k):
+            raise ValueError("BnPair: the residual of the paired apply pass is the pending branch's convolution output")
+        if ctx.pair_out is not None:
+            pass
+        elif pair_in is not None:
+            pc = pair_in.coef
+            _C.check(L.up_bn_apply_pair_t(y.data_ptr(), d.ldy, coef[0].data_ptr(), coef[2].data_ptr(), beta.data_ptr(),
+                                          residual.data_ptr(), k, pc[0].data_ptr(), pc[2].data_ptr(), pair_in.beta.data_ptr(),
+                                          int(relu), z.data_ptr(), d.ldy, _ptr(bits), rows, k, _dt(y), _stream(x)), "bn_apply_pair")
+            HOST_COUNTERS["bn_pair_fwd"] += 1
+            ctx.pair_in = pair_in
+        elif groups > 1:
             _C.check(L.up_bn_apply_groups_t(y.data_ptr(), d.ldy, coef.data_ptr(), beta.data_ptr(), _ptr(residual),
                                             _nhwc_ok(residual) if residual is not None else 0, int(relu), z.data_ptr(), d.ldy,
                                             _ptr(bits), rows // groups, k, groups, _dt(y), _stream(x)), "bn_apply_groups")
@@ -1011,7 +1041,13 @@
         lo = ctx.link_out
         masked = ctx.has_res and lo is not None and lo.armed and lo.masked_ok and ctx.relu and bits is not None and d.ldy == k \
             and (ctx.groups == 1 or GROUPED_REDUCE)
-        dres = fresh(y) if ctx.has_res and not masked else None
+        pi = ctx.pair_in
+        pair_skip = pi is not None and BN_PAIR_BWD and not masked and lo is None and ctx.relu and bits is not None and \
+            ctx.groups == 1
+        if pi is not None:
+            pi.bits, pi.dz_ptr = (bits, dz.data_ptr()) if pair_skip else (None, 0)
+        ctx.pair_skip = dz if pair_skip else None
+        dres = fresh(y) if ctx.has_res and not masked and not pair_skip else None
         dgb = torch.empty((2, k), dtype=torch.float32, device=x.device)
         if dz.dtype != y.dtype:
             raise TypeError(f"gradient {dz.dtype} vs saved convolution output {y.dtype}")
@@ -1075,8 +1111,13 @@
                                               acc[1].data_ptr() if acc is not None else None, partial.data_ptr(),
                                               partial.shape[0], rows, k, _dt(y), _stream(x)), "bn_bwd_prereduced")
             return ConvBnAct._finish_backward(ctx, x, weight, d, dy, dres, dgb, hand_over, (dz, bits) if masked else None)
+        relu = int(ctx.relu)
+        po = ctx.pair_out
+        if po is not None and po.bits is not None and po.dz_ptr == dz.data_ptr():
+            relu, bits = 1, po.bits
+            HOST_COUNTERS["bn_pair_bwd"] += 1
         _C.check(L.up_bn_bwd_acc_t(dz.data_ptr(), d.ldy, None, 0, _ptr(bits), y.data_ptr(), d.ldy, gamma.data_ptr(),
-                                   coef[0].data_ptr(), coef[1].data_ptr(), int(ctx.relu), int(ctx.train), dy.data_ptr(),
+                                   coef[0].data_ptr(), coef[1].data_ptr(), relu, int(ctx.train), dy.data_ptr(),
                                    d.ldy, _ptr(dres), d.ldy, dgb[0].data_ptr(), dgb[1].data_ptr(),
                                    acc[0].data_ptr() if acc is not None else None,
                                    acc[1].data_ptr() if acc is not None else None, ws.data_ptr(),
@@ -1105,8 +1146,10 @@
         elif ctx.link_out is not None and ctx.link_out.armed and dres is not None:
             ctx.link_out.grad, dres = dres, None
         dw = conv_bwd_weight(x, dy, weight, d, False)[0] if ctx.needs_input_grad[1] else None
+        if dres is None and getattr(ctx, "pair_skip", None) is not None:
+            dres, ctx.pair_skip = ctx.pair_skip, None
         return dx, dw, (dgb[0] if hand_over else None), (dgb[1] if hand_over else None), dres, None, None, None, None, None, \
-            None, None, None, None, None, None, None
+            None, None, None, None, None, None, None, None, None
 
 
 def conv_bn_act_eval_fused(x, weight, gamma, beta, rm, rv, cfg, relu, residual=None, eps=BN_EPS_DEFAULT):
@@ -1158,7 +1201,8 @@
     convolution's weight and bias (inference export, SURVEY 8f N1).  No parameters, no buffers, inference only."""
 
 
-def conv_bn_act(x, conv, bn, relu=True, residual=None, link_in=None, link_out=None, slot_in=None, slot_out=None, link_dx=None):
+def conv_bn_act(x, conv, bn, relu=True, residual=None, link_in=None, link_out=None, slot_in=None, slot_out=None, link_dx=None,
+                pair_out=None, pair_in=None):
     weight, cfg = conv.weight, ConvCfg(conv.stride[0], conv.padding[0], conv.dilation[0])
     if isinstance(bn, FoldedBatchNorm):
         if torch.is_grad_enabled() and (x.requires_grad or weight.requires_grad):
@@ -1183,7 +1227,7 @@
         mom = 0.0
     rm, rv = (bn.running_mean, bn.running_var) if bn.track_running_stats else (None, None)
     z = ConvBnAct.apply(x, weight, bn.weight, bn.bias, residual, rm, rv, cfg, relu, train, bn.eps, mom,
-                        link_in, link_out, slot_in, slot_out, link_dx)
+                        link_in, link_out, slot_in, slot_out, link_dx, pair_out if train else None, pair_in)
     node = z.grad_fn
     if node is not None and getattr(node, "slot_out", None) is not None:
         hooks = z._backward_hooks
```

Result: no change. 526.3 images/sec (median of 6 runs) (+0.5%).
